# AbeelLab/phasm

Hardware: AMD Instinct MI355X
Metric: overlaps_per_sec (higher is better)
Workload: dtype u64

## Files before the change

include/phasm_overlap.h:

```cpp
#ifndef PHASM_OVERLAP_H
#define PHASM_OVERLAP_H

#include <stddef.h>
#include <stdint.h>

#ifdef __cplusplus
extern "C" {
#endif

#define PO_ABI_VERSION 4

typedef enum {
    PO_OK = 0,
    PO_ERR_INVALID = 1,
    PO_ERR_NOMEM = 2,
    PO_ERR_HIP = 3,
    PO_ERR_CAPACITY = 4
} po_status;

typedef struct po_handle po_handle;
typedef struct po_result po_result;

typedef struct {
    uint32_t a_idx, b_idx;
// ... 192 lines not shown

typedef struct {
    uint64_t n_edges_in;
    uint64_t n_edges_out;
    uint64_t n_nodes;
    uint64_t n_nodes_removed;
    uint64_t n_candidates;
    uint64_t n_diamonds;
    uint64_t n_rounds;
    uint64_t n_invalid;
    float ms_setup, ms_rounds, ms_emit, ms_total;
} po_diamond_stats;

po_status po_layout_diamonds(po_handle* h, po_result* edges, const po_diamond_params* params, uint8_t* edge_flags_out,
                             po_result** kept_out);
po_status po_get_diamond_stats(const po_handle* h, po_diamond_stats* out);


typedef struct {
    uint32_t reserved;
} po_merge_params;

typedef struct {
    uint64_t n_edges_in;
    uint64_t n_edges_out;
    uint64_t n_nodes;
    uint64_t n_merged;
    uint64_t n_nodes_merged;
    uint64_t max_path_nodes;
    uint64_t n_self_loops;
    uint64_t n_cycle_nodes;
    uint64_t n_rounds;
    uint64_t n_overflow;
    uint64_t n_invalid;
    float ms_links, ms_rank, ms_number, ms_emit, ms_total;
} po_merge_stats;

po_status po_layout_merge(po_handle* h, po_result* edges, const po_merge_params* params, uint8_t* edge_flags_out,
                          po_result** merged_out);
po_status po_get_merge_stats(const po_handle* h, po_merge_stats* out);

po_status po_result_merged_paths(po_result* merged, uint64_t* n_paths, uint64_t* n_members, uint64_t* offsets_out,
                                 uint64_t cap_paths, uint32_t* members_out, int32_t* prefix_out, uint64_t cap_members,
                                 int64_t* lengths_out);


typedef struct {
    uint32_t reserved;
} po_coverage_params;

typedef struct {
    uint64_t read_length_sum;
    int64_t path_length;
} po_edge_coverage;

typedef struct {
    uint64_t n_rows, n_edges;
    uint64_t n_nodes;
    uint64_t n_pairs;
    uint64_t max_set;
    uint64_t n_zero_path;
    uint64_t n_invalid;
    float ms_sets, ms_edges, ms_total;
} po_coverage_stats;

po_status po_layout_coverage(po_handle* h, po_result* graph, po_result* rows, const po_coverage_params* params,
                             po_edge_coverage* coverage_out );
po_status po_get_coverage_stats(const po_handle* h, po_coverage_stats* out);


typedef struct {
    uint32_t reserved;
} po_components_params;

typedef struct {
    uint32_t first_node;
    uint32_t n_nodes;
    uint64_t n_edges;
} po_component;

typedef struct {
    uint64_t n_nodes;
    uint64_t n_edges;
    uint64_t n_components;
    uint64_t n_singletons;
    uint64_t max_component_nodes, max_component_edges;
    uint64_t n_invalid;
    uint32_t n_rounds;
    uint32_t n_batches;
    float ms_rounds, ms_label, ms_total;
} po_components_stats;

po_status po_layout_components(po_handle* h, po_result* graph, const po_components_params* params,
                               uint32_t* node_component_out, uint32_t* edge_component_out, po_component* components_out,
                               uint64_t* n_components_out);
po_status po_get_components_stats(const po_handle* h, po_components_stats* out);


typedef struct {
    uint32_t reserved;
} po_partition_params;

typedef struct {
    uint32_t first_node;
    uint32_t n_nodes;
    uint64_t n_edges;
    uint32_t n_r_in;
    uint32_t n_re_out;
} po_scc;

#define PO_PART_R_IN 1u
#define PO_PART_RE_OUT 2u
#define PO_PART_START 4u
#define PO_PART_SINK 8u

typedef struct {
    uint64_t n_nodes;
    uint64_t n_edges;
    uint64_t n_sccs, n_nonsingleton_sccs, n_singletons;
    uint64_t n_self_loops;
    uint64_t max_scc_nodes, max_scc_edges;
    uint64_t n_trimmed;
    uint64_t n_class[5];
    uint64_t n_invalid;
    uint32_t n_outer;
    uint32_t n_trim_rounds, n_forward_rounds, n_backward_rounds;
    uint32_t n_batches;
    float ms_ranks, ms_rounds, ms_label, ms_total;
} po_partition_stats;

po_status po_layout_partition(po_handle* h, po_result* graph, const po_partition_params* params, uint32_t* node_scc_out,
                              uint8_t* node_flags_out, uint8_t* edge_class_out, po_scc* sccs_out, uint64_t* n_sccs_out);
po_status po_get_partition_stats(const po_handle* h, po_partition_stats* out);

po_status po_graph_from_edges(po_handle* h, const po_edge* edges, uint64_t n_edges, const uint32_t* node_order,
                              uint64_t n_order, po_result** out);

po_status po_result_node_order(po_result* r, uint32_t* nodes_out, uint64_t cap, uint64_t* n_out);

typedef struct {
    uint64_t n_rows;
    float ms_first_contained;
    float ms_rank;
    float ms_total;
} po_node_order_stats;
po_status po_get_node_order_stats(const po_handle* h, po_node_order_stats* out);

uint64_t po_debug_host_ranges(uint64_t* out, uint64_t cap_entries);
uint64_t po_debug_store_words(const po_handle* h, int store, const uint64_t** words);
int po_debug_expand_records(const po_cand* records, uint64_t n, const uint32_t* lengths, uint32_t n_reads, uint32_t paired,
                            po_row* rows_out, uint64_t n_rows_expected);
int po_debug_expand_packed(const uint64_t* records, uint64_t n, uint32_t sh_b, uint32_t sh_p, const uint32_t* lengths, uint32_t n_reads,
                           uint32_t paired, po_row* rows_out, uint64_t n_rows_expected);
int po_debug_fault_backtrace(int fd);
int po_debug_pointer_info(const void* p, int32_t* hip_type, int32_t* hsa_type, uint64_t* base, uint64_t* bytes);

po_status po_get_stats(const po_handle* h, po_stats* out);
const char* po_last_error(const po_handle* h);
int po_abi_version(void);

#ifdef __cplusplus
}
#endif
#endif
```

phasm_amd/_lib.py:

```python
from __future__ import annotations

import ctypes
import os

import numpy as np

HERE = os.path.dirname(os.path.abspath(__file__))
LIB_PATH = os.environ.get("PHASM_LIB") or os.path.join(HERE, "libphasm_overlap.so")

PO_OK, PO_ERR_INVALID, PO_ERR_NOMEM, PO_ERR_HIP, PO_ERR_CAPACITY = range(5)

ROW_DTYPE = np.dtype([("a_idx", "<u4"), ("b_idx", "<u4"), ("astart", "<i4"),
                      ("aend", "<i4"), ("bstart", "<i4"), ("bend", "<i4")])


CAND_DTYPE = np.dtype([("a_idx", "<u4"), ("p", "<u4"), ("b_idx", "<u4"), ("type", "<u4")])


EDGE_DTYPE = np.dtype([("u", "<u4"), ("v", "<u4"), ("weight", "<i4"), ("overlap_len", "<i4")])
COVERAGE_DTYPE = np.dtype([("read_length_sum", "<u8"), ("path_length", "<i8")])
COMPONENT_DTYPE = np.dtype([("first_node", "<u4"), ("n_nodes", "<u4"), ("n_edges", "<u8")])
SCC_DTYPE = np.dtype([("first_node", "<u4"), ("n_nodes", "<u4"), ("n_edges", "<u8"), ("n_r_in", "<u4"), ("n_re_out", "<u4")])
PART_R_IN, PART_RE_OUT, PART_START, PART_SINK = 1, 2, 4, 8


class PoLayoutParams(ctypes.Structure):
    _fields_ = [("min_read_length", ctypes.c_uint32), ("min_overlap_length", ctypes.c_uint32),
                ("max_overhang_abs", ctypes.c_uint32), ("reserved", ctypes.c_uint32),
                ("max_overhang_rel", ctypes.c_double)]


class PoLayoutStats(ctypes.Structure):
    _fields_ = [("n_rows", ctypes.c_uint64), ("n_type", ctypes.c_uint64 * 4), ("n_short", ctypes.c_uint64),
                ("n_min_overlap", ctypes.c_uint64), ("n_overhang", ctypes.c_uint64), ("n_pass", ctypes.c_uint64),
                ("n_contained_reads", ctypes.c_uint64), ("n_edges", ctypes.c_uint64),
                ("ms_classify", ctypes.c_float), ("ms_dedupe", ctypes.c_float), ("ms_emit", ctypes.c_float),
                ("ms_total", ctypes.c_float)]

    def as_dict(self) -> dict:
        d = {name: getattr(self, name) for name, _ in self._fields_}
        d["n_type"] = list(self.n_type)
        return d


class PoReduceParams(ctypes.Structure):
    _fields_ = [("length_fuzz", ctypes.c_int32), ("reserved", ctypes.c_uint32)]


class PoReduceStats(ctypes.Structure):
    _fields_ = [("n_edges_in", ctypes.c_uint64), ("n_transitive", ctypes.c_uint64), ("n_asymmetric", ctypes.c_uint64),
                ("n_edges_out", ctypes.c_uint64), ("max_out_degree", ctypes.c_uint64),
                ("ms_csr", ctypes.c_float), ("ms_mark", ctypes.c_float), ("ms_symmetric", ctypes.c_float),
                ("ms_emit", ctypes.c_float), ("ms_total", ctypes.c_float)]

    def as_dict(self) -> dict:
        return {name: getattr(self, name) for name, _ in self._fields_}


class PoTipsParams(ctypes.Structure):
    _fields_ = [("max_tip_len", ctypes.c_uint32), ("max_tip_len_bases", ctypes.c_int32), ("reserved", ctypes.c_uint32)]


class PoTipsStats(ctypes.Structure):
    _fields_ = [("n_edges_in", ctypes.c_uint64), ("n_in_tip_edges", ctypes.c_uint64), ("n_out_tip_edges", ctypes.c_uint64),
                ("n_asymmetric", ctypes.c_uint64), ("n_edges_out", ctypes.c_uint64), ("n_nodes", ctypes.c_uint64),
                ("n_isolated_nodes", ctypes.c_uint64), ("n_candidates_in", ctypes.c_uint64), ("n_candidates_out", ctypes.c_uint64),
                ("n_rounds_in", ctypes.c_uint64), ("n_rounds_out", ctypes.c_uint64),
                ("ms_setup", ctypes.c_float), ("ms_incoming", ctypes.c_float), ("ms_outgoing", ctypes.c_float),
                ("ms_symmetric", ctypes.c_float), ("ms_emit", ctypes.c_float), ("ms_total", ctypes.c_float)]

    def as_dict(self) -> dict:
        return {name: getattr(self, name) for name, _ in self._fields_}


class PoDiamondParams(ctypes.Structure):
    _fields_ = [("reserved", ctypes.c_uint32)]


class PoDiamondStats(ctypes.Structure):
    _fields_ = [("n_edges_in", ctypes.c_uint64), ("n_edges_out", ctypes.c_uint64), ("n_nodes", ctypes.c_uint64),
                ("n_nodes_removed", ctypes.c_uint64), ("n_candidates", ctypes.c_uint64), ("n_diamonds", ctypes.c_uint64),
                ("n_rounds", ctypes.c_uint64), ("n_invalid", ctypes.c_uint64),
                ("ms_setup", ctypes.c_float), ("ms_rounds", ctypes.c_float), ("ms_emit", ctypes.c_float), ("ms_total", ctypes.c_float)]

    def as_dict(self) -> dict:
        return {name: getattr(self, name) for name, _ in self._fields_}


class PoMergeParams(ctypes.Structure):
    _fields_ = [("reserved", ctypes.c_uint32)]


class PoMergeStats(ctypes.Structure):
    _fields_ = [("n_edges_in", ctypes.c_uint64), ("n_edges_out", ctypes.c_uint64), ("n_nodes", ctypes.c_uint64),
                ("n_merged", ctypes.c_uint64), ("n_nodes_merged", ctypes.c_uint64), ("max_path_nodes", ctypes.c_uint64),
                ("n_self_loops", ctypes.c_uint64), ("n_cycle_nodes", ctypes.c_uint64), ("n_rounds", ctypes.c_uint64),
                ("n_overflow", ctypes.c_uint64), ("n_invalid", ctypes.c_uint64),
                ("ms_links", ctypes.c_float), ("ms_rank", ctypes.c_float), ("ms_number", ctypes.c_float), ("ms_emit", ctypes.c_float),
                ("ms_total", ctypes.c_float)]

    def as_dict(self) -> dict:
        return {name: getattr(self, name) for name, _ in self._fields_}


class PoCoverageParams(ctypes.Structure):
    _fields_ = [("reserved", ctypes.c_uint32)]


class PoCoverageStats(ctypes.Structure):
    _fields_ = [("n_rows", ctypes.c_uint64), ("n_edges", ctypes.c_uint64), ("n_nodes", ctypes.c_uint64), ("n_pairs", ctypes.c_uint64),
                ("max_set", ctypes.c_uint64), ("n_zero_path", ctypes.c_uint64), ("n_invalid", ctypes.c_uint64),
                ("ms_sets", ctypes.c_float), ("ms_edges", ctypes.c_float), ("ms_total", ctypes.c_float)]

    def as_dict(self) -> dict:
        return {name: getattr(self, name) for name, _ in self._fields_}


class PoComponentsParams(ctypes.Structure):
    _fields_ = [("reserved", ctypes.c_uint32)]


class PoComponentsStats(ctypes.Structure):
    _fields_ = [("n_nodes", ctypes.c_uint64), ("n_edges", ctypes.c_uint64), ("n_components", ctypes.c_uint64),
                ("n_singletons", ctypes.c_uint64), ("max_component_nodes", ctypes.c_uint64), ("max_component_edges", ctypes.c_uint64),
                ("n_invalid", ctypes.c_uint64), ("n_rounds", ctypes.c_uint32), ("n_batches", ctypes.c_uint32),
                ("ms_rounds", ctypes.c_float), ("ms_label", ctypes.c_float), ("ms_total", ctypes.c_float)]

    def as_dict(self) -> dict:
        return {name: getattr(self, name) for name, _ in self._fields_}


class PoPartitionParams(ctypes.Structure):
    _fields_ = [("reserved", ctypes.c_uint32)]


class PoPartitionStats(ctypes.Structure):
    _fields_ = [("n_nodes", ctypes.c_uint64), ("n_edges", ctypes.c_uint64), ("n_sccs", ctypes.c_uint64),
                ("n_nonsingleton_sccs", ctypes.c_uint64), ("n_singletons", ctypes.c_uint64), ("n_self_loops", ctypes.c_uint64),
                ("max_scc_nodes", ctypes.c_uint64), ("max_scc_edges", ctypes.c_uint64), ("n_trimmed", ctypes.c_uint64),
                ("n_class", ctypes.c_uint64 * 5), ("n_invalid", ctypes.c_uint64), ("n_outer", ctypes.c_uint32),
                ("n_trim_rounds", ctypes.c_uint32), ("n_forward_rounds", ctypes.c_uint32), ("n_backward_rounds", ctypes.c_uint32),
                ("n_batches", ctypes.c_uint32),
                ("ms_ranks", ctypes.c_float), ("ms_rounds", ctypes.c_float), ("ms_label", ctypes.c_float), ("ms_total", ctypes.c_float)]

    def as_dict(self) -> dict:
        d = {name: getattr(self, name) for name, _ in self._fields_}
        d["n_class"] = list(self.n_class)
        return d


class PoNodeOrderStats(ctypes.Structure):
    _fields_ = [("n_rows", ctypes.c_uint64), ("ms_first_contained", ctypes.c_float), ("ms_rank", ctypes.c_float),
                ("ms_total", ctypes.c_float)]

    def as_dict(self) -> dict:
        return {name: getattr(self, name) for name, _ in self._fields_}


class PoStats(ctypes.Structure):
    _fields_ = [
        ("bits_per_base", ctypes.c_uint32), ("kmer", ctypes.c_uint32),
        ("paired", ctypes.c_uint32), ("wide_index", ctypes.c_uint32),
        ("n_reads", ctypes.c_uint64), ("n_eligible", ctypes.c_uint64),
        ("total_bases", ctypes.c_uint64), ("shard_bases", ctypes.c_uint64),
        ("n_tiles", ctypes.c_uint64), ("n_candidates", ctypes.c_uint64),
        ("n_verified", ctypes.c_uint64), ("n_rows", ctypes.c_uint64),
        ("sum_overlap_bases", ctypes.c_uint64), ("verify_bytes_algo", ctypes.c_uint64),
        ("ms_index", ctypes.c_float), ("ms_scan_count", ctypes.c_float),
        ("ms_scan_fill", ctypes.c_float), ("ms_verify", ctypes.c_float),
        ("ms_select", ctypes.c_float), ("ms_emit", ctypes.c_float),
        ("ms_total", ctypes.c_float), ("ms_upload", ctypes.c_float),
        ("ms_scan_probe", ctypes.c_float), ("ms_verify_kernel", ctypes.c_float),
        ("verify_bytes_exec", ctypes.c_uint64), ("dp_steps", ctypes.c_uint64), ("dp_stopped", ctypes.c_uint64),
        ("max_diff", ctypes.c_uint32), ("band", ctypes.c_uint32), ("index_reused", ctypes.c_uint32),
        ("dp_lanes", ctypes.c_uint32), ("upload_bytes", ctypes.c_uint64),
        ("streamed", ctypes.c_uint32), ("n_deferred", ctypes.c_uint32),
        ("fused_tail", ctypes.c_uint32), ("tail_fallback", ctypes.c_uint32),
        ("n_predicted", ctypes.c_uint32), ("home_record_bytes", ctypes.c_uint32),
    ]

    def as_dict(self) -> dict:
        return {name: getattr(self, name) for name, _ in self._fields_}


_P = ctypes.c_void_p
SYMBOLS = [
    ("po_abi_version", ctypes.c_int, []),
    ("po_create", ctypes.c_int, [ctypes.POINTER(_P)]),
    ("po_destroy", None, [_P]),
    ("po_set_device", ctypes.c_int, [_P, ctypes.c_int]),
    ("po_add_sequence", ctypes.c_int, [_P, ctypes.c_char_p, ctypes.c_size_t, ctypes.c_char_p, ctypes.c_size_t]),
    ("po_add_fasta", ctypes.c_int, [_P, ctypes.c_char_p, ctypes.c_int, ctypes.POINTER(ctypes.c_uint64)]),
    ("po_num_sequences", ctypes.c_uint32, [_P]),
    ("po_get_id", ctypes.c_int, [_P, ctypes.c_uint32, ctypes.POINTER(ctypes.c_void_p), ctypes.POINTER(ctypes.c_size_t)]),
    ("po_get_length", ctypes.c_uint32, [_P, ctypes.c_uint32]),
    ("po_upload", ctypes.c_int, [_P]),
    ("po_invalidate", ctypes.c_int, [_P]),
    ("po_upload_piece", ctypes.c_int, [_P, ctypes.c_uint32, ctypes.c_uint32, ctypes.c_void_p, ctypes.c_uint64,
                                       ctypes.POINTER(ctypes.c_uint64), ctypes.POINTER(ctypes.c_int)]),
    ("po_upload_assemble", ctypes.c_int, [_P, ctypes.c_void_p, ctypes.c_uint64, ctypes.c_uint32]),
    ("po_upload_piece_part", ctypes.c_int, [_P, ctypes.c_uint32, ctypes.c_uint32, ctypes.c_uint32, ctypes.c_uint32, ctypes.c_void_p,
                                            ctypes.c_uint64, ctypes.POINTER(ctypes.c_uint64), ctypes.POINTER(ctypes.c_int)]),
    ("po_upload_assemble_parts", ctypes.c_int, [_P, ctypes.c_void_p, ctypes.c_uint64, ctypes.c_uint32, ctypes.c_uint32]),
    ("po_overlaps", ctypes.c_int, [_P, ctypes.c_uint32, ctypes.POINTER(_P)]),
    ("po_overlaps_to_host", ctypes.c_int, [_P, ctypes.c_uint32, ctypes.POINTER(_P)]),
    ("po_overlaps_ex", ctypes.c_int, [_P, ctypes.c_uint32, ctypes.c_uint32, ctypes.c_uint32, ctypes.POINTER(_P)]),
    ("po_overlaps_shard", ctypes.c_int, [_P, ctypes.c_uint32, ctypes.c_uint32, ctypes.c_uint32, ctypes.POINTER(_P)]),
    ("po_candidates_shard", ctypes.c_int, [_P, ctypes.c_uint32, ctypes.c_uint32, ctypes.c_uint32, ctypes.POINTER(_P)]),
    ("po_expand", ctypes.c_int, [_P, ctypes.c_void_p, ctypes.c_uint64, ctypes.POINTER(_P)]),
    ("po_candidates_shard_into", ctypes.c_int, [_P, ctypes.c_uint32, ctypes.c_uint32, ctypes.c_uint32, ctypes.c_void_p,
                                               ctypes.c_uint64, ctypes.POINTER(ctypes.c_int), ctypes.POINTER(_P)]),
    ("po_index_slice_build", ctypes.c_int, [_P, ctypes.c_uint32, ctypes.c_uint32, ctypes.c_uint32, ctypes.POINTER(ctypes.c_uint32),
                                            ctypes.POINTER(ctypes.c_uint32), ctypes.POINTER(ctypes.c_uint64)]),
    ("po_index_chunk_bytes", ctypes.c_uint64, [ctypes.c_uint32, ctypes.c_uint64, ctypes.POINTER(ctypes.c_uint64)]),
    ("po_index_slice_export", ctypes.c_int, [_P, ctypes.c_void_p, ctypes.c_uint64]),
    ("po_candidates_shard_indexed", ctypes.c_int, [_P, ctypes.c_uint32, ctypes.c_uint32, ctypes.c_uint32, ctypes.c_void_p, ctypes.c_uint32,
                                                   ctypes.c_uint32, ctypes.c_uint64, ctypes.c_void_p, ctypes.c_uint64,
                                                   ctypes.POINTER(ctypes.c_int), ctypes.POINTER(_P)]),
    ("po_overlaps_shard_indexed", ctypes.c_int, [_P, ctypes.c_uint32, ctypes.c_uint32, ctypes.c_uint32, ctypes.c_void_p, ctypes.c_uint32,
                                                 ctypes.c_uint32, ctypes.c_uint64, ctypes.POINTER(_P)]),
    ("po_shard_range", ctypes.c_int, [_P, ctypes.c_uint32, ctypes.c_uint32, ctypes.POINTER(ctypes.c_uint32), ctypes.POINTER(ctypes.c_uint32)]),
    ("po_result_count", ctypes.c_uint64, [_P]),
    ("po_result_rows", ctypes.c_void_p, [_P]),
    ("po_result_rows_range", ctypes.c_void_p, [_P, ctypes.c_uint64, ctypes.c_uint64]),
    ("po_result_device_rows", ctypes.c_void_p, [_P]),
    ("po_result_copy_to_device", ctypes.c_int, [_P, ctypes.c_void_p]),
    ("po_result_copy_prefix_to_device", ctypes.c_int, [_P, ctypes.c_void_p, ctypes.c_uint64]),
    ("po_result_free", None, [_P]),
    ("po_write_gfa_edges", ctypes.c_int, [_P, ctypes.c_int, ctypes.POINTER(ctypes.c_uint64)]),
    ("po_write_gfa_segments", ctypes.c_int, [_P, ctypes.c_int, ctypes.POINTER(ctypes.c_uint64)]),
    ("po_add_segment", ctypes.c_int, [_P, ctypes.c_char_p, ctypes.c_size_t, ctypes.c_uint32]),
    ("po_result_from_rows", ctypes.c_int, [_P, ctypes.c_void_p, ctypes.c_uint64, ctypes.POINTER(_P)]),
    ("po_add_gfa", ctypes.c_int, [_P, ctypes.c_char_p, ctypes.POINTER(ctypes.c_uint64), ctypes.POINTER(_P)]),
    ("po_layout_edges", ctypes.c_int, [_P, _P, ctypes.POINTER(PoLayoutParams), ctypes.c_void_p, ctypes.POINTER(_P)]),
    ("po_get_layout_stats", ctypes.c_int, [_P, ctypes.POINTER(PoLayoutStats)]),
    ("po_layout_reduce", ctypes.c_int, [_P, _P, ctypes.POINTER(PoReduceParams), ctypes.c_void_p, ctypes.POINTER(_P)]),
    ("po_get_reduce_stats", ctypes.c_int, [_P, ctypes.POINTER(PoReduceStats)]),
    ("po_layout_tips", ctypes.c_int, [_P, _P, ctypes.POINTER(PoTipsParams), ctypes.c_void_p, ctypes.POINTER(_P)]),
    ("po_get_tips_stats", ctypes.c_int, [_P, ctypes.POINTER(PoTipsStats)]),
    ("po_layout_diamonds", ctypes.c_int, [_P, _P, ctypes.POINTER(PoDiamondParams), ctypes.c_void_p, ctypes.POINTER(_P)]),
    ("po_get_diamond_stats", ctypes.c_int, [_P, ctypes.POINTER(PoDiamondStats)]),
    ("po_layout_merge", ctypes.c_int, [_P, _P, ctypes.POINTER(PoMergeParams), ctypes.c_void_p, ctypes.POINTER(_P)]),
    ("po_get_merge_stats", ctypes.c_int, [_P, ctypes.POINTER(PoMergeStats)]),
    ("po_result_merged_paths", ctypes.c_int, [_P, ctypes.POINTER(ctypes.c_uint64), ctypes.POINTER(ctypes.c_uint64), ctypes.c_void_p,
                                              ctypes.c_uint64, ctypes.c_void_p, ctypes.c_void_p, ctypes.c_uint64, ctypes.c_void_p]),
    ("po_layout_coverage", ctypes.c_int, [_P, _P, _P, ctypes.POINTER(PoCoverageParams), ctypes.c_void_p]),
    ("po_get_coverage_stats", ctypes.c_int, [_P, ctypes.POINTER(PoCoverageStats)]),
    ("po_layout_components", ctypes.c_int, [_P, _P, ctypes.POINTER(PoComponentsParams), ctypes.c_void_p, ctypes.c_void_p, ctypes.c_void_p,
                                            ctypes.POINTER(ctypes.c_uint64)]),
    ("po_get_components_stats", ctypes.c_int, [_P, ctypes.POINTER(PoComponentsStats)]),
    ("po_layout_partition", ctypes.c_int, [_P, _P, ctypes.POINTER(PoPartitionParams), ctypes.c_void_p, ctypes.c_void_p, ctypes.c_void_p,
                                           ctypes.c_void_p, ctypes.POINTER(ctypes.c_uint64)]),
    ("po_get_partition_stats", ctypes.c_int, [_P, ctypes.POINTER(PoPartitionStats)]),
    ("po_graph_from_edges", ctypes.c_int, [_P, ctypes.c_void_p, ctypes.c_uint64, ctypes.c_void_p, ctypes.c_uint64, ctypes.POINTER(_P)]),
    ("po_result_node_order", ctypes.c_int, [_P, ctypes.c_void_p, ctypes.c_uint64, ctypes.POINTER(ctypes.c_uint64)]),
    ("po_get_node_order_stats", ctypes.c_int, [_P, ctypes.POINTER(PoNodeOrderStats)]),
    ("po_get_stats", ctypes.c_int, [_P, ctypes.POINTER(PoStats)]),
    ("po_last_error", ctypes.c_char_p, [_P]),
    ("po_debug_fault_backtrace", ctypes.c_int, [ctypes.c_int]),
    ("po_debug_store_words", ctypes.c_uint64, [_P, ctypes.c_int, ctypes.POINTER(ctypes.c_void_p)]),
    ("po_debug_expand_packed", ctypes.c_int, [ctypes.c_void_p, ctypes.c_uint64, ctypes.c_uint32, ctypes.c_uint32, ctypes.c_void_p, ctypes.c_uint32,
                                              ctypes.c_uint32, ctypes.c_void_p, ctypes.c_uint64]),
    ("po_debug_expand_records", ctypes.c_int, [ctypes.c_void_p, ctypes.c_uint64, ctypes.c_void_p, ctypes.c_uint32, ctypes.c_uint32,
                                               ctypes.c_void_p, ctypes.c_uint64]),
    ("po_debug_host_ranges", ctypes.c_uint64, [ctypes.POINTER(ctypes.c_uint64), ctypes.c_uint64]),
    ("po_debug_pointer_info", ctypes.c_int, [ctypes.c_void_p, ctypes.POINTER(ctypes.c_int32), ctypes.POINTER(ctypes.c_int32),
                                             ctypes.POINTER(ctypes.c_uint64), ctypes.POINTER(ctypes.c_uint64)]),
]

_lib = None


def _preload_torch_hip_runtime() -> None:
    import importlib.util
    if os.environ.get("PHASM_HIP_RUNTIME") == "system":
        return
    try:
        spec = importlib.util.find_spec("torch")
    except (ImportError, ValueError):
        spec = None
    if spec is None or not spec.submodule_search_locations:
        return
    path = os.path.join(list(spec.submodule_search_locations)[0], "lib", "libamdhip64.so")
    if os.path.exists(path):
        try:
            ctypes.CDLL(path, mode=ctypes.RTLD_GLOBAL)
        except OSError:
            pass


def load() -> ctypes.CDLL:
    global _lib
    if _lib is None:
        _preload_torch_hip_runtime()
        if not os.path.exists(LIB_PATH):
            raise ImportError(
                "%s not found: build it with `python -m phasm_amd.build` (hipcc, gfx950). "
                "phasm_amd has no CPU fallback." % LIB_PATH)
        lib = ctypes.CDLL(LIB_PATH)
        for name, restype, argtypes in SYMBOLS:
            fn = getattr(lib, name)
            fn.restype = restype
            fn.argtypes = argtypes
        _lib = lib
    return _lib
```

phasm_amd/csrc/c_api.hip:

```cpp
#include "../../include/phasm_overlap.h"

#include <hip/hip_runtime.h>

#include <dlfcn.h>
#include <execinfo.h>
#include <fcntl.h>
#include <signal.h>
#include <sys/mman.h>
#include <sys/stat.h>
#include <unistd.h>

#include <algorithm>
#include <array>
#include <atomic>
#include <chrono>
#include <cmath>
#include <condition_variable>
#include <cstdio>
#include <cstdlib>
#include <cstring>
#include <deque>
#include <functional>
#include <memory>
#include <mutex>
// ... 113 lines not shown
    T* allocate(size_t n) {
        const size_t bytes = ((n * sizeof(T) + REG_PAGE - 1) / REG_PAGE) * REG_PAGE;
        void* base = nullptr;
        if (posix_memalign(&base, REG_PAGE, bytes + REG_PAGE) != 0 || !base) throw std::bad_alloc();
        RegHeader* hd = static_cast<RegHeader*>(base);
        hd->bytes = bytes;
        hd->registered = 0;
        char* data = static_cast<char*>(base) + REG_PAGE;
        if (getenv("PHASM_POISON_HOST")) std::memset(data, 0xA5, bytes);
        if (!g_reg_defer) reg_now(data);
        return reinterpret_cast<T*>(data);
    }
    static void reg_now(void* data) {
        RegHeader* hd = reinterpret_cast<RegHeader*>(static_cast<char*>(data) - REG_PAGE);
        if (hd->registered || hd->bytes < (1u << 20) || getenv("PHASM_NO_PIN")) return;
        if (hipHostRegister(data, hd->bytes, hipHostRegisterPortable) == hipSuccess) {
            hd->registered = 1;
            pin_note(data, hd->bytes, 2u);
        } else {
            (void)hipGetLastError();
        }
    }
    template <class U> void construct(U*) noexcept {}
    template <class U, class A0, class... Args> void construct(U* q, A0&& a0, Args&&... args) {
        ::new (static_cast<void*>(q)) U(std::forward<A0>(a0), std::forward<Args>(args)...);
    }
    void deallocate(T* p, size_t) {
        char* base = reinterpret_cast<char*>(p) - REG_PAGE;
        RegHeader* hd = reinterpret_cast<RegHeader*>(base);
        if (hd->registered) {
            pin_drop(p);
            (void)hipHostUnregister(p);
        }
        free(base);
    }
    template <class U> bool operator==(const RegAlloc<U>&) const { return true; }
    template <class U> bool operator!=(const RegAlloc<U>&) const { return false; }
};
using WordStore = std::vector<uint64_t, RegAlloc<uint64_t>>;
inline bool store_is_pinned(const WordStore& w) {
    if (w.capacity() == 0) return false;
    const RegHeader* hd = reinterpret_cast<const RegHeader*>(reinterpret_cast<const char*>(w.data()) - REG_PAGE);
    return hd->registered != 0;
}
constexpr size_t STAGE_MAX = 4u << 20;

struct po_handle {
    int device = 0;
    bool dev_ready = false;
    hipStream_t stream = nullptr;
    hipEvent_t ev_sets[2][EV_N] = {};
    hipEvent_t* ev = ev_sets[0];
    hipEvent_t ev_up0 = nullptr, ev_up1 = nullptr;
    uint64_t* pinned = nullptr;
    uint64_t* pinned_dev = nullptr;
    int n_cu = 256;
    size_t lds_max = 64 * 1024;
    std::string err;

    int bits = 2;
    std::vector<std::string> ids;
    std::vector<uint32_t> len;
    std::vector<uint64_t> cum_len;
    std::vector<uint64_t> woff;
    WordStore words[2];
    bool all_pairs_rc = true;
    bool all_pairs_rcx = true;
    uint64_t base1 = 0;
    uint64_t dev_words = 0;
    uint64_t upload_bytes = 0;
    std::vector<uint32_t> exc_off{0};
    std::vector<uint32_t> exc_pos;
    std::vector<uint8_t> exc_byte;
    std::vector<uint8_t> pair_state;
    uint64_t total_bases = 0;
    bool dirty = true;

    DevBuf d_words, d_woff, d_len, d_tiles, d_read_tile0, d_exc_off, d_exc_pos, d_exc_byte, d_pair_state;
    std::vector<uint32_t> h_read_tile0;
    uint32_t n_tiles = 0;
    uint32_t max_len = 0;
    size_t n_exc_uploaded = 0;
    bool paired = false;

    DevBuf d_table, d_slot_cnt, d_slot_cur, d_slot_start, d_read_slot, d_chain, d_chain_tmp, d_long_list;
    DevBuf d_entry_off;
    DevBuf d_bloom, d_selfrep, d_tile_count, d_tile_off, d_truemask, d_ps_blocks, d_scalars, d_left, d_left_cnt, d_tile_extra;
    DevBuf d_cand_a, d_cand_p, d_cand_b, d_type, d_rowcnt, d_row_off, d_flag, d_pair_key, d_pair_min;
    DevBuf d_vlabel, d_vrank, d_vperm;
    DevBuf d_chain_state;
    DevBuf d_tail_state;
    DevBuf spare_rows;
    DevBuf spare_cands;
    DevBuf spare_edges;
    DevBuf spare_nrank;
    HostBuf spare_host;
    HostBuf scratch_host;
    uint64_t pool_bases = 0;
    double ws_scale = 1.0;
    std::vector<void*> arena_chunks;
    char* arena_cur = nullptr;
    size_t arena_left = 0;
    int poison = -1;
    hipStream_t copy_stream = nullptr;
    DevBuf chunk_rows[PO_MAX_PIECES + 1];
    bool chunk_compact[PO_MAX_PIECES + 1] = {};
    bool home_on = false;
    HostBuf home_stage;
    size_t home_used = 0;
    uint64_t home_seq = 0;
    uint32_t home_gen = 0;
    uint32_t home_sh_b = 0, home_sh_p = 0;
    uint64_t home_pack_n = ~0ull, home_pack_bases = ~0ull;
    uint32_t home_pack_b = 0, home_pack_p = 0;
    uint64_t home_last_bytes = 0;

    hipStream_t up_stream = nullptr;
    hipEvent_t ev_piece[PO_MAX_PIECES] = {};
    hipStream_t rc_stream = nullptr;
    hipEvent_t ev_rc[PO_MAX_PIECES] = {};
    hipEvent_t ev_meta = nullptr;
    hipEvent_t ev_first = nullptr;
    WordStore first_words;
    uint32_t first_n = 0;
    WordStore lead_words;
    uint32_t lead_n = 0;
    uint32_t st_lead = 2;
    HostBuf meta_host;
    HostBuf stage_host;
    size_t stage_used = 0;
    uint32_t meta_n = 0xFFFFFFFFu;
    int meta_bits = 0;
    uint64_t elig_n = ~0ull, elig_val = 0;
    uint32_t elig_m = 0;
    DevBuf d_first, d_defer;
    uint32_t defer_need = 0;
    struct Pending {
        bool valid = false;
        uint32_t k = 0;
        po_stats S = {};
        bool ver_timed = false;
        bool full_events = true;
        bool pair_events = true;
        bool tail = false;
        bool compact = false;
        int zone = 48;
        uint32_t cap_c = 0;
        hipEvent_t* ev = nullptr;
    } st_pend;
    std::function<po_status()> st_harvest;
    uint64_t st_pred_cand[PO_MAX_PIECES] = {};
    std::vector<uint32_t> st_pred_sig;
    bool st_pred_valid = false;
    bool phase_events = true;
    bool pair_events = true;
    bool st_selfclean = false;
    bool st_early_index = false;
    bool st_tail_gave_up = false;
    bool idx_only = false;
    bool st_on = false;
    uint32_t st_r_begin = 0, st_r_end = 0, st_defer_cap = 0;
    uint64_t last_host_rows = 0;
    uint64_t upload_gen = 0;
    bool idx_valid = false;
    uint64_t idx_gen = 0;
    uint32_t idx_m = 0, idx_tbits = 0, idx_bits = 0, idx_ww = 0;
    bool idx_wide = false;
    uint32_t sl_build_slice = 0, sl_build_n = 0;
    bool sl_is_wide = false;
    uint32_t sl_tbits = 0;
    uint64_t sl_entries = 0;
    const void* ext_index = nullptr;
    uint32_t ext_slices = 0, ext_tbits = 0, ext_chunk_slots = 0, ext_chain_off = 0;
    const uint64_t* asm_pieces = nullptr;
    uint64_t asm_slot_words = 0;
    uint32_t asm_n = 0, asm_parts = 1;
    bool ex_on = false;
    uint32_t ex_E = 0, ex_W = 0;
    DevBuf d_end_a, d_end_b, d_dpcnt;
    int live_results = 0;

    po_stats stats = {};

    bool segments_only = false;
    int ids_paired = -1;
    hipEvent_t ev_lay[EV_LAY_N] = {};
    DevBuf d_lay_len, d_lay_cnt, d_rflag, d_removed, d_ekey, d_ecnt, d_ewin, d_eoff;
    DevBuf d_efirst;
    po_layout_stats lstats = {};

    DevBuf d_red[RB_N];
    po_reduce_stats rstats = {};

    DevBuf d_lay_firstc;
    DevBuf d_tip[TB_N];
    po_tips_stats tstats = {};
    po_diamond_stats dstats = {};
    po_node_order_stats nostats = {};

    DevBuf d_mrg[MB_N];
    po_merge_stats mstats = {};

    DevBuf d_cov[VB_N];
    po_coverage_stats cstats = {};

    DevBuf d_rank[RK_N];
    DevBuf d_cc[KB_N];
    po_components_stats ccstats = {};
    DevBuf d_scc[PB_N];
    po_partition_stats pstats = {};
};

struct po_result {
    po_handle* h = nullptr;
    DevBuf d_rows;
    uint64_t count = 0;
    size_t elem = sizeof(po_row);
    bool kind_edges = false;
    void* host = nullptr;
    size_t host_cap = 0;
    bool host_malloced = false;
    bool unique_twins = false;
    DevBuf d_rank;
    DevBuf d_nrank;
    bool merged = false;
    bool host_graph = false;
    uint64_t n_merged = 0, n_members = 0;
    DevBuf d_moff, d_member, d_prefix, d_mlen;
    void* ext_dst = nullptr;
    uint64_t ext_cap = 0;
    bool wrote_ext = false;
    bool compact = false;
};

namespace {

po_status fail(po_handle* h, po_status st, const std::string& msg) {
    if (h) h->err = msg;
    return st;
}

#define HIP_TRY(h, expr)                                                                        \
    do {                                                                                        \
        hipError_t e_ = (expr);                                                                 \
        if (e_ != hipSuccess) {                                                                 \
            return fail((h), e_ == hipErrorOutOfMemory ? PO_ERR_NOMEM : PO_ERR_HIP,             \
                        std::string(#expr) + ": " + hipGetErrorString(e_));                     \
        }                                                                                       \
    } while (0)

struct AllocTrace {
    const char* what;
    size_t bytes;
    std::chrono::steady_clock::time_point t0;
    bool on;
    AllocTrace(const char* w, size_t b) : what(w), bytes(b), on(getenv("PHASM_ALLOC_TRACE") != nullptr) {
        if (on) t0 = std::chrono::steady_clock::now();
    }
    ~AllocTrace() {
        if (on)
            std::fprintf(stderr, "[alloc] %-16s %10.3f MB  %8.3f ms\n", what, bytes / 1e6,
                         std::chrono::duration<double, std::milli>(std::chrono::steady_clock::now() - t0).count());
    }
};

po_status ensure(po_handle* h, DevBuf& b, size_t bytes, double scale = 1.0, bool arena_ok = true) {
    if (bytes <= b.cap) return PO_OK;
    AllocTrace tr("hipMalloc", bytes);
    const bool first = b.p == nullptr;
    b.release();
    size_t want = bytes + bytes / 8 + 256;
    if (scale > 1.0) want = (size_t)((double)bytes * scale) + 256;
    if (h && h->st_on) want += 8192;
    constexpr size_t ARENA_CHUNK = 64u << 20, ARENA_MAX = 8u << 20;
    if (h && first && arena_ok && want <= ARENA_MAX && !getenv("PHASM_NO_ARENA")) {
        want = (want + 255) & ~size_t(255);
        if (h->arena_left < want) {
            void* c = nullptr;
            if (hipMalloc(&c, ARENA_CHUNK) == hipSuccess) {
                h->arena_chunks.push_back(c);
                h->arena_cur = static_cast<char*>(c);
                h->arena_left = ARENA_CHUNK;
            } else {
                (void)hipGetLastError();
            }
        }
        if (h->arena_left >= want) {
            b.p = h->arena_cur;
            b.cap = want;
            b.arena = true;
            h->arena_cur += want;
            h->arena_left -= want;
            if (h->poison >= 0 && h->stream) (void)hipMemsetAsync(b.p, h->poison, want, h->stream);
            return PO_OK;
        }
    }
    hipError_t e = hipMalloc(&b.p, want);
    if (e != hipSuccess) {
        b.p = nullptr;
        return fail(h, PO_ERR_NOMEM, "hipMalloc(" + std::to_string(want) + " bytes): " + hipGetErrorString(e));
    }
    b.cap = want;
    if (h && h->poison >= 0 && h->stream) (void)hipMemsetAsync(b.p, h->poison, want, h->stream);
    return PO_OK;
}

po_status ensure_piece(po_handle* h, DevBuf& b, size_t bytes) { return ensure(h, b, bytes, h->ws_scale); }

po_status ensure_host(po_handle* h, HostBuf& b, size_t bytes) {
    if (bytes <= b.cap) return PO_OK;
    AllocTrace tr("hipHostMalloc", bytes);
    b.release();
    const size_t want = bytes + bytes / 16 + 4096;
    hipError_t e = hipHostMalloc(&b.p, want, hipHostMallocDefault);
    if (e != hipSuccess) {
        b.p = nullptr;
        return fail(h, PO_ERR_NOMEM, "hipHostMalloc(" + std::to_string(want) + " bytes): " + hipGetErrorString(e));
    }
    b.cap = want;
    pin_note(b.p, want, 1u);
    return PO_OK;
}

void quiesce_store(po_handle* h) {
    if (!h->dev_ready) return;
    (void)hipSetDevice(h->device);
    (void)hipStreamSynchronize(h->stream);
    if (h->up_stream) (void)hipStreamSynchronize(h->up_stream);
    if (h->rc_stream) (void)hipStreamSynchronize(h->rc_stream);
}

po_status init_device(po_handle* h);

inline bool home_enabled() {
    const char* e = getenv("PHASM_HOME");
    return !(e && atoi(e) == 0);
}

void result_pool_grow(po_handle* h, uint64_t bases = 0) {
    if (!bases) bases = h->total_bases;
    h->pool_bases = bases + bases / 2;
    if (getenv("PHASM_NO_POOL")) return;
    if (!h->dev_ready && init_device(h) != PO_OK) h->err.clear();
    const uint64_t want = std::min<uint64_t>(h->pool_bases / 160 * sizeof(po_row), 4ull << 30);
    if (h->spare_host.cap >= want || h->live_results) return;
    int n = 0;
    if (hipGetDeviceCount(&n) != hipSuccess || n == 0) {
        (void)hipGetLastError();
        h->pool_bases = ~0ull;
        return;
    }
    AllocTrace tr("result pool", want);
    h->spare_host.release();
    if (hipHostMalloc(&h->spare_host.p, want, hipHostMallocPortable) == hipSuccess) {
        h->spare_host.cap = want;
        pin_note(h->spare_host.p, want, 1u);
        if (home_enabled() && h->home_stage.cap < want / 3) (void)ensure_host(h, h->home_stage, want / 3);
        if (h->dev_ready && h->up_stream && h->copy_stream && want >= (16u << 20) && !getenv("PHASM_NO_WARM")) {
            void* w = nullptr;
            const size_t nb = 8u << 20;
            if (hipMalloc(&w, nb) == hipSuccess) {
                (void)hipMemcpyAsync(w, h->spare_host.p, nb, hipMemcpyHostToDevice, h->up_stream);
                (void)hipStreamSynchronize(h->up_stream);
                (void)hipMemcpyAsync(static_cast<char*>(h->spare_host.p) + nb, w, nb, hipMemcpyDeviceToHost, h->copy_stream);
                (void)hipStreamSynchronize(h->copy_stream);
                (void)hipFree(w);
            }
            (void)hipGetLastError();
        }
    } else {
        (void)hipGetLastError();
        h->spare_host.p = nullptr;
        h->pool_bases = ~0ull;
    }
}

#define PO_TRY(expr)                    \
    do {                                \
        po_status s_ = (expr);          \
        if (s_ != PO_OK) return s_;     \
    } while (0)

struct DevKit {
    int device = -1;
    hipStream_t stream = nullptr, copy_stream = nullptr, up_stream = nullptr, rc_stream = nullptr;
    hipEvent_t ev_sets[2][EV_N] = {};
    hipEvent_t ev_up0 = nullptr, ev_up1 = nullptr, ev_meta = nullptr, ev_first = nullptr;
    hipEvent_t ev_piece[PO_MAX_PIECES] = {}, ev_rc[PO_MAX_PIECES] = {}, ev_lay[EV_LAY_N] = {};

    uint64_t* pinned = nullptr;
    uint64_t* pinned_dev = nullptr;
};
static_assert(sizeof(DevKit::ev_lay) == sizeof(po_handle::ev_lay), "a kit carries every layout event of a handle");
std::mutex g_kit_mu;
std::vector<DevKit> g_kits;
constexpr size_t KIT_POOL_MAX = 8;

bool kit_take(po_handle* h) {
    std::lock_guard<std::mutex> lock(g_kit_mu);
    for (size_t i = 0; i < g_kits.size(); ++i) {
        if (g_kits[i].device != h->device) continue;
        const DevKit k = g_kits[i];
        g_kits.erase(g_kits.begin() + (long)i);
        h->stream = k.stream;
        h->copy_stream = k.copy_stream;
        h->up_stream = k.up_stream;
        h->rc_stream = k.rc_stream;
        std::memcpy(h->ev_sets, k.ev_sets, sizeof(k.ev_sets));
        h->ev_up0 = k.ev_up0;
        h->ev_up1 = k.ev_up1;
        h->ev_meta = k.ev_meta;
        h->ev_first = k.ev_first;
        std::memcpy(h->ev_piece, k.ev_piece, sizeof(k.ev_piece));
        std::memcpy(h->ev_rc, k.ev_rc, sizeof(k.ev_rc));
        std::memcpy(h->ev_lay, k.ev_lay, sizeof(k.ev_lay));
        h->pinned = k.pinned;
        h->pinned_dev = k.pinned_dev;
        return true;
    }
    return false;
}

bool kit_give(po_handle* h) {
    if (getenv("PHASM_NO_KIT_POOL") || !h->stream || !h->copy_stream || !h->up_stream || !h->rc_stream || !h->pinned) return false;
    if (hipStreamSynchronize(h->stream) != hipSuccess || hipStreamSynchronize(h->copy_stream) != hipSuccess ||
        hipStreamSynchronize(h->up_stream) != hipSuccess || hipStreamSynchronize(h->rc_stream) != hipSuccess) {
        (void)hipGetLastError();
        return false;
    }
    DevKit k;
    k.device = h->device;
    k.stream = h->stream;
    k.copy_stream = h->copy_stream;
    k.up_stream = h->up_stream;
    k.rc_stream = h->rc_stream;
    std::memcpy(k.ev_sets, h->ev_sets, sizeof(k.ev_sets));
    k.ev_up0 = h->ev_up0;
    k.ev_up1 = h->ev_up1;
    k.ev_meta = h->ev_meta;
    k.ev_first = h->ev_first;
    std::memcpy(k.ev_piece, h->ev_piece, sizeof(k.ev_piece));
    std::memcpy(k.ev_rc, h->ev_rc, sizeof(k.ev_rc));
    std::memcpy(k.ev_lay, h->ev_lay, sizeof(k.ev_lay));
    k.pinned = h->pinned;
    k.pinned_dev = h->pinned_dev;
    std::lock_guard<std::mutex> lock(g_kit_mu);
    if (g_kits.size() >= KIT_POOL_MAX) return false;
    g_kits.push_back(k);
    return true;
}


unsigned cpu_share() {
    static const unsigned share = [] {
        unsigned n = std::thread::hardware_concurrency();
        n = n ? n : 4u;
        long long q = -1, per = 100000;
        if (FILE* f = std::fopen("/sys/fs/cgroup/cpu.max", "r")) {
            char buf[64] = {0};
            if (std::fscanf(f, "%63s %lld", buf, &per) >= 1 && std::strcmp(buf, "max") != 0) q = atoll(buf);
            std::fclose(f);
        } else if (FILE* g = std::fopen("/sys/fs/cgroup/cpu/cpu.cfs_quota_us", "r")) {
            if (std::fscanf(g, "%lld", &q) != 1) q = -1;
            std::fclose(g);
            if (FILE* g2 = std::fopen("/sys/fs/cgroup/cpu/cpu.cfs_period_us", "r")) {
                if (std::fscanf(g2, "%lld", &per) != 1) per = 100000;
                std::fclose(g2);
            }
        }
        if (q > 0 && per > 0) n = std::min<unsigned>(n, (unsigned)std::max<long long>(1, q / per));
        return n;
    }();
    return share;
}

namespace home {

constexpr uint32_t CHUNK = 4096;

struct Job {
    const void* rec = nullptr;
    uint32_t sh_b = 0, sh_p = 0;
    uint64_t n_rec = 0;
    po_row* out = nullptr;
    uint64_t n_rows = 0;
    const volatile uint32_t* flag = nullptr;
    uint32_t want = 0;
    uint32_t paired = 0, bits = 2;
};

struct Pool {
    std::vector<std::thread> thr;
    std::mutex mu;
    std::condition_variable cv_queue;
    std::condition_variable cv_job;
    std::mutex call_mu;
// ... 428 lines not shown
    h->first_words.clear();
    h->lead_n = 0;
    h->lead_words.clear();
    h->exc_off.assign(1, 0);
    h->exc_pos.clear();
    h->exc_byte.clear();
    h->pair_state.clear();
}

const unsigned char* comp_table() {
    static unsigned char comp[256];
    static bool init = false;
    if (!init) {
        for (int i = 0; i < 256; ++i) comp[i] = (unsigned char)i;
        const char* from = "ACGTURYKMBVDHSWNacgturykmbvdhswn";
        const char* to = "TGCAAYRMKVBHDSWNtgcaayrmkvbhdswn";
        for (int i = 0; from[i]; ++i) comp[(unsigned char)from[i]] = (unsigned char)to[i];
        init = true;
    }
    return comp;
}

void host_pair_check(po_handle* h, size_t r, const unsigned char* s) {
    const size_t pair = r / 2;
    if (h->pair_state.size() <= pair) h->pair_state.resize(pair + 1, 0);
    const bool has_exc = h->exc_off[r - 1] != h->exc_off[r] || h->exc_off[r] != h->exc_off[r + 1];
    if (!has_exc) return;
    const uint32_t n = h->len[r];
    uint8_t state = 1;
    if (h->len[r - 1] != n) {
        state = 2;
    } else {
        std::vector<unsigned char> prev;
        materialize(h, r - 1, h->words, h->woff.data(), prev);
        const unsigned char* c = comp_table();
        for (uint32_t i = 0; i < n; ++i) {
            const unsigned char x = prev[n - 1 - i], y = s[i];
            if (c[x] != y || c[y] != x) {
                state = 2;
                break;
            }
        }
    }
    h->pair_state[pair] = state;
}

bool packed_is_revcomp(const po_handle* h, size_t r) {
    const uint32_t L = h->len[r];
    if (h->len[r - 1] != L) return false;
    if (h->exc_off[r - 1] != h->exc_off[r] || h->exc_off[r] != h->exc_off[r + 1]) return false;
    const uint64_t* R = h->words[0].data() + h->woff[r - 1];
    const uint64_t* S = h->words[1].data() + h->woff[r];
    const uint32_t nw = (L + 31) / 32;
    for (uint32_t w = 0; w < nw; ++w) {
        const int64_t o = (int64_t)L - 32 * (int64_t)w - 32;
        uint64_t x;
        uint32_t valid = 32;
        if (o >= 0) {
            const uint32_t sh = (uint32_t)(o & 31) * 2;
            x = sh ? (R[o >> 5] >> sh) | (R[(o >> 5) + 1] << (64 - sh)) : R[o >> 5];
        } else {
            valid = (uint32_t)(32 + o);
            x = R[0] << ((uint32_t)(-o) * 2);
        }
        uint64_t y = __builtin_bitreverse64(x);
        y = ((y >> 1) & 0x5555555555555555ull) | ((y & 0x5555555555555555ull) << 1);
        y = ~y;
        const uint64_t mask = valid >= 32 ? ~0ull : ((1ull << (valid * 2)) - 1ull);
        if (((y ^ S[w]) & mask) != 0) return false;
    }
    return true;
}

inline uint32_t cdiv(uint64_t a, uint32_t b) { return (uint32_t)((a + b - 1) / b); }

void note_first_words(po_handle* h) {
    const uint32_t n = (uint32_t)h->len.size();
    if (h->first_n == n && h->first_words.size() == 2 * (size_t)n) return;
    if (h->first_n > n || h->first_words.size() != 2 * (size_t)h->first_n) {
        h->first_n = 0;
        h->first_words.clear();
    }
    if (n - h->first_n > 1) h->first_words.reserve(2 * (size_t)n);
    for (uint32_t r = h->first_n; r < n; ++r) {
        const WordStore& store = h->words[r & 1];
        const uint64_t o = h->woff[r];
        h->first_words.push_back(o < store.size() ? store[o] : 0);
        h->first_words.push_back(o + 1 < store.size() ? store[o + 1] : 0);
    }
    h->first_n = n;
}

constexpr uint32_t LEAD_WORDS = 5;
void note_lead_words(po_handle* h) {
    const uint32_t n = (uint32_t)h->len.size();
    if (h->lead_n == n && h->lead_words.size() == (size_t)LEAD_WORDS * n) return;
    if (h->lead_n > n || h->lead_words.size() != (size_t)LEAD_WORDS * h->lead_n) {
        h->lead_n = 0;
        h->lead_words.clear();
    }
    h->lead_words.resize((size_t)LEAD_WORDS * n, 0);
    uint64_t* out = h->lead_words.data();
    for (uint32_t r = h->lead_n; r < n; ++r) {
        const WordStore& store = h->words[r & 1];
        const uint64_t o = h->woff[r];
        for (uint32_t k = 0; k < LEAD_WORDS; ++k) out[(size_t)r * LEAD_WORDS + k] = o + k < store.size() ? store[o + k] : 0;
    }
    h->lead_n = n;
}

uint64_t count_eligible(po_handle* h, uint32_t m) {
    const uint64_t n = h->len.size();
    if (h->elig_n != n || h->elig_m != m) {
        uint64_t c = 0;
        for (uint64_t r = 0; r < n; ++r) c += h->len[r] >= m;
        h->elig_n = n;
        h->elig_m = m;
        h->elig_val = c;
    }
    return h->elig_val;
}

void shard_range(const po_handle* h, uint32_t shard, uint32_t nshards, uint32_t* r_begin, uint32_t* r_end, uint64_t* bases);

void store0_range(const po_handle* h, uint32_t shard, uint32_t nshards, uint64_t* begin, uint64_t* count) {
    uint32_t rb = 0, re = 0;
    shard_range(h, shard, nshards, &rb, &re, nullptr);
    const uint32_t n = (uint32_t)h->len.size();
    const uint32_t e0 = (rb + 1u) & ~1u, e1 = (re + 1u) & ~1u;
    const uint64_t w0 = e0 < n ? h->woff[e0] : h->words[0].size();
    const uint64_t w1 = e1 < n ? h->woff[e1] : h->words[0].size();
    *begin = w0;
    *count = w1 > w0 ? w1 - w0 : 0;
}

void store0_part_range(const po_handle* h, uint32_t shard, uint32_t nshards, uint32_t part, uint32_t nparts, uint64_t* begin, uint64_t* count) {
    uint64_t wb = 0, wc = 0;
    store0_range(h, shard, nshards, &wb, &wc);
    const uint64_t cs = (((wc + nparts - 1) / nparts) + 1) & ~uint64_t(1);
    const uint64_t lo = std::min(wc, (uint64_t)part * cs), hi = std::min(wc, (uint64_t)(part + 1) * cs);
    *begin = wb + lo;
    *count = hi - lo;
}

const void* staged(po_handle* h, const void* src, size_t bytes) {
    if (!bytes || bytes > STAGE_MAX || !h->stage_host.p) return src;
    const size_t off = (h->stage_used + 63) & ~size_t(63);
    if (off + bytes > h->stage_host.cap) return src;
    std::memcpy(static_cast<char*>(h->stage_host.p) + off, src, bytes);
    h->stage_used = off + bytes;
    return static_cast<const char*>(h->stage_host.p) + off;
}

po_status upload_meta(po_handle* h, bool* generate_out) {
    const uint32_t n = (uint32_t)h->len.size();
    const size_t per = 64 / h->bits;
    {
        size_t need = 0;
        for (const WordStore& w : h->words)
            if (!store_is_pinned(w) && w.size() * 8 <= STAGE_MAX) need += w.size() * 8 + 64;
        if (h->bits == 2) need += ((size_t)n + 1) * 4 + h->exc_pos.size() * 5 + 192;
        need += n / 2 + 64;
        h->stage_used = 0;
        if (need > 256) PO_TRY(ensure_host(h, h->stage_host, need));
    }
    if (h->meta_n != n || h->meta_bits != h->bits || !h->meta_host.p) {
        h->h_read_tile0.assign((size_t)n + 1, 0);
        h->max_len = 0;
        uint64_t nt = 0;
        for (uint32_t r = 0; r < n; ++r) {
            h->h_read_tile0[r] = (uint32_t)nt;
            h->max_len = std::max(h->max_len, h->len[r]);
            const size_t nw = (h->len[r] + per - 1) / per;
            nt += (nw + po::TILE_WORDS - 1) / po::TILE_WORDS;
            if (nt > 0x7FFFFF00ull / po::WAVE) return fail(h, PO_ERR_CAPACITY, "too many scan tiles");
        }
        h->h_read_tile0[n] = (uint32_t)nt;
        h->n_tiles = (uint32_t)nt;
        PO_TRY(ensure_host(h, h->meta_host, (size_t)n * 16 + 64));
        char* mh = static_cast<char*>(h->meta_host.p);
        if (n) {
            std::memcpy(mh, h->woff.data(), (size_t)n * 8);
            std::memcpy(mh + (size_t)n * 8, h->len.data(), (size_t)n * 4);
        }
        std::memcpy(mh + (size_t)n * 12, h->h_read_tile0.data(), ((size_t)n + 1) * 4);
        h->meta_n = n;
        h->meta_bits = h->bits;
    }
    const char* mh = static_cast<const char*>(h->meta_host.p);

    const uint64_t base1 = (h->words[0].size() + 1) & ~uint64_t(1);
    const uint64_t nwords = base1 + h->words[1].size() + 72;
    const bool generate = h->bits == 2 && n >= 2 && (n % 2) == 0 && h->all_pairs_rcx && !getenv("PHASM_FULL_UPLOAD");
    *generate_out = generate;
    h->base1 = base1;
    h->dev_words = nwords;
    PO_TRY(ensure(h, h->d_words, nwords * 8));
    PO_TRY(ensure(h, h->d_woff, ((size_t)n + 1) * 8));
    PO_TRY(ensure(h, h->d_len, ((size_t)n + 1) * 4));
    PO_TRY(ensure(h, h->d_tiles, ((size_t)h->n_tiles + 1) * sizeof(po::TileRec)));
    PO_TRY(ensure(h, h->d_read_tile0, ((size_t)n + 1) * 4));
    HIP_TRY(h, hipEventRecord(h->ev_up0, h->stream));
    uint64_t* dw = h->d_words.as<uint64_t>();
    HIP_TRY(h, hipMemsetAsync(dw + base1 + h->words[1].size(), 0, 72 * 8, h->stream));
    if (base1 != h->words[0].size()) HIP_TRY(h, hipMemsetAsync(dw + h->words[0].size(), 0, 8, h->stream));
    h->upload_bytes = 0;
    if (n) {
        HIP_TRY(h, hipMemcpyAsync(h->d_woff.p, mh, (size_t)n * 8, hipMemcpyHostToDevice, h->stream));
        HIP_TRY(h, hipMemcpyAsync(h->d_len.p, mh + (size_t)n * 8, (size_t)n * 4, hipMemcpyHostToDevice, h->stream));
        h->upload_bytes += (size_t)n * 12;
        hipLaunchKernelGGL(po::k_abs_woff, dim3(cdiv(n, 256)), dim3(256), 0, h->stream, h->d_woff.as<uint64_t>(), n, base1);
    }
    HIP_TRY(h, hipMemcpyAsync(h->d_read_tile0.p, mh + (size_t)n * 12, ((size_t)n + 1) * 4, hipMemcpyHostToDevice, h->stream));
    h->upload_bytes += ((size_t)n + 1) * 4;
    if (h->n_tiles) {
        hipLaunchKernelGGL(po::k_build_tiles, dim3(cdiv(h->n_tiles, 256)), dim3(256), 0, h->stream, h->d_woff.as<uint64_t>(),
                           h->d_len.as<uint32_t>(), h->d_read_tile0.as<uint32_t>(), n, h->n_tiles, h->d_tiles.as<po::TileRec>());
    }
    const size_t n_exc = h->bits == 2 ? h->exc_pos.size() : 0;
    if (n_exc) {
        PO_TRY(ensure(h, h->d_exc_off, ((size_t)n + 1) * 4));
        PO_TRY(ensure(h, h->d_exc_pos, n_exc * 4));
        PO_TRY(ensure(h, h->d_exc_byte, n_exc));
        HIP_TRY(h, hipMemcpyAsync(h->d_exc_off.p, staged(h, h->exc_off.data(), ((size_t)n + 1) * 4), ((size_t)n + 1) * 4, hipMemcpyHostToDevice, h->stream));
        HIP_TRY(h, hipMemcpyAsync(h->d_exc_pos.p, staged(h, h->exc_pos.data(), n_exc * 4), n_exc * 4, hipMemcpyHostToDevice, h->stream));
        HIP_TRY(h, hipMemcpyAsync(h->d_exc_byte.p, staged(h, h->exc_byte.data(), n_exc), n_exc, hipMemcpyHostToDevice, h->stream));
        h->upload_bytes += ((size_t)n + 1) * 4 + n_exc * 5;
    }
    h->n_exc_uploaded = n_exc;
    HIP_TRY(h, hipGetLastError());
    return PO_OK;
}

po_status upload(po_handle* h) {
    PO_TRY(init_device(h));
    if (!h->dirty) return PO_OK;
    const uint32_t n = (uint32_t)h->len.size();
    bool generate = false;
    PO_TRY(upload_meta(h, &generate));
    uint64_t* dw = h->d_words.as<uint64_t>();
    const uint64_t base1 = h->base1;
    if (h->asm_pieces) {
        if (!generate) return fail(h, PO_ERR_INVALID, "po_upload_assemble needs reads added as (x, reverse complement of x) pairs");
        for (uint32_t part = 0; part < h->asm_parts; ++part) {
            for (uint32_t k = 0; k < h->asm_n; ++k) {
                uint64_t wb = 0, wc = 0;
                store0_part_range(h, k, h->asm_n, part, h->asm_parts, &wb, &wc);
                if (wc > h->asm_slot_words) return fail(h, PO_ERR_INVALID, "po_upload_assemble: a piece is longer than the slot");
                if (wc) HIP_TRY(h, hipMemcpyAsync(dw + wb, h->asm_pieces + ((size_t)part * h->asm_n + k) * h->asm_slot_words, wc * 8,
                                                  hipMemcpyDeviceToDevice, h->stream));
            }
        }
    } else if (!h->words[0].empty()) {
        const void* src0 = store_is_pinned(h->words[0]) ? h->words[0].data() : staged(h, h->words[0].data(), h->words[0].size() * 8);
        HIP_TRY(h, hipMemcpyAsync(dw, src0, h->words[0].size() * 8, hipMemcpyHostToDevice, h->stream));
        h->upload_bytes += h->words[0].size() * 8;
    }
    if (!generate && !h->words[1].empty()) {
        const void* src1 = store_is_pinned(h->words[1]) ? h->words[1].data() : staged(h, h->words[1].data(), h->words[1].size() * 8);
        HIP_TRY(h, hipMemcpyAsync(dw + base1, src1, h->words[1].size() * 8, hipMemcpyHostToDevice, h->stream));
        h->upload_bytes += h->words[1].size() * 8;
    }
    if (generate) {
        hipLaunchKernelGGL(po::k_revcomp_store, dim3(cdiv((uint64_t)(n / 2) * 64, 256)), dim3(256), 0, h->stream, dw,
                           h->d_woff.as<uint64_t>(), h->d_len.as<uint32_t>(), 0u, n / 2,
                           h->n_exc_uploaded ? h->d_exc_off.as<uint32_t>() : nullptr, h->d_exc_pos.as<uint32_t>());
        if (getenv("PHASM_VERIFY_GENERATED") && !h->words[1].empty()) {
            DevBuf tmp;
            PO_TRY(ensure(h, tmp, h->words[1].size() * 8));
            PO_TRY(ensure(h, h->d_scalars, 128));
            HIP_TRY(h, hipMemsetAsync(h->d_scalars.p, 0, 64, h->stream));
            HIP_TRY(h, hipMemcpyAsync(tmp.p, h->words[1].data(), h->words[1].size() * 8, hipMemcpyHostToDevice, h->stream));
            hipLaunchKernelGGL(po::k_count_diff, dim3(1024), dim3(256), 0, h->stream, dw + base1, tmp.as<uint64_t>(),
                               (uint64_t)h->words[1].size(), h->d_scalars.as<unsigned long long>());
            HIP_TRY(h, hipMemcpyAsync(h->pinned, h->d_scalars.p, 8, hipMemcpyDeviceToHost, h->stream));
            HIP_TRY(h, hipStreamSynchronize(h->stream));
            tmp.release();
            if (h->pinned[0] != 0)
                return fail(h, PO_ERR_HIP, "generated reverse-complement store differs from the host's in " +
                                               std::to_string(h->pinned[0]) + " words");
        }
    }
    HIP_TRY(h, hipGetLastError());
    const size_t n_exc = h->n_exc_uploaded;
    h->paired = false;
    const bool mirror_ok = !getenv("PHASM_NO_MIRROR");
    const bool try_paired = h->bits == 2 && n >= 2 && (n % 2) == 0 && mirror_ok && !generate;
    if (generate && mirror_ok) h->paired = true;
    if (try_paired) {
        PO_TRY(ensure(h, h->d_scalars, 128));
        HIP_TRY(h, hipMemsetAsync(h->d_scalars.p, 0, 64, h->stream));
        const uint8_t* pair_state = nullptr;
        if (n_exc) {
            h->pair_state.resize(n / 2, 0);
            PO_TRY(ensure(h, h->d_pair_state, n / 2));
            HIP_TRY(h, hipMemcpyAsync(h->d_pair_state.p, staged(h, h->pair_state.data(), n / 2), n / 2, hipMemcpyHostToDevice, h->stream));
            pair_state = h->d_pair_state.as<uint8_t>();
        }
        hipLaunchKernelGGL(po::k_paired_check, dim3(cdiv((uint64_t)(n / 2) * 64, 256)), dim3(256), 0, h->stream,
                           h->d_words.as<uint64_t>(), h->d_woff.as<uint64_t>(), h->d_len.as<uint32_t>(), n / 2, pair_state,
                           h->d_scalars.as<uint32_t>());
        HIP_TRY(h, hipGetLastError());
        HIP_TRY(h, hipMemcpyAsync(h->pinned, h->d_scalars.p, 8, hipMemcpyDeviceToHost, h->stream));
    }
    HIP_TRY(h, hipEventRecord(h->ev_up1, h->stream));
    HIP_TRY(h, hipStreamSynchronize(h->stream));
    if (try_paired) h->paired = (uint32_t)h->pinned[0] == 0;
    float ms = 0;
    (void)hipEventElapsedTime(&ms, h->ev_up0, h->ev_up1);
    h->stats.ms_upload = ms;
    h->stats.upload_bytes = h->upload_bytes;
    ++h->upload_gen;
    h->dirty = false;
    return PO_OK;
}

void shard_range(const po_handle* h, uint32_t shard, uint32_t nshards, uint32_t* r_begin, uint32_t* r_end, uint64_t* bases) {
    const uint32_t n = (uint32_t)h->len.size();
    std::vector<uint64_t>& cum = const_cast<po_handle*>(h)->cum_len;
    if (cum.size() != (size_t)n + 1) {
        size_t have = cum.empty() ? 0 : std::min(cum.size() - 1, (size_t)n);
        cum.resize((size_t)n + 1);
        if (have == 0) cum[0] = 0;
        for (size_t r = have; r < n; ++r) cum[r + 1] = cum[r] + h->len[r];
    }
    auto cut = [&](uint32_t s) -> uint32_t {
        if (s == 0) return 0;
        if (s >= nshards) return n;
        const uint64_t target = (uint64_t)((__uint128_t)cum[n] * s / nshards);
        return (uint32_t)(std::lower_bound(cum.begin(), cum.end(), target) - cum.begin());
    };
    *r_begin = cut(shard);
    *r_end = cut(shard + 1);
    if (*r_end < *r_begin) *r_end = *r_begin;
    if (bases) *bases = cum[*r_end] - cum[*r_begin];
}

po_status chain_state(po_handle* h, uint32_t n_tiles, po::ChainState** out, hipStream_t on) {
    const size_t need = po::chain_state_bytes(n_tiles);
    if (need > h->d_chain_state.cap) {
        PO_TRY(ensure(h, h->d_chain_state, std::max<size_t>(need * 2, 1u << 16)));
        HIP_TRY(h, hipMemsetAsync(h->d_chain_state.p, 0, h->d_chain_state.cap, on));
    }
    *out = h->d_chain_state.as<po::ChainState>();
    return PO_OK;
}

template <typename T>
po_status prefix_sum(po_handle* h, const T* in, uint64_t n, uint32_t* out, volatile uint64_t* total_host,
                     const uint64_t* also_src = nullptr, volatile uint64_t* also_host = nullptr, const uint32_t* extra = nullptr,
                     hipStream_t on = nullptr, uint64_t* total_dev_at = nullptr) {
    *total_host = 0;
    if (n == 0) return PO_OK;
    const hipStream_t ps = on ? on : h->stream;
    const uint32_t nblocks = cdiv(n, po::PS_TILE);
    uint64_t* total_dev = total_dev_at ? total_dev_at : h->d_scalars.as<uint64_t>();
    uint64_t* total_mapped = h->pinned_dev + (const_cast<uint64_t*>(total_host) - h->pinned);
    uint64_t* also_mapped = also_host ? h->pinned_dev + (const_cast<uint64_t*>(also_host) - h->pinned) : nullptr;
    if (nblocks <= 64 && !getenv("PHASM_PS_CLASSIC")) {

        po::ChainState* cs = nullptr;
        PO_TRY(chain_state(h, nblocks, &cs, ps));
        hipLaunchKernelGGL(po::k_ps_chain<T>, dim3(nblocks), dim3(po::PS_BLOCK), 0, ps, const_cast<T*>(in), extra, n, out, cs,
                           nblocks, total_dev, total_mapped, also_src, also_mapped);
        HIP_TRY(h, hipGetLastError());
        return PO_OK;
    }
    if (extra) {
        hipLaunchKernelGGL(po::k_add_extra, dim3(cdiv(n, 256)), dim3(256), 0, ps, const_cast<uint32_t*>(reinterpret_cast<const uint32_t*>(in)),
                           extra, 0u, (uint32_t)n);
    }
    PO_TRY(ensure_piece(h, h->d_ps_blocks, (size_t)nblocks * 8));
    uint64_t* blocks = h->d_ps_blocks.as<uint64_t>();
    hipLaunchKernelGGL(po::k_ps_reduce<T>, dim3(nblocks), dim3(po::PS_BLOCK), 0, ps, in, n, blocks);
    hipLaunchKernelGGL(po::k_ps_spine, dim3(1), dim3(1024), 0, ps, blocks, nblocks, total_dev, total_mapped, also_src, also_mapped);
    hipLaunchKernelGGL(po::k_ps_down<T>, dim3(nblocks), dim3(po::PS_BLOCK), 0, ps, in, n, blocks, out);
    HIP_TRY(h, hipGetLastError());
    return PO_OK;
}

po_status prefix_sum_small(po_handle* h, uint32_t* in, const uint32_t* extra, uint32_t n, uint32_t* out, volatile uint64_t* total_host,
                           const uint64_t* also_src, volatile uint64_t* also_host, hipStream_t on = nullptr, uint64_t* total_dev_at = nullptr) {
    *total_host = 0;
    if (n == 0) return PO_OK;
    const hipStream_t ps = on ? on : h->stream;
    uint64_t* total_dev = total_dev_at ? total_dev_at : h->d_scalars.as<uint64_t>();
    uint64_t* total_mapped = h->pinned_dev + (const_cast<uint64_t*>(total_host) - h->pinned);
    uint64_t* also_mapped = also_host ? h->pinned_dev + (const_cast<uint64_t*>(also_host) - h->pinned) : nullptr;
    hipLaunchKernelGGL(po::k_ps_small, dim3(1), dim3(1024), 0, ps, in, extra, n, out, total_dev, total_mapped,
                       also_src, also_mapped);
    HIP_TRY(h, hipGetLastError());
    return PO_OK;
}

void stage_times(po_stats& S, hipEvent_t* ev, bool ver_timed, bool full, bool pairs = true) {
    if (!full && !pairs) {
        S.ms_index = S.ms_scan_count = S.ms_scan_fill = S.ms_verify = S.ms_select = S.ms_emit = 0.f;
        S.ms_total = S.ms_scan_probe = S.ms_verify_kernel = 0.f;
        return;
    }
    if (!full) {
        S.ms_index = S.ms_scan_count = S.ms_scan_fill = S.ms_verify = S.ms_select = S.ms_emit = 0.f;
        (void)hipEventElapsedTime(&S.ms_total, ev[EV_START], ev[EV_EMIT]);
        (void)hipEventElapsedTime(&S.ms_scan_probe, ev[EV_PROBE0], ev[EV_PROBE1]);
        S.ms_verify_kernel = 0.f;
        if (ver_timed) (void)hipEventElapsedTime(&S.ms_verify_kernel, ev[EV_VER0], ev[EV_VER1]);
        return;
    }
    (void)hipEventElapsedTime(&S.ms_index, ev[EV_START], ev[EV_INDEX]);
    (void)hipEventElapsedTime(&S.ms_scan_count, ev[EV_INDEX], ev[EV_COUNT]);
    (void)hipEventElapsedTime(&S.ms_scan_fill, ev[EV_COUNT], ev[EV_FILL]);
    (void)hipEventElapsedTime(&S.ms_verify, ev[EV_FILL], ev[EV_VERIFY]);
    (void)hipEventElapsedTime(&S.ms_select, ev[EV_VERIFY], ev[EV_SELECT]);
    (void)hipEventElapsedTime(&S.ms_emit, ev[EV_SELECT], ev[EV_EMIT]);
    (void)hipEventElapsedTime(&S.ms_total, ev[EV_START], ev[EV_EMIT]);
    (void)hipEventElapsedTime(&S.ms_scan_probe, ev[EV_PROBE0], ev[EV_PROBE1]);
    S.ms_verify_kernel = 0.f;
    if (ver_timed) (void)hipEventElapsedTime(&S.ms_verify_kernel, ev[EV_VER0], ev[EV_VER1]);
}

uint64_t finish_piece(po_handle* h, bool* needs_classic) {
    po_handle::Pending& P = h->st_pend;
    const int o = P.tail ? P.zone : 2, c = P.tail ? P.zone + 1 : 4;
    *needs_classic = P.tail && h->pinned[P.zone + 7] != 0;
    if (P.cap_c) {
        P.S.n_candidates = h->pinned[P.zone + 8];
        if (P.S.n_candidates > P.cap_c) *needs_classic = true;
    }
    const uint64_t n_rows = h->pinned[o];
    P.S.n_rows = n_rows;
    P.S.n_verified = h->pinned[c];
    P.S.sum_overlap_bases = h->pinned[c + 1];
    P.S.verify_bytes_algo = h->pinned[c + 2];
    P.S.verify_bytes_exec = h->pinned[c + 3];
    stage_times(P.S, P.ev, P.ver_timed, P.full_events, P.pair_events);
    P.valid = false;
    return n_rows;
}

template <int BITS>
po_status run_overlaps(po_handle* h, uint32_t min_length, uint32_t shard, uint32_t nshards, bool want_cands,
                       po_result* res) {
    constexpr uint32_t W = 64 / BITS;
    const uint32_t n = (uint32_t)h->len.size();
    const uint32_t m = min_length ? min_length : 1;
    const uint32_t K = m < W ? m : W;
    const uint64_t kmask = K * BITS >= 64 ? ~0ull : ((1ull << (K * BITS)) - 1ull);
    hipStream_t st = h->stream;
    po_stats& S = h->stats;
    const float keep_upload = S.ms_upload;
    S = po_stats();
    S.ms_upload = keep_upload;
    S.upload_bytes = h->upload_bytes;
    S.bits_per_base = BITS;
    S.kmer = K;
    S.n_reads = n;
    S.total_bases = h->total_bases;
    const bool dp = h->ex_on;
    const uint32_t dpE = dp ? h->ex_E : 0u, dpW = dp && h->ex_E ? h->ex_W : 0u;
    const bool streamed = h->st_on;
    const uint32_t paired = (BITS == 2 && h->paired && dpE == 0) ? (streamed ? po::PAIRED_STREAM_ALL : nshards > 1 ? 2u : 1u) : 0u;
    const uint32_t paired_ver = streamed ? po::paired_stream(h->st_r_end) : paired;
    if (streamed && (!paired || want_cands)) return fail(h, PO_ERR_INVALID, "streamed step without strand pairs");
    S.paired = paired ? 1u : 0u;
    S.max_diff = dpE;
    S.band = dpW;
    if (dp && dpE && want_cands) return fail(h, PO_ERR_INVALID, "the candidate (multi-GPU) form has no inexact mode");
    if (dp && dpE && BITS == 2 && !h->exc_pos.empty())
        return fail(h, PO_ERR_INVALID, "po_overlaps_ex with max_diff > 0 needs pure upper-case ACGT reads (or the 8-bit representation)");

    uint32_t r_begin = 0, r_end = n;
    S.shard_bases = h->total_bases;
    if (streamed) {
        r_begin = h->st_r_begin;
        r_end = h->st_r_end;
        S.shard_bases = 0;
        for (uint32_t r = r_begin; r < r_end; ++r) S.shard_bases += h->len[r];
    } else if (nshards > 1) {
        shard_range(h, shard, nshards, &r_begin, &r_end, &S.shard_bases);
    }
    const uint32_t tile_begin = h->h_read_tile0[r_begin], tile_end = h->h_read_tile0[r_end];
    const uint32_t ntiles = tile_end - tile_begin;
    S.n_tiles = ntiles;

    const uint64_t n_elig = count_eligible(h, m);
    S.n_eligible = n_elig;
    res->count = 0;
    if (n == 0 || n_elig == 0 || ntiles == 0) return PO_OK;

    bool wide = n_elig > 160000 && m >= 2 * W - 1;
    if (const char* e = getenv("PHASM_INDEX")) {
        if (!strcmp(e, "wide")) wide = m >= 2 * W - 1;
        if (!strcmp(e, "narrow")) wide = false;
    }
    S.wide_index = wide ? 1u : 0u;
    uint32_t ww = 1;
    if (wide && BITS == 2) {
        ww = m >= W * 16 + W - 1 ? 16u : m >= W * 4 + W - 1 ? 4u : 1u;
        if (streamed) ww = (ww >= 4 && h->st_lead >= LEAD_WORDS) ? 4u : 1u;
        if (const char* e = getenv("PHASM_WIDE_WINDOW")) {
            const uint32_t v = (uint32_t)atoi(e);
            if ((v == 1 || v == 4 || v == 16) && v <= ww) ww = v;
        }
    }
    bool WA_ext = false;
    const bool slice_build = h->sl_build_n > 1;
    const bool ext_idx = h->ext_index != nullptr;
    if (slice_build) {
        h->sl_is_wide = wide;
        if (!wide) return PO_OK;
    }
    if (ext_idx && !wide) return fail(h, PO_ERR_INVALID, "a sliced index was supplied, but this call uses the narrow index");
    bool rows_late = false;
    bool cands_late = false, cands_ext = false;
    uint64_t cands_cap = 0;
    bool self_clean = false;
    bool used_tail = false;
    int tail_zone = 48;
    std::function<po_status()> tail_fallback;
    bool ver_timed = false;
    uint64_t n_keys = wide ? n_elig * W : n_elig;
    if (slice_build) n_keys = n_keys / h->sl_build_n + n_keys / (16ull * h->sl_build_n) + 4096;
    uint32_t tbits = 10;
    double table_mult = wide ? 2.0 : 5.0;
    if (const char* e = getenv("PHASM_TABLE_MULT")) table_mult = std::max(wide ? 2.0 : 1.5, atof(e));
    if (slice_build) table_mult = 1.5;
    while ((double)(1ull << tbits) < table_mult * (double)n_keys) ++tbits;
    if (ext_idx) tbits = h->ext_tbits;
    if (tbits > 30) return fail(h, PO_ERR_CAPACITY, "too many reads for the anchor table");
    const uint32_t nslots = (1u << tbits) + (wide ? 1u : po::PROBE_GROUP);
    uint32_t bloom_log2 = 13;
    while (bloom_log2 < 20 && (1ull << bloom_log2) < 16 * n_elig) ++bloom_log2;
    const size_t bloom_bytes = (size_t)1 << (bloom_log2 - 3);

    PO_TRY(ensure(h, h->d_scalars, 128));
    const size_t n_entries = wide ? (size_t)n * W : (size_t)n;
    const size_t chain_elem = wide ? 8 : 4;
    if (!ext_idx) {
        PO_TRY(ensure(h, h->d_table, (size_t)nslots * sizeof(po::Slot)));
        PO_TRY(ensure(h, h->d_slot_cnt, (size_t)nslots * 4));
        PO_TRY(ensure(h, h->d_slot_cur, (size_t)nslots * 4));
        PO_TRY(ensure(h, h->d_slot_start, ((size_t)nslots + 1) * 4));
        PO_TRY(ensure(h, h->d_read_slot, n_entries * 4));
        const size_t chain_entries = slice_build ? n_entries / h->sl_build_n + n_entries / (4ull * h->sl_build_n) + 65536 : n_entries;
        PO_TRY(ensure(h, h->d_chain, std::min(chain_entries, n_entries) * chain_elem));
        PO_TRY(ensure(h, h->d_chain_tmp, std::min(chain_entries, n_entries) * chain_elem));
        PO_TRY(ensure(h, h->d_long_list, (size_t)nslots * 4));
        if (wide) PO_TRY(ensure(h, h->d_entry_off, n_entries * 2));
    }
    PO_TRY(ensure(h, h->d_bloom, bloom_bytes));
    PO_TRY(ensure(h, h->d_selfrep, (size_t)n * 4));
    PO_TRY(ensure(h, h->d_tile_count, ((size_t)h->n_tiles + 1) * 4));
    PO_TRY(ensure(h, h->d_tile_off, ((size_t)h->n_tiles + 2) * 4 * 2));
    PO_TRY(ensure(h, h->d_truemask, ((size_t)h->n_tiles + 1) * po::WAVE * 4));

    const uint64_t* words = h->d_words.as<uint64_t>();
    const uint64_t* woff = h->d_woff.as<uint64_t>();
    const uint32_t* len = h->d_len.as<uint32_t>();
    po::Slot* table = h->d_table.as<po::Slot>();
    uint32_t* slot_cnt = h->d_slot_cnt.as<uint32_t>();
    uint32_t* slot_cur = h->d_slot_cur.as<uint32_t>();
    uint32_t* slot_start = h->d_slot_start.as<uint32_t>();
    uint32_t* read_slot = h->d_read_slot.as<uint32_t>();
    uint32_t* chain = h->d_chain.as<uint32_t>();
    uint32_t* bloom = h->d_bloom.as<uint32_t>();
    uint32_t* selfrep = h->d_selfrep.as<uint32_t>();
    const uint32_t parity = streamed ? (shard & 1u) : 0u;
    unsigned long long* scalars = h->d_scalars.as<unsigned long long>() + 8 * parity;
    uint32_t* const tile_off_p = h->d_tile_off.as<uint32_t>() + (size_t)parity * ((size_t)h->n_tiles + 2);
    uint32_t* n_long = reinterpret_cast<uint32_t*>(scalars + 1);

    if (h->poison >= 0) {
        DevBuf* ws[] = {&h->d_table, &h->d_slot_cnt, &h->d_slot_cur, &h->d_slot_start, &h->d_read_slot, &h->d_chain,
                        &h->d_chain_tmp, &h->d_long_list, &h->d_bloom, &h->d_selfrep, &h->d_tile_count, &h->d_tile_off,
                        &h->d_truemask, &h->d_ps_blocks, &h->d_left, &h->d_left_cnt, &h->d_tile_extra, &h->d_cand_a,
                        &h->d_cand_p, &h->d_cand_b, &h->d_type, &h->d_rowcnt, &h->d_row_off, &h->d_flag, &h->d_pair_key,
                        &h->d_vlabel, &h->d_vrank, &h->d_vperm, &h->spare_rows, &h->spare_cands};
        for (DevBuf* b : ws)
            if (b->p) HIP_TRY(h, hipMemsetAsync(b->p, h->poison, b->cap, st));
    }
// ... 48 lines not shown
        hipLaunchKernelGGL(k_cfill, dim3(cdiv(n_entries, 256)), dim3(256), 0, st, read_slot, entry_off,
                           (uint64_t)n_entries, slot_start, slot_cur, chain64, len);
        hipLaunchKernelGGL(po::k_chain_sort_short<uint64_t>, dim3(cdiv(nslots, 256)), dim3(256), 0, st, slot_cnt, slot_start,
                           nslots, chain64, h->d_long_list.as<uint32_t>(), n_long);
        hipLaunchKernelGGL(po::k_chain_sort_long<uint64_t>, dim3(64), dim3(256), 0, st, slot_cnt, slot_start,
                           h->d_long_list.as<uint32_t>(), n_long, chain64, h->d_chain_tmp.as<uint64_t>());
        hipLaunchKernelGGL(k_fin, dim3(cdiv(nslots, 256)), dim3(256), 0, st, table, nslots, slot_cnt,
                           slot_start, chain64, len);
    }
    HIP_TRY(h, hipGetLastError());
    if (h->phase_events) HIP_TRY(h, hipEventRecord(h->ev[EV_INDEX], st));
    if (slice_build) {
        HIP_TRY(h, hipStreamSynchronize(st));
        h->sl_tbits = tbits;
        h->sl_entries = h->pinned[0];
        if (h->phase_events) (void)hipEventElapsedTime(&S.ms_index, h->ev[EV_START], h->ev[EV_INDEX]);
        return PO_OK;
    }
    if (ext_idx) {
        WA_ext = true;
    }
    if (h->idx_only) {
        h->idx_valid = true;
        h->idx_gen = h->upload_gen;
        h->idx_m = m;
        h->idx_wide = wide;
        h->idx_tbits = tbits;
        h->idx_bits = (uint32_t)BITS;
        h->idx_ww = ww;
        return PO_OK;
    }
    h->idx_valid = !ext_idx;
    h->idx_gen = h->upload_gen;
    h->idx_m = m;
    h->idx_wide = wide;
    h->idx_tbits = tbits;
    h->idx_bits = (uint32_t)BITS;
    h->idx_ww = ww;

    po::ScanArgs A = {};
    A.words = words;
    A.tiles = h->d_tiles.as<po::TileRec>();
    A.tile_begin = tile_begin;
    A.tile_end = tile_end;
    A.m = m;
    A.kmask = kmask;
    A.bloom = bloom;
    A.bloom_log2 = bloom_log2;
    A.table = table;
    A.tbits = tbits;
    A.chain = chain;
    A.len = len;
    A.paired = paired;
    A.selfrep = selfrep;
    A.n_selfrep = reinterpret_cast<uint32_t*>(scalars + 2);
    A.tile_count = h->d_tile_count.as<uint32_t>();
    A.tile_off = tile_off_p;
    A.truemask = h->d_truemask.as<uint32_t>();
#ifdef PO_STAMPS
    PO_TRY(ensure(h, h->d_flag, (size_t)4096 * 64));
    HIP_TRY(h, hipMemsetAsync(h->d_flag.p, 0, (size_t)4096 * 64, st));
    A.dbg = h->d_flag.as<unsigned long long>();
#endif
    uint32_t scan_waves = po::SCAN_BLOCK / 64;
    if (const char* e = getenv("PHASM_SCAN_WAVES")) scan_waves = std::max(1, std::min(16, atoi(e)));
    const uint32_t scan_grid = std::max<uint32_t>(1, std::min<uint32_t>((uint32_t)h->n_cu, cdiv(ntiles, scan_waves)));
    po::WideArgs WA = {};
    WA.words = words;
    WA.tiles = A.tiles;
    WA.tile_begin = tile_begin;
    WA.tile_end = tile_end;
    WA.m = m;
    WA.table = table;
    WA.tbits = tbits;
    WA.chain = h->d_chain.as<uint64_t>();
    WA.n_slices = 1;
    if (WA_ext) {
        WA.table = static_cast<const po::Slot*>(h->ext_index);
        WA.chain = nullptr;
        WA.n_slices = h->ext_slices;
        WA.chunk_slots = h->ext_chunk_slots;
        WA.chain_off_slots = h->ext_chain_off;
    }
    WA.len = len;
    WA.paired = paired;
    WA.tile_count = A.tile_count;
    WA.lane_slot = A.truemask;
    WA.tile_off = A.tile_off;
    if (wide) {
        if (h->pair_events) HIP_TRY(h, hipEventRecord(h->ev[EV_PROBE0], st));
        auto wscan = streamed ? (ww == 4 ? po::k_wide_scan<BITS, false, BITS == 2, 4> : po::k_wide_scan<BITS, false, BITS == 2, 1>)
                     : ww == 16 ? po::k_wide_scan<BITS, false, false, 16> : ww == 4 ? po::k_wide_scan<BITS, false, false, 4> : po::k_wide_scan<BITS, false, false, 1>;
        hipLaunchKernelGGL(wscan, dim3(cdiv(ntiles, 4)), dim3(256), 0, st, WA, po::CandGuard{nullptr, 0u});
        if (h->pair_events) HIP_TRY(h, hipEventRecord(h->ev[EV_PROBE1], st));
    } else {
        const size_t scan_lds = (size_t)scan_waves * po::SCAN_LDS_PER_WAVE + bloom_bytes;
        if (scan_lds > h->lds_max) return fail(h, PO_ERR_HIP, "device LDS too small for the scan kernel");
        constexpr bool CAN_STREAM = BITS == 2;
        auto probe_full = streamed ? po::k_scan_probe<BITS, true, CAN_STREAM> : po::k_scan_probe<BITS, true, false>;
        auto probe_part = streamed ? po::k_scan_probe<BITS, false, CAN_STREAM> : po::k_scan_probe<BITS, false, false>;
        HIP_TRY(h, hipFuncSetAttribute(reinterpret_cast<const void*>(probe_full), hipFuncAttributeMaxDynamicSharedMemorySize, (int)scan_lds));
        HIP_TRY(h, hipFuncSetAttribute(reinterpret_cast<const void*>(probe_part), hipFuncAttributeMaxDynamicSharedMemorySize, (int)scan_lds));
        const uint32_t n_scan_waves = scan_grid * scan_waves;
        PO_TRY(ensure(h, h->d_left, (size_t)n_scan_waves * po::LEFT_CAP * sizeof(uint2)));
        PO_TRY(ensure(h, h->d_left_cnt, (size_t)n_scan_waves * 4));
        PO_TRY(ensure(h, h->d_tile_extra, ((size_t)h->n_tiles + 1) * 4));
        self_clean = streamed && !getenv("PHASM_DEBUG_LEFT") && !getenv("PHASM_PIECE_RESET");
        if (fold_clear && self_clean && h->st_selfclean) {
        } else if (fold_clear) {
            const uint32_t te0 = self_clean ? 0u : tile_begin, ten = self_clean ? h->n_tiles : ntiles;
            hipLaunchKernelGGL(po::k_call_reset, dim3(cdiv(std::max(std::max(n, 16u), std::max(n_scan_waves, ten)), 256)), dim3(256), 0, st,
                               selfrep, n, self_clean ? h->d_scalars.as<unsigned long long>() : scalars, self_clean ? 16u : 8u,
                               h->d_left_cnt.as<uint32_t>(), n_scan_waves, h->d_tile_extra.as<uint32_t>() + te0, ten);
        } else {
            HIP_TRY(h, hipMemsetAsync(h->d_left_cnt.p, 0, (size_t)n_scan_waves * 4, st));
            HIP_TRY(h, hipMemsetAsync(h->d_tile_extra.as<uint32_t>() + tile_begin, 0, (size_t)ntiles * 4, st));
        }
        A.left = h->d_left.as<uint2>();
        A.left_cnt = h->d_left_cnt.as<uint32_t>();
        A.tile_extra = h->d_tile_extra.as<uint32_t>();
        if (h->pair_events) HIP_TRY(h, hipEventRecord(h->ev[EV_PROBE0], st));
        hipLaunchKernelGGL(K == W ? probe_full : probe_part, dim3(scan_grid), dim3(scan_waves * 64), scan_lds, st, A);
        if (h->pair_events) HIP_TRY(h, hipEventRecord(h->ev[EV_PROBE1], st));
        auto fixup = streamed ? po::k_scan_fixup<BITS, CAN_STREAM> : po::k_scan_fixup<BITS, false>;
        hipLaunchKernelGGL(fixup, dim3(n_scan_waves), dim3(256), 0, st, A, n_scan_waves, self_clean ? 1u : 0u);
        if (getenv("PHASM_DEBUG_LEFT")) {
            PO_TRY(ensure_host(h, h->scratch_host, (size_t)n_scan_waves * 4));
            HIP_TRY(h, hipMemcpyAsync(h->scratch_host.p, h->d_left_cnt.p, (size_t)n_scan_waves * 4, hipMemcpyDeviceToHost, st));
            HIP_TRY(h, hipStreamSynchronize(st));
            const uint32_t* lc = static_cast<const uint32_t*>(h->scratch_host.p);
            uint64_t sum = 0;
            uint32_t mx = 0;
            for (uint32_t k = 0; k < n_scan_waves; ++k) sum += lc[k], mx = std::max(mx, lc[k]);
            std::fprintf(stderr, "[left] %u scan waves deferred %llu positions (max %u per wave, cap %d)\n", n_scan_waves,
                         (unsigned long long)sum, mx, (int)po::LEFT_CAP);
        }
    }
    HIP_TRY(h, hipGetLastError());
#ifdef PO_STAMPS
    if (!wide) {
        std::vector<unsigned long long> dbg(4096 * 8);
        HIP_TRY(h, hipMemcpyAsync(dbg.data(), h->d_flag.p, dbg.size() * 8, hipMemcpyDeviceToHost, st));
        HIP_TRY(h, hipStreamSynchronize(st));
        double sum[6] = {0, 0, 0, 0, 0, 0};
        for (size_t w = 0; w < 4096; ++w) for (int k = 0; k < 6; ++k) sum[k] += (double)dbg[w * 8 + k];
        if (sum[5] > 0)
            std::fprintf(stderr, "[stamps] per pass (cycles): wait_rw %.0f  filter %.0f  wait_probe %.0f  consume %.0f  issue %.0f  (passes %.0f)\n",
                         sum[0] / sum[5], sum[1] / sum[5], sum[2] / sum[5], sum[3] / sum[5], sum[4] / sum[5], sum[5]);
    }
#endif
    const int zone = 64 + 16 * (int)(shard & 1u);
    uint32_t cap_c = 0;
    bool async_count = false, pred_order = true;
    if (streamed && h->st_harvest && h->st_pred_valid && !dp && !want_cands && !getenv("PHASM_SYNC_COUNT") && !getenv("PHASM_TAIL_CLASSIC")) {
        uint64_t pred = h->st_pred_cand[shard];
        uint64_t cap = pred + pred / 50 + 256;
        if (const char* e = getenv("PHASM_PRED_SCALE")) cap = pred = (uint64_t)((double)pred * atof(e));
        const uint64_t worst = cap * 4u;
        bool order = pred >= 400000 && (r_end - r_begin) >= 4096;
        if (const char* e = getenv("PHASM_VERIFY_ORDER")) order = atoi(e) != 0;
        pred_order = order;
        auto fits = [](const DevBuf& b, uint64_t bytes) { return b.p && b.cap >= bytes; };
        async_count = pred > 0 && cap < (16u << 20) && cdiv(cap, po::TAIL_TILE) <= po::TAIL_MAX_TILES &&
                      fits(h->d_cand_a, cap * 4) && fits(h->d_cand_p, cap * 4) && fits(h->d_cand_b, cap * 4) && fits(h->d_type, cap) &&
                      fits(h->d_rowcnt, cap) && fits(h->d_row_off, (cap + 1) * 4) &&
                      fits(h->spare_rows, h->home_on ? cap * sizeof(po::Cand) : worst * sizeof(po_row)) &&
                      (!order || (fits(h->d_vlabel, (uint64_t)(r_end - r_begin) * 4) && fits(h->d_vperm, (uint64_t)(r_end - r_begin) * 4) &&
                                  fits(h->d_vrank, (uint64_t)(r_end - r_begin) * 4))) && h->dev_words < 0xFFFFFFF0ull;
        cap_c = (uint32_t)cap;
    }
    volatile uint64_t* count_slot = async_count ? &h->pinned[zone + 8] : &h->pinned[1];
    volatile uint64_t* also_slot = async_count ? &h->pinned[zone + 9] : &h->pinned[8];
    if (ntiles <= po::PS_SMALL_MAX) {
        PO_TRY(prefix_sum_small(h, A.tile_count + tile_begin, wide ? nullptr : A.tile_extra + tile_begin, ntiles,
                                tile_off_p + tile_begin, count_slot,
                                reinterpret_cast<const uint64_t*>(scalars + 2), also_slot, st, reinterpret_cast<uint64_t*>(scalars)));
    } else {
        PO_TRY(prefix_sum<uint32_t>(h, A.tile_count + tile_begin, ntiles, tile_off_p + tile_begin, count_slot,
                                    reinterpret_cast<const uint64_t*>(scalars + 2), also_slot,
                                    wide ? nullptr : A.tile_extra + tile_begin, st, reinterpret_cast<uint64_t*>(scalars)));
    }
    if (h->phase_events) HIP_TRY(h, hipEventRecord(h->ev[EV_COUNT], st));
    po::CandGuard G = {nullptr, 0u};
    uint64_t n_cand64;
    uint32_t n_selfrep_reads;
    if (async_count) {
        n_cand64 = cap_c;
        n_selfrep_reads = 0;
        S.n_predicted = 1;
        G.n_dev = scalars;
        G.cap = cap_c;
    } else {
        if (h->st_pend.valid && h->st_harvest) {
            HIP_TRY(h, hipEventSynchronize(h->st_pend.ev[EV_DONE]));
            PO_TRY(h->st_harvest());
        }
        HIP_TRY(h, hipStreamSynchronize(st));
        n_cand64 = h->pinned[1];
        n_selfrep_reads = (uint32_t)h->pinned[8];
    }
    if (nshards > 1 || streamed || wide || dpE) n_selfrep_reads |= 1u;
    S.n_candidates = n_cand64;
    if (n_cand64 >= 0xFFFFFF00ull)
        return fail(h, PO_ERR_CAPACITY, "candidate count " + std::to_string(n_cand64) + " exceeds one call's capacity (2^32)");
    const uint32_t n_cand = (uint32_t)n_cand64;

    uint64_t n_rows64 = 0;
    po::PairSlot* ptab = nullptr;
    uint32_t pbits = 0;
    uint32_t* n_deferred = reinterpret_cast<uint32_t*>(scalars + 1) + 1;
    const uint32_t* gate = nullptr;
    const uint64_t worst_rows = (uint64_t)n_cand * (paired ? 4u : 2u);
    std::function<po_status()> classic_tail;
    const bool sel_in_verify = (nshards > 1 || streamed || wide) && !dp && !getenv("PHASM_SELECT_KERNEL");
    if (n_cand) {
        PO_TRY(ensure_piece(h, h->d_cand_a, (size_t)n_cand * 4));
        PO_TRY(ensure_piece(h, h->d_cand_p, (size_t)n_cand * 4));
        PO_TRY(ensure_piece(h, h->d_cand_b, (size_t)n_cand * 4));
        PO_TRY(ensure_piece(h, h->d_type, (size_t)n_cand));
        PO_TRY(ensure_piece(h, h->d_rowcnt, (size_t)n_cand));
        PO_TRY(ensure_piece(h, h->d_row_off, ((size_t)n_cand + 1) * 4));
        A.cand_a = h->d_cand_a.as<uint32_t>();
        A.cand_p = h->d_cand_p.as<uint32_t>();
        A.cand_b = h->d_cand_b.as<uint32_t>();
        if (wide) {
            WA.cand_a = A.cand_a;
            WA.cand_p = A.cand_p;
            WA.cand_b = A.cand_b;
            auto wfill = streamed ? (ww == 4 ? po::k_wide_scan<BITS, true, BITS == 2, 4> : po::k_wide_scan<BITS, true, BITS == 2, 1>)
                         : ww == 16 ? po::k_wide_scan<BITS, true, false, 16> : ww == 4 ? po::k_wide_scan<BITS, true, false, 4> : po::k_wide_scan<BITS, true, false, 1>;
            hipLaunchKernelGGL(wfill, dim3(cdiv(ntiles, 4)), dim3(256), 0, st, WA, G);
        } else {
            auto fill = streamed ? po::k_scan_fill<BITS, BITS == 2> : po::k_scan_fill<BITS, false>;
            hipLaunchKernelGGL(fill, dim3(cdiv(ntiles, 4 * po::FILL_TILES)), dim3(256), 0, st, A, G);
        }
        const bool use_order_early = [&]() {
            bool u = n_cand >= 400000 && (r_end - r_begin) >= 4096;
            if (const char* e = getenv("PHASM_VERIFY_ORDER")) u = atoi(e) != 0;
            if (async_count) u = pred_order;
            return u && !dp;
        }();
        const bool defer_needed = streamed && r_end < n;
        if (defer_needed && !use_order_early) {
            hipLaunchKernelGGL(po::k_defer_split, dim3(cdiv(n_cand, 256)), dim3(256), 0, st, A.cand_a, A.cand_p, A.cand_b, n_cand,
                               r_end, h->d_defer.as<po::Cand>(), h->st_defer_cap, h->d_defer.as<uint32_t>() + (size_t)h->st_defer_cap * 4, G);
        }
        HIP_TRY(h, hipGetLastError());
        if (h->phase_events) HIP_TRY(h, hipEventRecord(h->ev[EV_FILL], st));
        if (dp) {
            if (2ull * h->max_len + 64ull >= (1ull << 30))
                return fail(h, PO_ERR_CAPACITY, "po_overlaps_ex: reads of 2^29 bases or more are beyond the DP kernel");
            PO_TRY(ensure(h, h->d_end_a, (size_t)n_cand * 4));
            PO_TRY(ensure(h, h->d_end_b, (size_t)n_cand * 4));
            PO_TRY(ensure(h, h->d_dpcnt, 64));
            HIP_TRY(h, hipMemsetAsync(h->d_dpcnt.p, 0, 64, st));
            po::ExtArgs X = {};
            X.words = words;
            X.woff = woff;
            X.len = len;
            X.cand_a = A.cand_a;
            X.cand_p = A.cand_p;
            X.cand_b = A.cand_b;
            X.n_cand = n_cand;
            X.max_diff = dpE;
            X.band = dpW;
            X.paired = paired;
            X.exc_off = h->n_exc_uploaded ? h->d_exc_off.as<uint32_t>() : nullptr;
            X.exc_pos = h->d_exc_pos.as<uint32_t>();
            X.exc_byte = h->d_exc_byte.as<uint8_t>();
            X.type = h->d_type.as<uint8_t>();
            X.end_a = h->d_end_a.as<uint32_t>();
            X.end_b = h->d_end_b.as<uint32_t>();
            X.counters = h->d_dpcnt.as<unsigned long long>();
            bool lanes = BITS == 2 && dpW <= 15;
            bool bitvec = lanes;
            if (const char* e = getenv("PHASM_DP_KERNEL")) {
                if (!strcmp(e, "wave")) lanes = bitvec = false;
                if (!strcmp(e, "lanes")) bitvec = false;
                if ((!strcmp(e, "lanes") || !strcmp(e, "bits")) && !(BITS == 2 && dpW <= 15))
                    return fail(h, PO_ERR_INVALID, "PHASM_DP_KERNEL=lanes|bits needs 2-bit reads and band <= 15");
            }
            if (const char* e = getenv("PHASM_DP_KERNEL_SOFT"))
                if (!strcmp(e, "lanes")) bitvec = false;
            S.dp_lanes = bitvec ? 2u : lanes ? 1u : 0u;
            if (h->pair_events) HIP_TRY(h, hipEventRecord(h->ev[EV_VER0], st));
            if (lanes) {
                const uint32_t* perm = nullptr;
                bool sorted = n_cand >= 4096;
                if (const char* e = getenv("PHASM_DP_SORT")) sorted = atoi(e) != 0;
                if (sorted) {
                    const uint32_t max_bins = (uint32_t)((std::min<size_t>(h->lds_max, 160 * 1024) - 1024) / 4);
                    const uint32_t max_rows = h->max_len + dpW;
                    uint32_t shift = 0;
                    while ((max_rows >> shift) + 1 > max_bins) ++shift;
                    const uint32_t n_bins = (max_rows >> shift) + 1;
                    const size_t sort_lds = ((size_t)n_bins + po::SORT_BLOCK / 64) * 4;
                    PO_TRY(ensure(h, h->d_vlabel, (size_t)n_cand * 4));
                    PO_TRY(ensure(h, h->d_vrank, (size_t)n_cand * 4));
                    PO_TRY(ensure(h, h->d_vperm, (size_t)n_cand * 4));
                    hipLaunchKernelGGL(po::k_dp_rows, dim3(cdiv(n_cand, 256)), dim3(256), 0, st, A.cand_a, A.cand_p, A.cand_b, len, n_cand,
                                       dpW, h->d_vlabel.as<uint32_t>());
                    if (sort_lds > 48 * 1024)
                        HIP_TRY(h, hipFuncSetAttribute(reinterpret_cast<const void*>(po::k_read_sort),
                                                       hipFuncAttributeMaxDynamicSharedMemorySize, (int)sort_lds));
                    hipLaunchKernelGGL(po::k_read_sort, dim3(1), dim3(po::SORT_BLOCK), sort_lds, st, h->d_vlabel.as<uint32_t>(), n_cand,
                                       shift, n_bins, h->d_vrank.as<uint32_t>());
                    hipLaunchKernelGGL(po::k_read_invert, dim3(cdiv(n_cand, 256)), dim3(256), 0, st, h->d_vrank.as<uint32_t>(), n_cand, 0u,
                                       h->d_vperm.as<uint32_t>());
                    perm = h->d_vperm.as<uint32_t>();
                }
                auto kern = bitvec ? po::k_extend_bits : dpW <= 4 ? po::k_extend_lanes<4> : dpW <= 8 ? po::k_extend_lanes<8> : po::k_extend_lanes<15>;
                hipLaunchKernelGGL(kern, dim3(cdiv(n_cand, 256)), dim3(256), 0, st, X, perm);
            } else {
                hipLaunchKernelGGL((po::k_extend_dp<BITS>), dim3(cdiv(n_cand, 256 / po::WAVE)), dim3(256), 0, st, X);
            }
            if (h->pair_events) HIP_TRY(h, hipEventRecord(h->ev[EV_VER1], st));
            HIP_TRY(h, hipMemcpyAsync(h->pinned + 32, h->d_dpcnt.p, 16, hipMemcpyDeviceToHost, st));
            ver_timed = true;
        } else {
            const uint64_t need_words = ((uint64_t)h->max_len + W - 1) / W + 3;
            const uint32_t lds_words_raw = (uint32_t)std::min<uint64_t>(need_words, 8192 - 1100);
            const uint32_t n_a = r_end - r_begin;
            const uint32_t* perm = nullptr;
            const bool use_order = use_order_early;
            if (use_order) {
                const uint32_t max_bins = (uint32_t)((std::min<size_t>(h->lds_max, 160 * 1024) - 1024) / 4);
                uint32_t shift = 0, n_bins;
                while ((n >> shift) + 1 > max_bins) ++shift;
                n_bins = (n >> shift) + 1;
                const size_t sort_lds = ((size_t)n_bins + po::SORT_BLOCK / 64) * 4;
                PO_TRY(ensure(h, h->d_vlabel, (size_t)n_a * 4));
                PO_TRY(ensure(h, h->d_vperm, (size_t)n_a * 4));
                po::DeferOut dfo = {};
                if (defer_needed) {
                    dfo.cand_p = A.cand_p;
                    dfo.b_limit = r_end;
                    dfo.list = h->d_defer.as<uint4>();
                    dfo.cap = h->st_defer_cap;
                    dfo.counter = h->d_defer.as<uint32_t>() + (size_t)h->st_defer_cap * 4;
                }
                hipLaunchKernelGGL(po::k_read_label, dim3(cdiv((uint64_t)n_a * 16, 256)), dim3(256), 0, st,
                                   h->d_read_tile0.as<uint32_t>(), tile_off_p, A.cand_b, r_begin, n_a, paired,
                                   h->d_vlabel.as<uint32_t>(), dfo, G);
                if (sort_lds > 48 * 1024)
                    HIP_TRY(h, hipFuncSetAttribute(reinterpret_cast<const void*>(po::k_read_sort),
                                                   hipFuncAttributeMaxDynamicSharedMemorySize, (int)sort_lds));
                PO_TRY(ensure(h, h->d_vrank, (size_t)n_a * 4));
                hipLaunchKernelGGL(po::k_read_sort, dim3(1), dim3(po::SORT_BLOCK), sort_lds, st, h->d_vlabel.as<uint32_t>(), n_a,
                                   shift, n_bins, h->d_vrank.as<uint32_t>());
                hipLaunchKernelGGL(po::k_read_invert, dim3(cdiv(n_a, 256)), dim3(256), 0, st, h->d_vrank.as<uint32_t>(), n_a, r_begin,
                                   h->d_vperm.as<uint32_t>());
                perm = h->d_vperm.as<uint32_t>();
            }
            const uint32_t ver_grid = perm ? 8 * ((n_a + 7) / 8) : n_a;
            bool staged = h->dev_words < 0xFFFFFFF0ull;
            if (const char* e = getenv("PHASM_VERIFY_STAGED")) staged = staged && atoi(e) != 0;
            auto verify = paired == 2u ? (staged ? po::k_verify_a<BITS, true, true> : po::k_verify_a<BITS, true, false>)
                                       : (staged ? po::k_verify_a<BITS, false, true> : po::k_verify_a<BITS, false, false>);
            if (streamed) verify = staged ? po::k_verify_a<BITS, false, true, BITS == 2> : po::k_verify_a<BITS, false, false, BITS == 2>;
            const uint32_t lds_words = (lds_words_raw + 1u) & ~1u;
            const size_t ver_lds = (size_t)lds_words * 8 + (size_t)po::VREC_CAP * sizeof(po::VRec) + 16;
            if (ver_lds > 48 * 1024)
                HIP_TRY(h, hipFuncSetAttribute(reinterpret_cast<const void*>(verify), hipFuncAttributeMaxDynamicSharedMemorySize, (int)ver_lds));
            if (h->pair_events) HIP_TRY(h, hipEventRecord(h->ev[EV_VER0], st));
            hipLaunchKernelGGL(verify, dim3(ver_grid), dim3(po::VER_BLOCK), ver_lds, st,
                               words, woff, len, h->d_read_tile0.as<uint32_t>(), tile_off_p, A.cand_p,
                               A.cand_b, r_begin, lds_words, paired_ver,
                               h->n_exc_uploaded ? h->d_exc_off.as<uint32_t>() : nullptr, h->d_exc_pos.as<uint32_t>(),
                               h->d_exc_byte.as<uint8_t>(), h->d_type.as<uint8_t>(), perm, n_a, G,
                               sel_in_verify ? selfrep : nullptr, sel_in_verify ? n_deferred : nullptr);
            if (h->pair_events) HIP_TRY(h, hipEventRecord(h->ev[EV_VER1], st));
            ver_timed = true;
        }
        HIP_TRY(h, hipGetLastError());
#ifdef PO_VSTAMPS
        {
            unsigned long long v[64 * 8], z[64 * 8] = {};
            HIP_TRY(h, hipStreamSynchronize(st));
            HIP_TRY(h, hipMemcpyFromSymbol(v, HIP_SYMBOL(po::g_vstamps), sizeof(v)));
            HIP_TRY(h, hipMemcpyToSymbol(HIP_SYMBOL(po::g_vstamps), z, sizeof(z)));
            double sum[8] = {};
            for (int i = 0; i < 64; ++i) for (int k = 0; k < 8; ++k) sum[k] += (double)v[i * 8 + k];
            if (sum[6] > 0)
                std::fprintf(stderr, "[vstamps] per wave (shader clocks): setup %.0f  wait_b %.0f  lds+cmp %.0f  book+init %.0f  life %.0f | iterations %.1f  group-steps/iteration %.2f  waves %.0f\n",
                             sum[0] / sum[6], sum[1] / sum[6], sum[2] / sum[6], sum[3] / sum[6], sum[4] / sum[6], sum[5] / sum[6], sum[7] / sum[5], sum[6]);
        }
#endif
        if (h->phase_events) HIP_TRY(h, hipEventRecord(h->ev[EV_VERIFY], st));
        if ((nshards > 1 || streamed || wide || dpE) && !sel_in_verify) {
            static_assert(po::SEL_CAP == 512, "k_select_local hashes to 9 bits");
            hipLaunchKernelGGL(po::k_select_local, dim3(cdiv(r_end - r_begin, 256 / po::WAVE)), dim3(256), 0, st,
                               h->d_read_tile0.as<uint32_t>(), tile_off_p, A.cand_p, A.cand_b, h->d_type.as<uint8_t>(),
                               r_begin, r_end - r_begin, selfrep, n_deferred, G);
        }
        const bool home_tail_ok = h->home_on && !want_cands && !dpE && !getenv("PHASM_TAIL_CLASSIC") &&
                                  (!n_selfrep_reads || ((nshards > 1 || streamed || wide) && n_cand < (16u << 20))) &&
                                  cdiv(n_cand, po::TAIL_TILE) <= po::TAIL_MAX_TILES;
        if (home_tail_ok && !async_count && h->spare_rows.cap < (size_t)n_cand * sizeof(po::Cand))
            PO_TRY(ensure(h, h->spare_rows, (size_t)n_cand * sizeof(po::Cand) + (streamed ? 65536 : 0), 1.0, false));
        const bool compact_tail = home_tail_ok && h->spare_rows.p && h->spare_rows.cap >= (size_t)n_cand * sizeof(po::Cand);
        const bool can_tail = compact_tail ||
                              (!want_cands && !dpE && h->spare_rows.p && h->spare_rows.cap >= worst_rows * sizeof(po_row) &&
                               (!n_selfrep_reads || ((nshards > 1 || streamed || wide) && n_cand < (16u << 20))) &&
                               cdiv(n_cand, po::TAIL_TILE) <= (streamed || h->home_on ? po::TAIL_MAX_TILES : 4096u) && !getenv("PHASM_TAIL_CLASSIC"));
        if (async_count && !can_tail) return fail(h, PO_ERR_HIP, "internal: a piece with a predicted candidate count needs the fused tail");
        classic_tail = [&]() -> po_status {
        if (n_selfrep_reads) {
            uint32_t n_sus;
            if ((nshards > 1 || streamed || wide) && n_cand < (4u << 20)) {
                n_sus = n_cand;
                gate = n_deferred;
            } else {
                uint32_t* n_suspect = reinterpret_cast<uint32_t*>(scalars + 2) + 1;
                hipLaunchKernelGGL(po::k_count_suspects, dim3(std::min<uint32_t>(cdiv(n_cand, 256), (uint32_t)h->n_cu * 8)), dim3(256), 0,
                                   st, A.cand_b, h->d_type.as<uint8_t>(), n_cand, selfrep, n_suspect);
                HIP_TRY(h, hipMemcpyAsync(h->pinned + 8, scalars + 2, 8, hipMemcpyDeviceToHost, st));
                HIP_TRY(h, hipStreamSynchronize(st));
                n_sus = (uint32_t)(h->pinned[8] >> 32);
            }
            if (n_sus) {
                pbits = 4;
                while ((1ull << pbits) < 2ull * n_sus) ++pbits;
                PO_TRY(ensure_piece(h, h->d_pair_key, ((size_t)1 << pbits) * sizeof(po::PairSlot)));
                hipLaunchKernelGGL(po::k_fill_gated, dim3((uint32_t)h->n_cu * 8), dim3(256), 0, st, h->d_pair_key.as<uint4>(),
                                   (uint64_t)((size_t)1 << pbits) * sizeof(po::PairSlot) / 16, 0xFFFFFFFFu, gate);
                ptab = h->d_pair_key.as<po::PairSlot>();
                hipLaunchKernelGGL(po::k_select_mark, dim3(cdiv(n_cand, 256)), dim3(256), 0, st, A.cand_a, A.cand_p, A.cand_b,
                                   h->d_type.as<uint8_t>(), n_cand, selfrep, ptab, pbits, gate);
            }
        }
        if (want_cands) PO_TRY(ensure(h, h->d_flag, (size_t)n_cand));
        hipLaunchKernelGGL(po::k_select, dim3(cdiv(n_cand, 256)), dim3(256), 0, st, A.cand_a, A.cand_p, A.cand_b,
                           h->d_type.as<uint8_t>(), n_cand, selfrep, ptab, pbits, paired, h->d_rowcnt.as<uint8_t>(),
                           want_cands ? h->d_flag.as<uint8_t>() : nullptr, gate);
        HIP_TRY(h, hipGetLastError());
        if (!want_cands) {
            PO_TRY(prefix_sum<uint8_t>(h, h->d_rowcnt.as<uint8_t>(), n_cand, h->d_row_off.as<uint32_t>(), &h->pinned[2]));
            if (h->phase_events) HIP_TRY(h, hipEventRecord(h->ev[EV_SELECT], st));
            rows_late = h->spare_rows.p && h->spare_rows.cap >= worst_rows * sizeof(po_row);
            if (!rows_late) {
                HIP_TRY(h, hipStreamSynchronize(st));
                n_rows64 = h->pinned[2];
                if (n_rows64 >= 0xFFFFFF00ull) return fail(h, PO_ERR_CAPACITY, "row count exceeds one call's capacity (2^32)");
            }
        }
        if (want_cands) {
            PO_TRY(prefix_sum<uint8_t>(h, h->d_flag.as<uint8_t>(), n_cand, h->d_row_off.as<uint32_t>(), &h->pinned[3]));
            if (h->phase_events) HIP_TRY(h, hipEventRecord(h->ev[EV_SELECT], st));
            po::Cand* dst;
            uint64_t dst_cap;
            if (res->ext_dst && res->ext_cap && !getenv("PHASM_COMPACT_SYNC")) {
                dst = static_cast<po::Cand*>(res->ext_dst);
                dst_cap = res->ext_cap;
                cands_late = true;
                cands_ext = true;
            } else if (h->spare_cands.p && h->spare_cands.cap >= (size_t)n_cand * sizeof(po::Cand) && !getenv("PHASM_COMPACT_SYNC")) {
                res->d_rows = h->spare_cands;
                h->spare_cands = DevBuf();
                dst = res->d_rows.as<po::Cand>();
                dst_cap = n_cand;
                cands_late = true;
            } else {
                HIP_TRY(h, hipStreamSynchronize(st));
                const uint64_t n_ver = h->pinned[3];
                if (res->ext_dst && n_ver <= res->ext_cap) {
                    dst = static_cast<po::Cand*>(res->ext_dst);
                    res->wrote_ext = true;
                } else {
                    if (h->spare_cands.p && h->spare_cands.cap >= n_ver * sizeof(po::Cand)) {
                        res->d_rows = h->spare_cands;
                        h->spare_cands = DevBuf();
                    }
                    PO_TRY(ensure(h, res->d_rows, std::max<size_t>(n_ver * sizeof(po::Cand), 256), 1.0, false));
                    dst = res->d_rows.as<po::Cand>();
                }
                dst_cap = n_ver;
                n_rows64 = n_ver;
            }
            cands_cap = dst_cap;
            hipLaunchKernelGGL(po::k_compact, dim3(cdiv(n_cand, 256)), dim3(256), 0, st, A.cand_a, A.cand_p, A.cand_b,
                               h->d_type.as<uint8_t>(), h->d_flag.as<uint8_t>(), h->d_row_off.as<uint32_t>(), n_cand, dst,
                               (uint32_t)std::min<uint64_t>(dst_cap, 0xFFFFFFFFull));
            HIP_TRY(h, hipGetLastError());
            res->elem = sizeof(po::Cand);
        } else {
            if (rows_late || (h->spare_rows.cap >= n_rows64 * sizeof(po_row) && h->spare_rows.p)) {
                res->d_rows = h->spare_rows;
                h->spare_rows = DevBuf();
            } else {
                h->spare_rows.release();
            }
            if (!rows_late) {
                const size_t exact = n_rows64 * sizeof(po_row);
                size_t roomy = worst_rows * sizeof(po_row) <= (2ull << 30) ? (size_t)(worst_rows * sizeof(po_row)) : 0;
                if (roomy && streamed) roomy += 4096 * sizeof(po_row);
                PO_TRY(ensure(h, res->d_rows, std::max<size_t>(std::max(exact, roomy), 256), 1.0, false));
            }
            if (dpE)
                hipLaunchKernelGGL(po::k_emit_ex, dim3(std::min<uint32_t>(cdiv(n_cand, 256), (uint32_t)h->n_cu * 16)), dim3(256), 0,
                                   st, A.cand_a, A.cand_p, A.cand_b, h->d_type.as<uint8_t>(), h->d_end_a.as<uint32_t>(),
                                   h->d_end_b.as<uint32_t>(), h->d_row_off.as<uint32_t>(), n_cand, len,
                                   res->d_rows.as<po::Row>(), (uint32_t)BITS, scalars + 4);
            else
            hipLaunchKernelGGL(po::k_emit, dim3(std::min<uint32_t>(cdiv(n_cand, 256), (uint32_t)h->n_cu * 16)), dim3(256), 0,
                               st, A.cand_a, A.cand_p, A.cand_b, h->d_type.as<uint8_t>(), h->d_row_off.as<uint32_t>(),
                               n_cand, len, res->d_rows.as<po::Row>(), (uint32_t)BITS, paired, scalars + 4);
            HIP_TRY(h, hipGetLastError());
        }
        return PO_OK;
        };
        if (can_tail) {
            const uint32_t n_tt = cdiv(n_cand, po::TAIL_TILE);
            if (((size_t)po::TAIL_MAX_TILES + 4) * 4 > h->d_tail_state.cap) {
                PO_TRY(ensure(h, h->d_tail_state, ((size_t)po::TAIL_MAX_TILES + 4) * 4));
                HIP_TRY(h, hipMemsetAsync(h->d_tail_state.p, 0, h->d_tail_state.cap, st));
            }
            uint32_t* tile_rows = h->d_tail_state.as<uint32_t>();
            uint32_t* tail_done = tile_rows + po::TAIL_MAX_TILES;
            const uint32_t* tgate = n_selfrep_reads ? n_deferred : nullptr;
            hipLaunchKernelGGL(compact_tail ? po::k_tile_rows<true> : po::k_tile_rows<false>, dim3(n_tt), dim3(po::TAIL_BLOCK), 0, st, A.cand_a,
                               A.cand_b, h->d_type.as<uint8_t>(), n_cand, paired, tgate, tile_rows, G);
            if (h->phase_events) HIP_TRY(h, hipEventRecord(h->ev[EV_SELECT], st));
            rows_late = true;
            used_tail = true;
            S.fused_tail = 1;
            res->d_rows = h->spare_rows;
            h->spare_rows = DevBuf();
            tail_zone = async_count ? zone : 48;
            h->pinned[tail_zone] = 0;
            h->pinned[tail_zone + 7] = 0;
            if (compact_tail) {
                res->compact = true;
                hipLaunchKernelGGL(po::k_tail_cands, dim3(n_tt), dim3(po::TAIL_BLOCK), 0, st, A.cand_a, A.cand_p, A.cand_b, h->d_type.as<uint8_t>(),
                                   n_cand, res->d_rows.as<po::Cand>(), paired, tgate, tile_rows, n_tt, tail_done,
                                   scalars + 3, h->pinned_dev + tail_zone, G, h->home_sh_b, h->home_sh_p);
            } else
            hipLaunchKernelGGL(po::k_tail, dim3(n_tt), dim3(po::TAIL_BLOCK), 0, st, A.cand_a, A.cand_p, A.cand_b, h->d_type.as<uint8_t>(),
                               n_cand, len, res->d_rows.as<po::Row>(), (uint32_t)BITS, paired, tgate, tile_rows, n_tt, tail_done,
                               scalars + 4, h->pinned_dev + tail_zone, G);
            HIP_TRY(h, hipGetLastError());
        } else {
            PO_TRY(classic_tail());
        }
        tail_fallback = [&]() -> po_status {
            h->spare_rows = res->d_rows;
            res->d_rows = DevBuf();
            res->compact = false;
            rows_late = false;
            used_tail = false;
            S.fused_tail = 0;
            S.tail_fallback = 1;
            PO_TRY(classic_tail());
// ... 1457 lines not shown
    const bool ftrace = getenv("PHASM_FASTA_TRACE") != nullptr;
    const auto ft0 = std::chrono::steady_clock::now();
    auto fmark = [&](const char* what) {
        if (ftrace) std::fprintf(stderr, "[fasta] %s at %.1f ms\n", what, std::chrono::duration<double, std::milli>(std::chrono::steady_clock::now() - ft0).count());
    };
    g_reg_defer = true;
    try {
        h->words[0].resize(cur[0]);
        h->words[1].resize(cur[1]);
    } catch (...) {
        g_reg_defer = false;
        throw;
    }
    g_reg_defer = false;
    fmark("stores sized");
    uint64_t* words[2] = {h->words[0].data(), h->words[1].data()};
    std::thread reg_thread;
    try {
        uint64_t* blocks[2] = {h->words[0].capacity() ? words[0] : nullptr, h->words[1].capacity() ? words[1] : nullptr};
        reg_thread = std::thread([blocks, &fmark] {
            for (int k = 0; k < 2; ++k)
                if (blocks[k]) RegAlloc<uint64_t>::reg_now(blocks[k]);
            fmark("stores registered");
        });
    } catch (const std::system_error&) {
    }
    struct RegJoin {
        std::thread& t;
        po_handle* h;
        ~RegJoin() {
            if (t.joinable()) t.join();
            else
                for (int k = 0; k < 2; ++k)
                    if (h->words[k].capacity()) RegAlloc<uint64_t>::reg_now(h->words[k].data());
        }
    } reg_join{reg_thread, h};
    const uint8_t* lut = g_lut.v;
    const unsigned char* comp = comp_table();
    std::atomic<size_t> next{0};
    std::atomic<int> bad{0};
    auto pack = [&](const unsigned char* sq, size_t n, uint64_t* w) -> uint8_t {
        uint8_t b = 0;
        const size_t full = n / 32;
        for (size_t k = 0; k < full; ++k) {
            const unsigned char* q = sq + k * 32;
            uint64_t acc = 0;
            for (int j = 0; j < 32; ++j) {
                const uint8_t c = lut[q[j]];
                b |= c;
                acc |= (uint64_t)(c & 3) << (2 * j);
            }
            w[k] = acc;
        }
        if (full * 32 < n) {
            uint64_t acc = 0;
            for (size_t i = full * 32; i < n; ++i) {
                const uint8_t c = lut[sq[i]];
                b |= c;
                acc |= (uint64_t)(c & 3) << (2 * (i & 31));
            }
            w[full] = acc;
        }
        return b;
    };
    auto worker = [&]() {
      try {
        std::string seq, rc;
        for (;;) {
            const size_t lo = next.fetch_add(64);
            if (lo >= recs.size() || bad.load(std::memory_order_relaxed)) return;
            const size_t hi = std::min(recs.size(), lo + 64);
            for (size_t i = lo; i < hi; ++i) {
                const FastaRec& r = recs[i];
                seq.clear();
                seq.reserve(r.seq_len);
                for (const char* p = r.seq_begin; p < r.seq_end;) {
                    const char* nl = static_cast<const char*>(std::memchr(p, '\n', (size_t)(r.seq_end - p)));
                    size_t n = nl ? (size_t)(nl - p) + 1 : (size_t)(r.seq_end - p);
                    const char* q = p;
                    size_t m = n;
                    trim_seq_line(q, m);
                    seq.append(q, m);
                    p += n;
                }
                const size_t n = seq.size();
                if (n != r.seq_len) {
                    bad.store(1);
                    return;
                }
                rc.resize(n);
                for (size_t k = 0; k < n; ++k) rc[k] = (char)comp[(unsigned char)seq[n - 1 - k]];
                const size_t nw = (n + 31) / 32;
                for (int k = 0; k < 2; ++k) {
                    const size_t prev_end = i ? off[2 * (i - 1) + k] + (recs[i - 1].seq_len + 31) / 32 + 1 : old_words[k];
                    if (off[2 * i + k] > prev_end) words[k][off[2 * i + k] - 1] = 0;
                    words[k][off[2 * i + k] + nw] = 0;
                }
                uint8_t b = pack(reinterpret_cast<const unsigned char*>(seq.data()), n, words[0] + off[2 * i]);
                b |= pack(reinterpret_cast<const unsigned char*>(rc.data()), n, words[1] + off[2 * i + 1]);
                if (n != r.seq_len || (b & 0x80)) {
                    bad.store(1);
                    return;
                }
            }
        }
      } catch (...) {
        bad.store(1);
      }
    };
    {
        const unsigned hw = std::max(1u, cpu_share() > 3 ? cpu_share() - 2 : cpu_share());
        const unsigned n_thr = std::max(1u, std::min(hw, 16u));
        std::vector<std::thread> thr;
        try {
            for (unsigned t = 1; t < n_thr; ++t) thr.emplace_back(worker);
        } catch (const std::system_error&) {
        }
        worker();
        for (auto& th : thr) th.join();
    }
    fmark("packed");
    if (bad.load()) {
        h->words[0].resize(old_words[0]);
        h->words[1].resize(old_words[1]);
        return false;
    }
    h->ids.reserve(h->ids.size() + 2 * recs.size());
    for (size_t i = 0; i < recs.size(); ++i) {
        std::string id(recs[i].name, recs[i].name_len);
        id.push_back('+');
        h->ids.push_back(id);
        id.back() = '-';
        h->ids.push_back(std::move(id));
        for (int k = 0; k < 2; ++k) {
            h->len.push_back((uint32_t)recs[i].seq_len);
            h->woff.push_back(off[2 * i + k]);
            h->exc_off.push_back((uint32_t)h->exc_pos.size());
        }
        h->total_bases += 2 * recs[i].seq_len;
    }
    h->dirty = true;
    h->ids_paired = -1;
    if (n_records) *n_records = recs.size();
    fmark("ids and tables appended");
    return true;
}

}

extern "C" {

int po_abi_version(void) { return PO_ABI_VERSION; }

po_status po_create(po_handle** out) {
    if (!out) return PO_ERR_INVALID;
    po_handle* h = new (std::nothrow) po_handle();
    if (!h) return PO_ERR_NOMEM;
    *out = h;
    return PO_OK;
}

void po_destroy(po_handle* h) {
    if (!h) return;
    if (h->dev_ready) {
        (void)hipSetDevice(h->device);
        (void)hipStreamSynchronize(h->stream);
        DevBuf* bufs[] = {&h->d_words, &h->d_woff, &h->d_len, &h->d_tiles, &h->d_read_tile0, &h->d_left, &h->d_left_cnt, &h->d_tile_extra, &h->d_exc_off, &h->d_exc_pos, &h->d_exc_byte, &h->d_pair_state, &h->d_truemask,
                          &h->d_table, &h->d_slot_cnt, &h->d_slot_cur, &h->d_slot_start, &h->d_read_slot, &h->d_chain,
                          &h->d_chain_tmp, &h->d_long_list, &h->d_entry_off, &h->d_bloom, &h->d_selfrep, &h->d_tile_count, &h->d_tile_off,
                          &h->d_ps_blocks, &h->d_scalars, &h->d_cand_a, &h->d_cand_p, &h->d_cand_b, &h->d_type,
                          &h->d_rowcnt, &h->d_row_off, &h->d_flag, &h->d_pair_key, &h->d_pair_min, &h->spare_rows, &h->spare_cands, &h->spare_edges, &h->spare_nrank,
                          &h->d_vlabel, &h->d_vrank, &h->d_vperm, &h->d_end_a, &h->d_end_b, &h->d_dpcnt, &h->d_lay_len, &h->d_lay_cnt, &h->d_rflag, &h->d_removed, &h->d_ekey, &h->d_ecnt,
                          &h->d_ewin, &h->d_eoff, &h->d_chain_state, &h->d_tail_state, &h->d_efirst, &h->d_lay_firstc};
        if (h->copy_stream) (void)hipStreamSynchronize(h->copy_stream);
        if (h->up_stream) (void)hipStreamSynchronize(h->up_stream);
        if (h->rc_stream) (void)hipStreamSynchronize(h->rc_stream);
        for (DevBuf* b : bufs) b->release();
        for (DevBuf& b : h->d_red) b.release();
        for (DevBuf& b : h->d_tip) b.release();
        for (DevBuf& b : h->d_mrg) b.release();
        for (DevBuf& b : h->d_cov) b.release();
        for (DevBuf& b : h->d_rank) b.release();
        for (DevBuf& b : h->d_cc) b.release();
        for (DevBuf& b : h->d_scc) b.release();
        const bool pooled = kit_give(h);
        if (!pooled) {
        for (int i = 0; i < 2 * EV_N; ++i) (void)hipEventDestroy(h->ev_sets[i / EV_N][i % EV_N]);
        for (hipEvent_t e : h->ev_lay)
            if (e) (void)hipEventDestroy(e);
        (void)hipEventDestroy(h->ev_up0);
        (void)hipEventDestroy(h->ev_up1);
        if (h->pinned) {
            pin_drop(h->pinned);
            (void)hipHostFree(h->pinned);
        }
        }
        h->spare_host.release();
        h->scratch_host.release();
        h->home_stage.release();
        for (DevBuf& b : h->chunk_rows) b.release();
        h->d_first.release();
        h->d_defer.release();
        h->meta_host.release();
        h->stage_host.release();
        for (void* c : h->arena_chunks) (void)hipFree(c);
        h->arena_chunks.clear();
        if (!pooled) {
        if (h->up_stream) {
            (void)hipStreamSynchronize(h->up_stream);
            (void)hipStreamDestroy(h->up_stream);
        }
        for (hipEvent_t e : h->ev_piece)
            if (e) (void)hipEventDestroy(e);
        for (hipEvent_t e : h->ev_rc)
            if (e) (void)hipEventDestroy(e);
        if (h->ev_meta) (void)hipEventDestroy(h->ev_meta);
        if (h->rc_stream) {
            (void)hipStreamSynchronize(h->rc_stream);
            (void)hipStreamDestroy(h->rc_stream);
        }
        if (h->ev_first) (void)hipEventDestroy(h->ev_first);
        if (h->copy_stream) {
            (void)hipStreamSynchronize(h->copy_stream);
            (void)hipStreamDestroy(h->copy_stream);
        }
        (void)hipStreamDestroy(h->stream);
        }
    }
    h->spare_host.release();
    h->home_stage.release();
    delete h;
}

po_status po_set_device(po_handle* h, int device) {
    if (!h) return PO_ERR_INVALID;
    if (h->dev_ready && device != h->device) return fail(h, PO_ERR_INVALID, "device already initialised");
    h->device = device;
    return PO_OK;
}

po_status po_add_sequence(po_handle* h, const char* id, size_t id_len, const char* seq, size_t seq_len) {
    if (!h || (!id && id_len) || (!seq && seq_len)) return PO_ERR_INVALID;
    if (h->segments_only) return fail(h, PO_ERR_INVALID, "this handle holds GFA segments (no sequences); use a new handle");
    if (seq_len > 0x7FFFFFF0ull) return fail(h, PO_ERR_CAPACITY, "read longer than 2^31 bases");
    if (h->len.size() >= 0xFFFFFFF0ull) return fail(h, PO_ERR_CAPACITY, "too many reads");
    quiesce_store(h);
    try {
        const unsigned char* s = reinterpret_cast<const unsigned char*>(seq);
        if (h->bits != 2 || !append_packed(h, s, seq_len, 2)) {
            if (h->bits == 2) widen_to_bytes(h);
            append_packed(h, s, seq_len, 8);
        }
        h->ids.emplace_back(id ? id : "", id_len);
        h->len.push_back((uint32_t)seq_len);
        h->total_bases += seq_len;
        h->dirty = true;
        h->ids_paired = -1;
        if (h->total_bases >= h->pool_bases && h->total_bases >= (64ull << 20)) result_pool_grow(h);
        if (h->bits == 2 && h->first_n + 1 == h->len.size()) note_first_words(h);
        if (h->bits == 2 && (h->len.size() & 1) == 0) {
            const size_t r = h->len.size() - 1;
            if (!h->exc_pos.empty()) host_pair_check(h, r, s);
            const bool has_exc = h->exc_off[r - 1] != h->exc_off[r] || h->exc_off[r] != h->exc_off[r + 1];
            if (h->all_pairs_rcx) {
                const bool ok = has_exc ? (h->pair_state.size() > r / 2 && h->pair_state[r / 2] == 1) : packed_is_revcomp(h, r);
                h->all_pairs_rcx = ok;
                if (has_exc || !ok) h->all_pairs_rc = false;
            } else {
                h->all_pairs_rc = false;
            }
        }
    } catch (const std::bad_alloc&) {
        return fail(h, PO_ERR_NOMEM, "out of host memory in po_add_sequence");
    }
    return PO_OK;
}

po_status po_add_fasta(po_handle* h, const char* path, int both_strands, uint64_t* n_records) {
    if (!h || !path) return PO_ERR_INVALID;
    if (n_records) *n_records = 0;
    quiesce_store(h);
    if (both_strands && !h->segments_only && !getenv("PHASM_FASTA_SEQUENTIAL")) {
        const int fd = ::open(path, O_RDONLY);
        if (fd < 0) return fail(h, PO_ERR_INVALID, std::string("cannot open ") + path);
        struct stat sb;
        bool done = false;
        if (::fstat(fd, &sb) == 0 && sb.st_size > 0) {
            void* m = ::mmap(nullptr, (size_t)sb.st_size, PROT_READ, MAP_PRIVATE, fd, 0);
            if (m != MAP_FAILED) {
                std::thread warm;
                if ((uint64_t)sb.st_size >= (32ull << 20) && !h->dev_ready && !getenv("PHASM_NO_POOL") && !getenv("PHASM_NO_WARM")) {
                    const uint64_t est_bases = 2ull * (uint64_t)sb.st_size;
                    try {
                        warm = std::thread([h, est_bases] {
                            if (h->total_bases + est_bases >= h->pool_bases) result_pool_grow(h, h->total_bases + est_bases);
                        });
                    } catch (const std::system_error&) {
                    }
                }
                struct Joiner {
                    std::thread& t;
                    ~Joiner() {
                        if (t.joinable()) t.join();
                    }
                } joiner{warm};
                try {
                    const auto tf0 = std::chrono::steady_clock::now();
                    done = add_fasta_parallel(h, static_cast<const char*>(m), (size_t)sb.st_size, n_records);
                    if (getenv("PHASM_FASTA_TRACE")) {
                        const double t_parse = std::chrono::duration<double, std::milli>(std::chrono::steady_clock::now() - tf0).count();
                        if (warm.joinable()) warm.join();
                        std::fprintf(stderr, "[fasta] parsed and packed in %.1f ms; the device and the result pool were ready %.1f ms after the start\n", t_parse,
                                     std::chrono::duration<double, std::milli>(std::chrono::steady_clock::now() - tf0).count());
                    }
                } catch (const std::bad_alloc&) {
                    ::munmap(m, (size_t)sb.st_size);
                    ::close(fd);
                    return fail(h, PO_ERR_NOMEM, "out of host memory in po_add_fasta");
                } catch (const std::system_error&) {
                    done = false;
                }
                ::munmap(m, (size_t)sb.st_size);
            }
        }
        ::close(fd);
        if (done) {
            if (h->total_bases >= h->pool_bases && h->total_bases >= (64ull << 20)) result_pool_grow(h);
            if (h->bits == 2) note_first_words(h);
            return PO_OK;
        }
    }
    FILE* f = std::fopen(path, "rb");
    if (!f) return fail(h, PO_ERR_INVALID, std::string("cannot open ") + path);
    const unsigned char* comp = comp_table();
    po_status st = PO_OK;
    uint64_t nrec = 0;
    try {
        std::string name, seq, rc, line;
        bool have = false;
        std::vector<char> buf(1 << 22);
        auto flush_record = [&]() -> po_status {
            if (!have) return PO_OK;
            ++nrec;
            if (!both_strands) return po_add_sequence(h, name.data(), name.size(), seq.data(), seq.size());
            std::string id = name + "+";
            po_status s1 = po_add_sequence(h, id.data(), id.size(), seq.data(), seq.size());
            if (s1 != PO_OK) return s1;
            rc.resize(seq.size());
            for (size_t i = 0, n = seq.size(); i < n; ++i) rc[i] = (char)comp[(unsigned char)seq[n - 1 - i]];
            id.back() = '-';
            return po_add_sequence(h, id.data(), id.size(), rc.data(), rc.size());
        };
        auto handle_line = [&](const char* p, size_t n) -> po_status {
            while (n && (p[n - 1] == '\r' || p[n - 1] == '\n')) --n;
            if (n == 0) return PO_OK;
            if (p[0] == '>') {
                po_status s1 = flush_record();
                if (s1 != PO_OK) return s1;
                name.assign(p + 1, n - 1);
                seq.clear();
                have = true;
            } else if (have) {
                while (n && (p[n - 1] == ' ' || p[n - 1] == '\t')) --n;
                size_t b = 0;
                while (b < n && (p[b] == ' ' || p[b] == '\t')) ++b;
                seq.append(p + b, n - b);
            }
            return PO_OK;
        };
        size_t got;
        while (st == PO_OK && (got = std::fread(buf.data(), 1, buf.size(), f)) > 0) {
            size_t pos = 0;
            while (pos < got && st == PO_OK) {
                const char* nl = static_cast<const char*>(std::memchr(buf.data() + pos, '\n', got - pos));
                if (!nl) {
                    line.append(buf.data() + pos, got - pos);
                    pos = got;
                } else {
                    const size_t len = (size_t)(nl - (buf.data() + pos)) + 1;
                    if (line.empty()) {
                        st = handle_line(buf.data() + pos, len);
                    } else {
                        line.append(buf.data() + pos, len);
                        st = handle_line(line.data(), line.size());
                        line.clear();
                    }
                    pos += len;
                }
            }
        }
        if (st == PO_OK && !line.empty()) st = handle_line(line.data(), line.size());
        if (st == PO_OK) st = flush_record();
    } catch (const std::bad_alloc&) {
        st = fail(h, PO_ERR_NOMEM, "out of host memory in po_add_fasta");
    }
    std::fclose(f);
    if (n_records) *n_records = nrec;
    return st;
}

uint32_t po_num_sequences(const po_handle* h) { return h ? (uint32_t)h->len.size() : 0; }

po_status po_get_id(const po_handle* h, uint32_t idx, const char** id, size_t* id_len) {
    if (!h || idx >= h->ids.size() || !id || !id_len) return PO_ERR_INVALID;
    *id = h->ids[idx].data();
    *id_len = h->ids[idx].size();
    return PO_OK;
}

uint32_t po_get_length(const po_handle* h, uint32_t idx) { return (h && idx < h->len.size()) ? h->len[idx] : 0; }

po_status po_upload(po_handle* h) {
    if (!h) return PO_ERR_INVALID;
    po_status st;
    try {
        st = upload(h);
    } catch (const std::bad_alloc&) {
        st = fail(h, PO_ERR_NOMEM, "out of host memory in po_upload");
    }
    if (st != PO_OK && h->dev_ready) (void)hipStreamSynchronize(h->stream);
    return st;
}

po_status po_upload_piece_part(po_handle* h, uint32_t shard, uint32_t nshards, uint32_t part, uint32_t nparts, void* dst_device,
                               uint64_t capacity_words, uint64_t* word_count, int* ok) {
    if (!h || !word_count || !ok || nshards == 0 || shard >= nshards || nparts == 0 || part >= nparts || nparts > 64) return PO_ERR_INVALID;
    *ok = 0;
    *word_count = 0;
    const uint32_t n = (uint32_t)h->len.size();
    if (!(h->bits == 2 && n >= 2 && (n % 2) == 0 && h->all_pairs_rc && h->exc_pos.empty()) || h->segments_only) return PO_OK;
    PO_TRY(init_device(h));
    uint64_t wb = 0, wc = 0;
    try {
        store0_part_range(h, shard, nshards, part, nparts, &wb, &wc);
    } catch (const std::bad_alloc&) {
        return fail(h, PO_ERR_NOMEM, "out of host memory");
    }
    *word_count = wc;
    *ok = 1;
    if (!dst_device) return PO_OK;
    if (wc > capacity_words) return fail(h, PO_ERR_INVALID, "po_upload_piece: the piece does not fit the destination");
    if (wc) {
        const void* src = h->words[0].data() + wb;
        if (!store_is_pinned(h->words[0]) && wc * 8 <= STAGE_MAX) {
            h->stage_used = 0;
            PO_TRY(ensure_host(h, h->stage_host, wc * 8 + 64));
            src = staged(h, src, wc * 8);
        }
        HIP_TRY(h, hipMemcpyAsync(dst_device, src, wc * 8, hipMemcpyHostToDevice, h->stream));
    }
    HIP_TRY(h, hipStreamSynchronize(h->stream));
    h->upload_bytes = (part == 0 ? 0 : h->upload_bytes) + wc * 8;
    return PO_OK;
}

po_status po_upload_piece(po_handle* h, uint32_t shard, uint32_t nshards, void* dst_device, uint64_t capacity_words,
                          uint64_t* word_count, int* ok) {
    return po_upload_piece_part(h, shard, nshards, 0, 1, dst_device, capacity_words, word_count, ok);
}

po_status po_upload_assemble_parts(po_handle* h, const void* pieces_device, uint64_t slot_words, uint32_t nshards, uint32_t nparts) {
    if (!h || !pieces_device || nshards == 0 || nparts == 0 || nparts > 64) return PO_ERR_INVALID;
    h->asm_pieces = static_cast<const uint64_t*>(pieces_device);
    h->asm_slot_words = slot_words;
    h->asm_n = nshards;
    h->asm_parts = nparts;
    h->dirty = true;
    const uint64_t piece_bytes = h->upload_bytes;
    po_status st;
    try {
        st = upload(h);
    } catch (const std::bad_alloc&) {
        st = fail(h, PO_ERR_NOMEM, "out of host memory in po_upload_assemble");
    }
    h->asm_pieces = nullptr;
    h->asm_parts = 1;
    if (st != PO_OK && h->dev_ready) (void)hipStreamSynchronize(h->stream);
    if (st == PO_OK) {
        h->upload_bytes += piece_bytes;
        h->stats.upload_bytes = h->upload_bytes;
// ... 121 lines not shown
    const bool pack = !(pk && atoi(pk) == 0);
    h->home_sh_b = pack ? h->home_pack_b : 0u;
    h->home_sh_p = pack ? h->home_pack_p : 0u;
    return true;
}

void home_wait(po_handle* h) {
    if (h->home_on) home::wait_all(home::g_pool);
}

int home_end(po_handle* h, po_stats* sum = nullptr) {
    if (!h->home_on) return 0;
    home::Pool* P = home::g_pool;
    home::wait_all(P);
    const int err = P->error.load();
    if (sum) {
        sum->sum_overlap_bases += P->sum_l.load();
        sum->verify_bytes_algo += P->sum_b.load();
        sum->verify_bytes_exec += P->sum_e.load();
    }
    if (P->tracing)
        for (size_t i = 0; i < P->trace.size(); ++i)
            std::fprintf(stderr, "[home] piece %zu: records home at %.3f ms, %.0f rows written at %.3f ms (since the call set the pool up)\n", i,
                         P->trace[i][0] * 1e-3, P->trace[i][2], P->trace[i][1] * 1e-3);
    h->home_on = false;
    P->call_mu.unlock();
    return err;
}

po_status rows_room(po_handle* h, HostRows& R, uint64_t nk, uint32_t k, uint32_t n_chunks, double seen_share) {
    const size_t need = (size_t)(R.total + nk) * sizeof(po_row);
    if (need <= R.hb.cap) return PO_OK;
    uint64_t guess = std::max<uint64_t>(h->last_host_rows, (R.total + nk) * n_chunks / (k + 1));
    if (seen_share > 0.0) guess = std::max<uint64_t>(guess, (uint64_t)((double)(R.total + nk) / seen_share * 1.05));
    HostBuf bigger;
    PO_TRY(ensure_host(h, bigger, std::max<size_t>(need, (size_t)(guess + guess / 8) * sizeof(po_row))));
    home_wait(h);
    if (hipStreamSynchronize(h->copy_stream) != hipSuccess) {
        bigger.release();
        return fail(h, PO_ERR_HIP, "copy stream");
    }
    if (R.total) std::memcpy(bigger.p, R.hb.p, (size_t)R.total * sizeof(po_row));
    R.hb.release();
    R.hb = bigger;
    return PO_OK;
}

po_status append_home(po_handle* h, HostRows& R, const DevBuf& dev, uint64_t n_rec, uint64_t nk, uint32_t k, uint32_t n_chunks,
                      double seen_share = 0.0) {
    if (nk == 0) return PO_OK;
    home::Pool* P = home::g_pool;
    PO_TRY(rows_room(h, R, nk, k, n_chunks, seen_share));
    const size_t elem = h->home_sh_b ? sizeof(uint64_t) : sizeof(po::Cand);
    const size_t bytes = (size_t)n_rec * elem;
    constexpr uint64_t N_EV = 32;
    if (h->home_used + bytes > h->home_stage.cap || (h->home_seq && h->home_seq % N_EV == 0)) {
        home_wait(h);
        if (hipStreamSynchronize(h->copy_stream) != hipSuccess) return fail(h, PO_ERR_HIP, "copy stream");
        h->home_used = 0;
        if (bytes > h->home_stage.cap)
            PO_TRY(ensure_host(h, h->home_stage, std::max<size_t>({bytes * 2, (size_t)(h->home_last_bytes + h->home_last_bytes / 8), (size_t)8 << 20})));
    }
    const uint32_t slot = (uint32_t)(h->home_seq % N_EV);
    const uint32_t want = ++h->home_gen;
    char* dst = static_cast<char*>(h->home_stage.p) + h->home_used;
    HIP_TRY(h, hipMemcpyAsync(dst, dev.p, bytes, hipMemcpyDeviceToHost, h->copy_stream));
    hipLaunchKernelGGL(po::k_fill_u32, dim3(1), dim3(64), 0, h->copy_stream, reinterpret_cast<uint32_t*>(h->pinned_dev + 96 + slot), (uint64_t)1, want);
    HIP_TRY(h, hipGetLastError());
    home::Job j;
    j.rec = dst;
    j.sh_b = h->home_sh_b;
    j.sh_p = h->home_sh_p;
    j.n_rec = n_rec;
    j.out = static_cast<po_row*>(R.hb.p) + R.total;
    j.n_rows = nk;
    j.flag = reinterpret_cast<const volatile uint32_t*>(h->pinned + 96 + slot);
    j.want = want;
    j.paired = (h->bits == 2 && h->paired) ? 1u : 0u;
    j.bits = (uint32_t)h->bits;
    home::submit(P, j);
    ++h->home_seq;
    h->home_used += (bytes + 255) & ~size_t(255);
    h->home_last_bytes += bytes;
    R.total += nk;
    return PO_OK;
}

po_status append_rows(po_handle* h, HostRows& R, const DevBuf& dev, uint64_t nk, uint32_t k, uint32_t n_chunks, double seen_share = 0.0) {
    if (nk == 0) return PO_OK;
    PO_TRY(rows_room(h, R, nk, k, n_chunks, seen_share));
    HIP_TRY(h, hipMemcpyAsync(static_cast<char*>(R.hb.p) + (size_t)R.total * sizeof(po_row), dev.p, (size_t)nk * sizeof(po_row),
                              hipMemcpyDeviceToHost, h->copy_stream));
    R.total += nk;
    return PO_OK;
}

void add_stats(po_stats& sum, const po_stats& S) {
    sum.n_candidates += S.n_candidates;
    sum.n_verified += S.n_verified;
    sum.n_rows += S.n_rows;
    sum.sum_overlap_bases += S.sum_overlap_bases;
    sum.verify_bytes_algo += S.verify_bytes_algo;
    sum.verify_bytes_exec += S.verify_bytes_exec;
    sum.n_tiles += S.n_tiles;
    sum.shard_bases += S.shard_bases;
    sum.fused_tail += S.fused_tail;
    sum.tail_fallback += S.tail_fallback;
    sum.n_predicted += S.n_predicted;
    sum.ms_index += S.ms_index;
    sum.ms_scan_count += S.ms_scan_count;
    sum.ms_scan_fill += S.ms_scan_fill;
    sum.ms_verify += S.ms_verify;
    sum.ms_select += S.ms_select;
    sum.ms_emit += S.ms_emit;
    sum.ms_total += S.ms_total;
    sum.ms_scan_probe += S.ms_scan_probe;
    sum.ms_verify_kernel += S.ms_verify_kernel;
}

po_status run_chunk(po_handle* h, uint32_t min_length, uint32_t k, uint32_t n_chunks, uint64_t* nk) {
    po_result part;
    part.h = h;
    if (h->chunk_rows[k].p) {
        h->spare_rows.release();
        h->spare_rows = h->chunk_rows[k];
        h->chunk_rows[k] = DevBuf();
    }
    const po_status st = h->bits == 2 ? run_overlaps<2>(h, min_length, k, n_chunks, false, &part)
                                      : run_overlaps<8>(h, min_length, k, n_chunks, false, &part);
    h->chunk_rows[k] = part.d_rows;
    h->chunk_compact[k] = part.compact;
    part.d_rows = DevBuf();
    *nk = part.count;
    return st;
}

bool stream_eligible(const po_handle* h, uint32_t min_length) {
    const uint32_t n = (uint32_t)h->len.size();
    if (!h->dirty || h->bits != 2 || n < 4 || (n % 2) != 0 || !h->all_pairs_rcx) return false;
    if (h->asm_pieces || h->ex_on || h->sl_build_n > 1 || h->ext_index) return false;
    if (getenv("PHASM_FULL_UPLOAD") || getenv("PHASM_NO_MIRROR")) return false;
    bool want = n >= 4096 && h->words[0].size() * 8 >= (16ull << 20);
    if (const char* e = getenv("PHASM_STREAM")) want = atoi(e) != 0;
    if (!want) return false;
    const uint32_t m = min_length ? min_length : 1;
    const uint64_t n_elig = count_eligible(const_cast<po_handle*>(h), m);
    if (n_elig == 0) return false;
    return true;
}

std::vector<uint32_t> stream_bounds(const po_handle* h) {
    const uint32_t n = (uint32_t)h->len.size();
    const uint64_t bytes0 = (uint64_t)h->words[0].size() * 8;
    uint64_t max_pieces = h->chunk_rows[0].p ? 12 : 8;
    const bool big = bytes0 >= (512ull << 20) && h->chunk_rows[0].p;
    if (big) max_pieces = 15;
    if (const char* e = getenv("PHASM_STREAM_MAX_PIECES")) max_pieces = (uint64_t)std::max(2, std::min(PO_MAX_PIECES - 1, atoi(e)));
    const uint32_t n_pieces = (uint32_t)std::min<uint64_t>(max_pieces, std::max<uint64_t>(2, (bytes0 + (8ull << 20)) / (16ull << 20)));
    const double skew = big ? 1.6 : 1.25;
    std::vector<uint32_t> cuts;
    for (uint32_t i = 1; i < n_pieces; ++i) cuts.push_back((uint32_t)(1000.0 * (1.0 - std::pow(1.0 - (double)i / n_pieces, skew))));
    if (const char* e = getenv("PHASM_STREAM_CUTS")) {
        cuts.clear();
        for (const char* q = e; *q;) {
            char* endp = nullptr;
            const long v = strtol(q, &endp, 10);
            if (endp == q) break;
            if (v > 0 && v < 1000 && (cuts.empty() || (uint32_t)v > cuts.back()) && cuts.size() + 1 < (size_t)PO_MAX_PIECES) cuts.push_back((uint32_t)v);
            q = *endp ? endp + 1 : endp;
        }
    }
    std::vector<uint32_t> b{0};
    const uint64_t total = h->words[0].size();
    for (uint32_t c : cuts) {
        const uint64_t target = total * c / 1000;
        uint32_t lo = 0, hi = n / 2;
        while (lo < hi) {
            const uint32_t mid = (lo + hi) / 2;
            if (h->woff[2 * (size_t)mid] >= target) hi = mid; else lo = mid + 1;
        }
        if (2 * lo > b.back() && 2 * lo < n) b.push_back(2 * lo);
    }
    b.push_back(n);
    return b;
}

po_status stream_begin(po_handle* h, const std::vector<uint32_t>& bounds) {
    const uint32_t n = (uint32_t)h->len.size();
    const uint32_t P = (uint32_t)bounds.size() - 1;
    bool generate = false;
    if (!h->up_stream) HIP_TRY(h, hipStreamCreateWithFlags(&h->up_stream, hipStreamNonBlocking));
    for (uint32_t k = 0; k < P; ++k)
        if (!h->ev_piece[k]) HIP_TRY(h, hipEventCreate(&h->ev_piece[k]));
    auto queue_piece = [&](uint32_t k) -> po_status {
        uint64_t* dw = h->d_words.as<uint64_t>();
        const uint64_t wb = bounds[k] < n ? h->woff[bounds[k]] : h->words[0].size();
        const uint64_t we = bounds[k + 1] < n ? h->woff[bounds[k + 1]] : h->words[0].size();
        if (we > wb) {
            HIP_TRY(h, hipMemcpyAsync(dw + wb, h->words[0].data() + wb, (we - wb) * 8, hipMemcpyHostToDevice, h->up_stream));
            h->upload_bytes += (we - wb) * 8;
        }
        HIP_TRY(h, hipEventRecord(h->ev_piece[k], h->up_stream));
        return PO_OK;
    };
    PO_TRY(upload_meta(h, &generate));
    if (!generate) return fail(h, PO_ERR_INVALID, "streamed step on reads that are not (x, reverse complement of x) pairs");
    uint64_t* dw = h->d_words.as<uint64_t>();
    if (h->poison >= 0) {
        HIP_TRY(h, hipEventRecord(h->ev_up1, h->stream));
        HIP_TRY(h, hipStreamWaitEvent(h->up_stream, h->ev_up1, 0));
    }
    HIP_TRY(h, hipEventRecord(h->ev_up0, h->up_stream));
    PO_TRY(queue_piece(0));
    if (P > 1) {
        const uint32_t r0 = h->st_early_index ? 0u : bounds[1];
        if (h->st_lead > 2) {
            note_lead_words(h);
            PO_TRY(ensure(h, h->d_first, (size_t)n * LEAD_WORDS * 8));
            HIP_TRY(h, hipMemcpyAsync(h->d_first.as<uint64_t>() + (size_t)LEAD_WORDS * r0, h->lead_words.data() + (size_t)LEAD_WORDS * r0,
                                      (size_t)(n - r0) * LEAD_WORDS * 8, hipMemcpyHostToDevice, h->stream));
            h->upload_bytes += (size_t)(n - r0) * LEAD_WORDS * 8;
            hipLaunchKernelGGL(po::k_scatter_lead, dim3(cdiv((uint64_t)(n - r0) * LEAD_WORDS, 256)), dim3(256), 0, h->stream, dw,
                               h->d_woff.as<uint64_t>(), h->d_len.as<uint32_t>(), h->d_first.as<uint64_t>(), LEAD_WORDS, r0, n);
        } else {
            note_first_words(h);
            PO_TRY(ensure(h, h->d_first, (size_t)n * 16));
            HIP_TRY(h, hipMemcpyAsync(h->d_first.as<uint64_t>() + 2 * (size_t)r0, h->first_words.data() + 2 * (size_t)r0,
                                      (size_t)(n - r0) * 16, hipMemcpyHostToDevice, h->stream));
            h->upload_bytes += (size_t)(n - r0) * 16;
            hipLaunchKernelGGL(po::k_scatter_first, dim3(cdiv(n - r0, 256)), dim3(256), 0, h->stream, dw, h->d_woff.as<uint64_t>(),
                               h->d_first.as<ulonglong2>(), r0, n);
        }
        HIP_TRY(h, hipGetLastError());
        if (!h->ev_first) HIP_TRY(h, hipEventCreateWithFlags(&h->ev_first, hipEventDisableTiming));
        HIP_TRY(h, hipEventRecord(h->ev_first, h->stream));
        HIP_TRY(h, hipStreamWaitEvent(h->up_stream, h->ev_first, 0));
    }
    for (uint32_t k = 1; k < P; ++k) PO_TRY(queue_piece(k));
    HIP_TRY(h, hipEventRecord(h->ev_up1, h->up_stream));
    if (!h->rc_stream) HIP_TRY(h, hipStreamCreateWithFlags(&h->rc_stream, hipStreamNonBlocking));
    if (!h->ev_meta) HIP_TRY(h, hipEventCreateWithFlags(&h->ev_meta, hipEventDisableTiming));
    HIP_TRY(h, hipEventRecord(h->ev_meta, h->stream));
    HIP_TRY(h, hipStreamWaitEvent(h->rc_stream, h->ev_meta, 0));
    for (uint32_t k = 0; k < P; ++k) {
        if (!h->ev_rc[k]) HIP_TRY(h, hipEventCreateWithFlags(&h->ev_rc[k], hipEventDisableTiming));
        HIP_TRY(h, hipStreamWaitEvent(h->rc_stream, h->ev_piece[k], 0));
        const uint32_t p0 = bounds[k] / 2, p1 = bounds[k + 1] / 2;
        if (p1 > p0)
            hipLaunchKernelGGL(po::k_revcomp_store, dim3(cdiv((uint64_t)(p1 - p0) * 64, 256)), dim3(256), 0, h->rc_stream, dw,
                               h->d_woff.as<uint64_t>(), h->d_len.as<uint32_t>(), p0, p1,
                               h->n_exc_uploaded ? h->d_exc_off.as<uint32_t>() : nullptr, h->d_exc_pos.as<uint32_t>());
        HIP_TRY(h, hipGetLastError());
        HIP_TRY(h, hipEventRecord(h->ev_rc[k], h->rc_stream));
    }
    h->st_defer_cap = std::max<uint32_t>(1u << 16, h->defer_need + h->defer_need / 2);
    if (const char* e = getenv("PHASM_DEFER_CAP")) h->st_defer_cap = (uint32_t)std::max(1, atoi(e));
    PO_TRY(ensure(h, h->d_defer, (size_t)h->st_defer_cap * sizeof(po::Cand) + 16));
    if (!getenv("PHASM_DEFER_CAP")) h->st_defer_cap = (uint32_t)std::min<size_t>((h->d_defer.cap - 16) / sizeof(po::Cand), 0xFFFFFF00u);
    HIP_TRY(h, hipMemsetAsync(h->d_defer.as<char>() + (size_t)h->st_defer_cap * sizeof(po::Cand), 0, 16, h->stream));
    h->paired = true;
    ++h->upload_gen;
    h->dirty = false;
    return PO_OK;
}

po_status overlaps_streamed(po_handle* h, uint32_t min_length, HostRows& R, po_stats& sum, bool* overflow) {
    *overflow = false;
    const uint32_t n = (uint32_t)h->len.size();
    const std::vector<uint32_t> bounds = stream_bounds(h);
    const uint32_t P = (uint32_t)bounds.size() - 1;
    const bool trace = getenv("PHASM_STREAM_TRACE") != nullptr;
    const auto t_start = std::chrono::steady_clock::now();
    auto since = [&]() { return std::chrono::duration<double, std::milli>(std::chrono::steady_clock::now() - t_start).count(); };
    std::vector<uint32_t> sig(bounds);
    sig.push_back(min_length);
    sig.push_back((uint32_t)(h->total_bases & 0xFFFFFFFFu));
    h->st_pred_valid = h->st_pred_valid && sig == h->st_pred_sig;
    uint64_t new_pred[PO_MAX_PIECES] = {};
    h->st_selfclean = false;
    h->st_early_index = P > 1 && h->poison < 0 && !getenv("PHASM_NO_INDEX_REUSE") && !getenv("PHASM_LATE_INDEX");
    {
        const uint32_t m = min_length ? min_length : 1;
        const char* idx = getenv("PHASM_INDEX");
        const char* win = getenv("PHASM_WIDE_WINDOW");
        const bool wide = (idx && !strcmp(idx, "wide")) || (!(idx && !strcmp(idx, "narrow")) && count_eligible(h, m) > 160000);
        h->st_lead = (h->bits == 2 && wide && m >= 32u * 4u + 31u && !(win && atoi(win) < 4) && !getenv("PHASM_STREAM_LEAD2")) ? LEAD_WORDS : 2u;
    }
    PO_TRY(stream_begin(h, bounds));
    if (trace) std::fprintf(stderr, "[stream] %u pieces queued at %.3f ms\n", P, since());
    if (h->st_early_index) {
        po_result part;
        part.h = h;
        h->st_on = true;
        h->st_r_begin = bounds[0];
        h->st_r_end = bounds[1];
        h->idx_only = true;
        const po_status ist = run_overlaps<2>(h, min_length, 0, P, false, &part);
        h->idx_only = false;
        h->st_on = false;
        part.d_rows.release();
        if (ist != PO_OK) {
            (void)hipStreamSynchronize(h->stream);
            (void)hipStreamSynchronize(h->up_stream);
            (void)hipStreamSynchronize(h->rc_stream);
            h->dirty = true;
            return ist;
        }
    }
    uint64_t* dw = h->d_words.as<uint64_t>();
    po_status st = PO_OK;
    auto completed = [&](uint32_t k, const po_stats& S, uint64_t nk) -> po_status {
        add_stats(sum, S);
        new_pred[k] = S.n_candidates;
        const double seen = (double)bounds[k + 1] / (double)n;
        if (h->chunk_compact[k]) PO_TRY(append_home(h, R, h->chunk_rows[k], S.n_verified, nk, k, P, seen * seen));
        else PO_TRY(append_rows(h, R, h->chunk_rows[k], nk, k, P, seen * seen));
        if (trace) {
            float up = 0;
            (void)hipEventElapsedTime(&up, h->ev_up0, h->ev_piece[k]);
            std::fprintf(stderr, "[stream] piece %u reads [%u, %u): landed %.3f ms after the first copy started, rows counted at %.3f ms (device %.3f ms: scan %.3f verify %.3f), %llu rows (%.1f MB) queued for home\n",
                         k, bounds[k], bounds[k + 1], up, since(), S.ms_total, S.ms_scan_count + S.ms_scan_fill, S.ms_verify,
                         (unsigned long long)nk, nk * 24e-6);
        }
        return PO_OK;
    };
    h->st_pend.valid = false;
    bool tail_gave_up = false;
    h->st_harvest = [&]() -> po_status {
        const uint32_t k = h->st_pend.k;
        bool needs_classic = false;
        const uint64_t nk = finish_piece(h, &needs_classic);
        if (needs_classic) {
            tail_gave_up = true;
            return PO_OK;
        }
        return completed(k, h->st_pend.S, nk);
    };
    if (getenv("PHASM_STREAM_SYNC")) h->st_harvest = nullptr;
    for (uint32_t k = 0; k < P && st == PO_OK; ++k) {
        if (hipStreamWaitEvent(h->stream, h->ev_rc[k], 0) != hipSuccess) { st = fail(h, PO_ERR_HIP, "hipStreamWaitEvent"); break; }
        h->st_on = true;
        h->st_r_begin = bounds[k];
        h->st_r_end = bounds[k + 1];
        h->ws_scale = 1.0;
        {
            const double mine = (double)bounds[k + 1] * bounds[k + 1] - (double)bounds[k] * bounds[k];
            for (uint32_t j = k + 1; j < P; ++j)
                h->ws_scale = std::max(h->ws_scale, ((double)bounds[j + 1] * bounds[j + 1] - (double)bounds[j] * bounds[j]) / mine * 1.1);
        }
        h->ev = h->ev_sets[k & 1];
        uint64_t nk = 0;
        st = run_chunk(h, min_length, k, P, &nk);
        h->st_on = false;
        h->ws_scale = 1.0;
        if (st != PO_OK || tail_gave_up) break;
        if (h->st_pend.valid && h->st_pend.k == k) continue;
        if (h->st_pend.valid) {
            if (hipStreamSynchronize(h->stream) != hipSuccess) { st = fail(h, PO_ERR_HIP, "stream"); break; }
            st = h->st_harvest();
            if (st != PO_OK) break;
        }
        st = completed(k, h->stats, nk);
    }
    if (st == PO_OK && h->st_pend.valid && !tail_gave_up) {
        if (hipStreamSynchronize(h->stream) != hipSuccess) st = fail(h, PO_ERR_HIP, "stream");
        else st = h->st_harvest();
    }
    h->st_harvest = nullptr;
    h->st_pend.valid = false;
    h->ev = h->ev_sets[0];
    if (st == PO_OK && tail_gave_up) {
        (void)hipStreamSynchronize(h->stream);
        (void)hipStreamSynchronize(h->up_stream);
        (void)hipStreamSynchronize(h->rc_stream);
        h->dirty = true;
        h->st_tail_gave_up = true;
        h->st_pred_valid = false;
        *overflow = true;
        return PO_OK;
    }
    if (st != PO_OK) {
        (void)hipStreamSynchronize(h->up_stream);
        (void)hipStreamSynchronize(h->rc_stream);
        h->dirty = true;
        h->st_pred_valid = false;
        return st;
    }
    h->st_pred_sig = sig;
    std::memcpy(h->st_pred_cand, new_pred, sizeof(new_pred));
    h->st_pred_valid = true;
    float ms = 0;
    (void)hipEventSynchronize(h->ev_up1);
    (void)hipEventElapsedTime(&ms, h->ev_up0, h->ev_up1);
    h->stats.ms_upload = ms;
    HIP_TRY(h, hipMemcpyAsync(h->pinned + 40, h->d_defer.as<char>() + (size_t)h->st_defer_cap * sizeof(po::Cand), 8,
                              hipMemcpyDeviceToHost, h->stream));
    HIP_TRY(h, hipStreamSynchronize(h->stream));
    const uint32_t n_def = (uint32_t)h->pinned[40];
    h->defer_need = n_def;
    if (n_def > h->st_defer_cap) {
        *overflow = true;
        return PO_OK;
    }
    if (n_def) {
        hipStream_t s = h->stream;
        po::Cand* list = h->d_defer.as<po::Cand>();
        PO_TRY(ensure(h, h->d_rowcnt, (size_t)n_def));
        PO_TRY(ensure(h, h->d_row_off, ((size_t)n_def + 1) * 4));
        HIP_TRY(h, hipEventRecord(h->ev[EV_START], s));
        hipLaunchKernelGGL(po::k_verify_flat, dim3(cdiv((uint64_t)n_def * 64, 256)), dim3(256), 0, s, dw, h->d_woff.as<uint64_t>(),
                           h->d_len.as<uint32_t>(), list, n_def, h->n_exc_uploaded ? h->d_exc_off.as<uint32_t>() : nullptr,
                           h->d_exc_pos.as<uint32_t>(), h->d_exc_byte.as<uint8_t>());
        hipLaunchKernelGGL(po::k_deferred_rowcnt, dim3(cdiv(n_def, 256)), dim3(256), 0, s, list, n_def, 1u, h->d_rowcnt.as<uint8_t>());
        HIP_TRY(h, hipGetLastError());
        PO_TRY(prefix_sum<uint8_t>(h, h->d_rowcnt.as<uint8_t>(), n_def, h->d_row_off.as<uint32_t>(), &h->pinned[2]));
        HIP_TRY(h, hipStreamSynchronize(s));
        const uint64_t n_rows = h->pinned[2];
        if (n_rows) {
            PO_TRY(ensure(h, h->chunk_rows[P], n_rows * sizeof(po_row)));
            unsigned long long* scalars = h->d_scalars.as<unsigned long long>();
            HIP_TRY(h, hipMemsetAsync(scalars + 4, 0, 32, s));
            hipLaunchKernelGGL(po::k_emit_cands, dim3(std::min<uint32_t>(cdiv(n_def, 256), (uint32_t)h->n_cu * 16)), dim3(256), 0, s,
                               list, h->d_rowcnt.as<uint8_t>(), h->d_row_off.as<uint32_t>(), n_def, h->d_len.as<uint32_t>(),
                               h->chunk_rows[P].as<po::Row>(), 2u, 1u, scalars + 4);
            HIP_TRY(h, hipGetLastError());
            HIP_TRY(h, hipMemcpyAsync(h->pinned + 4, scalars + 4, 4 * sizeof(uint64_t), hipMemcpyDeviceToHost, s));
            HIP_TRY(h, hipEventRecord(h->ev[EV_EMIT], s));
            HIP_TRY(h, hipStreamSynchronize(s));
            float ms_def = 0;
            (void)hipEventElapsedTime(&ms_def, h->ev[EV_START], h->ev[EV_EMIT]);
            sum.n_verified += h->pinned[4];
            sum.sum_overlap_bases += h->pinned[5];
            sum.verify_bytes_algo += h->pinned[6];
            sum.verify_bytes_exec += h->pinned[7];
            sum.n_rows += n_rows;
            sum.ms_verify += ms_def;
            sum.ms_total += ms_def;
            PO_TRY(append_rows(h, R, h->chunk_rows[P], n_rows, P, P + 1));
        }
    }
    (void)n;
    if (trace) {
        std::fprintf(stderr, "[stream] deferred list settled at %.3f ms (%u candidates)\n", since(), n_def);
        (void)hipStreamSynchronize(h->copy_stream);
        std::fprintf(stderr, "[stream] last row home at %.3f ms\n", since());
    }
    return PO_OK;
}

}
}

po_status po_overlaps_to_host(po_handle* h, uint32_t min_length, po_result** out) {
    if (!h || !out) return PO_ERR_INVALID;
    *out = nullptr;
    if (h->segments_only) return fail(h, PO_ERR_INVALID, "this handle holds GFA segments without sequences: nothing to overlap");
    uint32_t n_chunks = (h->len.size() >= 8192 && h->total_bases >= (64ull << 20)) ? 4u : 1u;
    if (const char* e = getenv("PHASM_HOST_CHUNKS")) n_chunks = (uint32_t)std::max(1, std::min(4, atoi(e)));
    po_result* r = new (std::nothrow) po_result();
    if (!r) return fail(h, PO_ERR_NOMEM, "out of host memory");
    r->h = h;
    po_status st = PO_OK;
    HostRows R;
    po_stats sum = {};
    bool streamed = false, overflowed = false;
    float ms_upload = 0;
    try {
        st = init_device(h);
        if (st == PO_OK && !h->copy_stream && hipStreamCreateWithFlags(&h->copy_stream, hipStreamNonBlocking) != hipSuccess)
            st = fail(h, PO_ERR_HIP, "cannot create the copy stream");
        if (st == PO_OK && h->spare_host.p) {
            R.hb = h->spare_host;
            h->spare_host = HostBuf();
        }
        if (st == PO_OK) {
            (void)home_begin(h);
            h->home_last_bytes = 0;
        }
        if (st == PO_OK && stream_eligible(h, min_length)) {
            bool overflow = false;
            st = overlaps_streamed(h, min_length, R, sum, &overflow);
            ms_upload = h->stats.ms_upload;
            if (st == PO_OK && !overflow) {
                streamed = true;
            } else if (st == PO_OK) {
                overflowed = true;
                home_wait(h);
                if (h->home_on) {
                    home::g_pool->sum_l.store(0);
                    home::g_pool->sum_b.store(0);
                    home::g_pool->sum_e.store(0);
                }
                if (hipStreamSynchronize(h->copy_stream) != hipSuccess) st = fail(h, PO_ERR_HIP, "copy stream");
                R.total = 0;
                sum = po_stats();
            }
        }
        if (st == PO_OK && !streamed) st = upload(h);
        for (uint32_t k = 0; k < n_chunks && st == PO_OK && !streamed; ++k) {
            uint64_t nk = 0;
            st = run_chunk(h, min_length, k, n_chunks, &nk);
            if (st != PO_OK) break;
            add_stats(sum, h->stats);
            st = h->chunk_compact[k] ? append_home(h, R, h->chunk_rows[k], h->stats.n_verified, nk, k, n_chunks)
                                     : append_rows(h, R, h->chunk_rows[k], nk, k, n_chunks);
        }
    } catch (const std::bad_alloc&) {
        st = fail(h, PO_ERR_NOMEM, "out of host memory in po_overlaps_to_host");
    }
    h->st_on = false;
    h->st_harvest = nullptr;
    h->st_pend.valid = false;
    h->ev = h->ev_sets[0];
    if (h->dev_ready) (void)hipStreamSynchronize(h->stream);
    if (h->up_stream) (void)hipStreamSynchronize(h->up_stream);
    if (h->rc_stream) (void)hipStreamSynchronize(h->rc_stream);
    if (h->copy_stream && hipStreamSynchronize(h->copy_stream) != hipSuccess && st == PO_OK) st = fail(h, PO_ERR_HIP, "row copy device->host");
    {
        const int herr = home_end(h, &sum);
        if (herr && st == PO_OK)
            st = fail(h, PO_ERR_HIP, herr == 1 ? "internal: the host's row count of a piece differs from the device's"
                                     : herr == 2 ? "internal: a verified-candidate record names a read the handle does not hold"
                                                 : "the event behind a device->host copy of records failed");
    }
    if (st != PO_OK) {
        R.hb.release();
        delete r;
        return st;
    }
    po_stats& S = h->stats;
    S.n_candidates = sum.n_candidates;
    S.n_verified = sum.n_verified;
    S.n_rows = sum.n_rows;
    S.sum_overlap_bases = sum.sum_overlap_bases;
    S.verify_bytes_algo = sum.verify_bytes_algo;
    S.verify_bytes_exec = sum.verify_bytes_exec;
    S.n_tiles = sum.n_tiles;
    S.shard_bases = sum.shard_bases;
    S.ms_index = sum.ms_index;
    S.ms_scan_count = sum.ms_scan_count;
    S.ms_scan_fill = sum.ms_scan_fill;
    S.ms_verify = sum.ms_verify;
    S.ms_select = sum.ms_select;
    S.ms_emit = sum.ms_emit;
    S.ms_total = sum.ms_total;
    S.ms_scan_probe = sum.ms_scan_probe;
    S.ms_verify_kernel = sum.ms_verify_kernel;
    S.fused_tail = sum.fused_tail;
    S.n_predicted = sum.n_predicted;
    S.home_record_bytes = h->home_last_bytes ? (h->home_sh_b ? 8u : 16u) : 0u;
    S.tail_fallback = sum.tail_fallback + (h->st_tail_gave_up ? 1u : 0u);
    h->st_tail_gave_up = false;
    S.streamed = streamed ? 1u : 0u;
    S.n_deferred = (streamed || overflowed) ? h->defer_need : 0u;
    if (streamed) {
        S.ms_upload = ms_upload;
        S.upload_bytes = h->upload_bytes;
    }
    h->last_host_rows = R.total;
    r->count = R.total;
    r->unique_twins = h->bits == 2 && h->paired;
    if (R.total) {
        r->host = R.hb.p;
        r->host_cap = R.hb.cap;
    } else if (R.hb.p) {
        h->spare_host = R.hb;
    }
    ++h->live_results;
    *out = r;
    return PO_OK;
}

po_status po_index_slice_build(po_handle* h, uint32_t min_length, uint32_t slice, uint32_t n_slices, uint32_t* is_wide,
                               uint32_t* slice_bits, uint64_t* chain_entries) {
    if (!h || !is_wide || !slice_bits || !chain_entries) return PO_ERR_INVALID;
    if (n_slices < 2 || slice >= n_slices) return fail(h, PO_ERR_INVALID, "po_index_slice_build: need 2 or more slices and slice < n_slices");
    *is_wide = 0;
    *slice_bits = 0;
    *chain_entries = 0;
    h->sl_build_slice = slice;
    h->sl_build_n = n_slices;
    h->sl_is_wide = false;
    po_result* r = nullptr;
    const po_status st = overlaps_common(h, min_length, 0, 1, false, &r);
    h->sl_build_n = 0;
    if (r) po_result_free(r);
    if (st != PO_OK) return st;
    *is_wide = h->sl_is_wide ? 1u : 0u;
    if (h->sl_is_wide) {
        *slice_bits = h->sl_tbits;
        *chain_entries = h->sl_entries;
    }
    return PO_OK;
}

static bool slice_args_ok(uint32_t n_slices, uint32_t slice_bits, uint64_t chain_capacity) {
    return n_slices >= 2 && n_slices <= 4096 && slice_bits >= 1 && slice_bits <= 30 && chain_capacity < (1ull << 36);
}

uint64_t po_index_chunk_bytes(uint32_t slice_bits, uint64_t chain_capacity, uint64_t* chain_offset_bytes) {
    if (chain_offset_bytes) *chain_offset_bytes = 0;
    if (slice_bits < 1 || slice_bits > 30 || chain_capacity >= (1ull << 36)) return 0;
    const uint64_t off = ((((1ull << slice_bits) + 1ull) * sizeof(po::Slot)) + 255ull) & ~255ull;
    if (chain_offset_bytes) *chain_offset_bytes = off;
    return (off + chain_capacity * 8ull + 255ull) & ~255ull;
}

po_status po_index_slice_export(po_handle* h, void* dst_device, uint64_t chain_capacity) {
    if (!h || !dst_device) return PO_ERR_INVALID;
    if (!h->sl_is_wide || !h->dev_ready) return fail(h, PO_ERR_INVALID, "po_index_slice_export: no sub-table has been built on this handle");
    if (chain_capacity < h->sl_entries) return fail(h, PO_ERR_INVALID, "po_index_slice_export: chain capacity below this sub-table's entries");
    uint64_t off = 0;
    (void)po_index_chunk_bytes(h->sl_tbits, chain_capacity, &off);
    HIP_TRY(h, hipSetDevice(h->device));
    HIP_TRY(h, hipMemcpyAsync(dst_device, h->d_table.p, ((size_t)(1ull << h->sl_tbits) + 1) * sizeof(po::Slot), hipMemcpyDeviceToDevice, h->stream));
    if (h->sl_entries)
        HIP_TRY(h, hipMemcpyAsync(static_cast<char*>(dst_device) + off, h->d_chain.p, (size_t)h->sl_entries * 8, hipMemcpyDeviceToDevice, h->stream));
    HIP_TRY(h, hipStreamSynchronize(h->stream));
    return PO_OK;
}

po_status po_candidates_shard_indexed(po_handle* h, uint32_t min_length, uint32_t shard, uint32_t nshards,
                                      const void* index_device, uint32_t n_slices, uint32_t slice_bits, uint64_t chain_capacity,
                                      void* dst_device, uint64_t capacity, int* written, po_result** out) {
    if (written) *written = 0;
    if (!h || !out || !index_device) return PO_ERR_INVALID;
    if (!slice_args_ok(n_slices, slice_bits, chain_capacity))
        return fail(h, PO_ERR_INVALID, "sliced index: need 2..4096 slices of 2^1..2^30 slots (slice_bits as po_index_slice_build reported it)");
    if (!dst_device && capacity) return PO_ERR_INVALID;
    uint64_t off = 0;
    const uint64_t chunk = po_index_chunk_bytes(slice_bits, chain_capacity, &off);
    if ((chunk / 16) * n_slices >= 0xFFFFFFF0ull) return fail(h, PO_ERR_CAPACITY, "sliced index larger than 64 GB");
    h->ext_index = index_device;
    h->ext_slices = n_slices;
    h->ext_tbits = slice_bits;
    h->ext_chunk_slots = (uint32_t)(chunk / 16);
    h->ext_chain_off = (uint32_t)(off / 16);
    const po_status st = overlaps_common(h, min_length, shard, nshards, true, out, dst_device, capacity);
    h->ext_index = nullptr;
    if (st == PO_OK && written) *written = (*out)->wrote_ext ? 1 : 0;
    return st;
}

po_status po_overlaps_shard_indexed(po_handle* h, uint32_t min_length, uint32_t shard, uint32_t nshards, const void* index_device,
                                    uint32_t n_slices, uint32_t slice_bits, uint64_t chain_capacity, po_result** out) {
    if (!h || !out || !index_device) return PO_ERR_INVALID;
    if (!slice_args_ok(n_slices, slice_bits, chain_capacity))
        return fail(h, PO_ERR_INVALID, "sliced index: need 2..4096 slices of 2^1..2^30 slots (slice_bits as po_index_slice_build reported it)");
    uint64_t off = 0;
    const uint64_t chunk = po_index_chunk_bytes(slice_bits, chain_capacity, &off);
    if ((chunk / 16) * n_slices >= 0xFFFFFFF0ull) return fail(h, PO_ERR_CAPACITY, "sliced index larger than 64 GB");
    h->ext_index = index_device;
    h->ext_slices = n_slices;
    h->ext_tbits = slice_bits;
    h->ext_chunk_slots = (uint32_t)(chunk / 16);
    h->ext_chain_off = (uint32_t)(off / 16);
    const po_status st = overlaps_common(h, min_length, shard, nshards, false, out);
    h->ext_index = nullptr;
    return st;
}

po_status po_overlaps_ex(po_handle* h, uint32_t min_length, uint32_t max_diff, uint32_t band, po_result** out) {
    if (!h || !out) return PO_ERR_INVALID;
// ... 836 lines not shown
```

phasm_amd/overlapper.py:

```python
from __future__ import annotations

import ctypes
import os
from typing import List, Optional, Tuple

import numpy as np

from . import _lib
from ._lib import CAND_DTYPE, EDGE_DTYPE, ROW_DTYPE, PoLayoutParams, PoLayoutStats, PoNodeOrderStats, PoReduceParams, PoReduceStats, PoStats, PoTipsParams, PoTipsStats, PoDiamondParams, PoDiamondStats, PoMergeParams, PoMergeStats, PoCoverageParams, PoCoverageStats, COVERAGE_DTYPE, PoComponentsParams, PoComponentsStats, COMPONENT_DTYPE, PoPartitionParams, PoPartitionStats, SCC_DTYPE

OverlapT = Tuple[str, str, int, int, int, int]

_PYT = [False, None]


def _pytuples():
    if not _PYT[0]:
        _PYT[0] = True
        path = os.path.join(os.path.dirname(os.path.abspath(__file__)), "_pytuples.so")
        if os.path.exists(path) and not os.environ.get("PHASM_NO_PYTUPLES"):
            try:
                lib = ctypes.PyDLL(path)
                lib.po_rows_to_tuples.restype = ctypes.py_object
                lib.po_rows_to_tuples.argtypes = [ctypes.c_void_p, ctypes.c_uint64, ctypes.py_object]
# ... 302 lines not shown
        _check(self._h, self._lib.po_add_segment(self._h, b, len(b), int(length)))

    def add_gfa(self, path: str) -> Tuple[int, OverlapResult]:
        n = ctypes.c_uint64()
        r = ctypes.c_void_p()
        _check(self._h, self._lib.po_add_gfa(self._h, os.fsencode(path), ctypes.byref(n), ctypes.byref(r)))
        return int(n.value), OverlapResult(self, r)

    def result_from_rows(self, rows: np.ndarray) -> OverlapResult:
        if rows.dtype != ROW_DTYPE:
            arr = np.asarray(rows)
            out = np.empty(len(arr), dtype=ROW_DTYPE)
            for k, name in enumerate(ROW_DTYPE.names):
                out[name] = arr[:, k]
            rows = out
        rows = np.ascontiguousarray(rows)
        r = ctypes.c_void_p()
        _check(self._h, self._lib.po_result_from_rows(self._h, rows.ctypes.data_as(ctypes.c_void_p), len(rows), ctypes.byref(r)))
        return OverlapResult(self, r)

    def layout_edges(self, rows: OverlapResult, min_read_length: int = 0, min_overlap_length: int = 0,
                     max_overhang_abs: int = 1000, max_overhang_rel: float = 0.8,
                     want_removed: bool = True) -> Tuple[OverlapResult, Optional[np.ndarray]]:
        prm = PoLayoutParams(int(min_read_length), int(min_overlap_length), int(max_overhang_abs), 0, float(max_overhang_rel))
        removed = np.zeros(len(self) // 2, dtype=np.uint8) if want_removed else None
        r = ctypes.c_void_p()
        _check(self._h, self._lib.po_layout_edges(
            self._h, rows._ptr, ctypes.byref(prm),
            removed.ctypes.data_as(ctypes.c_void_p) if removed is not None and len(removed) else None, ctypes.byref(r)))
        return OverlapResult(self, r, EDGE_DTYPE), removed

    def _edge_stage(self, fn, edges: OverlapResult, prm, want_flags: bool):
        flags = np.zeros(len(edges), dtype=np.uint8) if want_flags else None
        r = ctypes.c_void_p()
        _check(self._h, fn(self._h, edges._ptr, ctypes.byref(prm),
                           flags.ctypes.data_as(ctypes.c_void_p) if flags is not None and len(flags) else None, ctypes.byref(r)))
        kept = OverlapResult(self, r, EDGE_DTYPE)
        return (kept, flags) if want_flags else kept

    def _stats(self, fn, struct) -> dict:
        s = struct()
        _check(self._h, fn(self._h, ctypes.byref(s)))
        return s.as_dict()

    def layout_stats(self) -> dict:
        return self._stats(self._lib.po_get_layout_stats, PoLayoutStats)

    def layout_reduce(self, edges: OverlapResult, length_fuzz: int = 1000, want_flags: bool = False):
        if not -2**31 <= int(length_fuzz) < 2**31:
            raise ValueError("length_fuzz does not fit 32 bits")
        prm = PoReduceParams(int(length_fuzz), 0)
        return self._edge_stage(self._lib.po_layout_reduce, edges, prm, want_flags)

    def reduce_stats(self) -> dict:
        return self._stats(self._lib.po_get_reduce_stats, PoReduceStats)

    def layout_tips(self, edges: OverlapResult, max_tip_len: int = 4, max_tip_len_bases: int = 5000, want_flags: bool = False):
        if not 0 <= int(max_tip_len) < 2**32:
            raise ValueError("max_tip_len does not fit 32 bits")
        if not -2**31 <= int(max_tip_len_bases) < 2**31:
            raise ValueError("max_tip_len_bases does not fit 32 bits")
        prm = PoTipsParams(int(max_tip_len), int(max_tip_len_bases), 0)
        return self._edge_stage(self._lib.po_layout_tips, edges, prm, want_flags)

    def layout_diamonds(self, edges: OverlapResult, want_flags: bool = False):
        prm = PoDiamondParams(0)
        return self._edge_stage(self._lib.po_layout_diamonds, edges, prm, want_flags)

    def diamond_stats(self) -> dict:
        return self._stats(self._lib.po_get_diamond_stats, PoDiamondStats)

    def layout_merge(self, edges: OverlapResult, want_flags: bool = False):
        prm = PoMergeParams(0)
        return self._edge_stage(self._lib.po_layout_merge, edges, prm, want_flags)

    def merge_stats(self) -> dict:
        return self._stats(self._lib.po_get_merge_stats, PoMergeStats)

    def layout_coverage(self, graph: OverlapResult, rows: OverlapResult) -> np.ndarray:
        prm = PoCoverageParams(0)
        out = np.zeros(len(graph), dtype=COVERAGE_DTYPE)
        _check(self._h, self._lib.po_layout_coverage(
            self._h, graph._ptr, rows._ptr, ctypes.byref(prm), out.ctypes.data_as(ctypes.c_void_p) if len(out) else None))
        return out

    def coverage_stats(self) -> dict:
        return self._stats(self._lib.po_get_coverage_stats, PoCoverageStats)

    def _graph_stage(self, fn, graph: OverlapResult, prm, n_order: Optional[int], outputs):
        if n_order is None:
            n_order = len(graph.node_order())
        arrays = [np.zeros(int(n_order) if per == "node" else len(graph), dtype=dt) for dt, per in outputs]
        n = ctypes.c_uint64()
        _check(self._h, fn(self._h, graph._ptr, ctypes.byref(prm), *[_ptr(a) for a in arrays], ctypes.byref(n)))
        return (*arrays[:-1], arrays[-1][:int(n.value)].copy())

    def layout_components(self, graph: OverlapResult, n_order: Optional[int] = None):
        return self._graph_stage(self._lib.po_layout_components, graph, PoComponentsParams(0), n_order,
                                 [(np.uint32, "node"), (np.uint32, "edge"), (COMPONENT_DTYPE, "node")])

    def components_stats(self) -> dict:
        return self._stats(self._lib.po_get_components_stats, PoComponentsStats)

    def layout_partition(self, graph: OverlapResult, n_order: Optional[int] = None):
        return self._graph_stage(self._lib.po_layout_partition, graph, PoPartitionParams(0), n_order,
                                 [(np.uint32, "node"), (np.uint8, "node"), (np.uint8, "edge"), (SCC_DTYPE, "node")])

    def partition_stats(self) -> dict:
        return self._stats(self._lib.po_get_partition_stats, PoPartitionStats)

    def graph_from_edges(self, edges, node_order) -> OverlapResult:
        edges = np.asarray(edges)
        if edges.dtype != EDGE_DTYPE:
            arr = edges.reshape(-1, 4)
            out = np.empty(len(arr), dtype=EDGE_DTYPE)
            for k, name in enumerate(EDGE_DTYPE.names):
                out[name] = arr[:, k]
            edges = out
        edges = np.ascontiguousarray(edges)
        order = np.ascontiguousarray(np.asarray(node_order, dtype=np.int64).reshape(-1))
        if len(order) and (order.min() < 0 or order.max() >= 2**32):
            raise ValueError("a node of the node order does not fit 32 bits")
        order = order.astype(np.uint32)
        r = ctypes.c_void_p()
        _check(self._h, self._lib.po_graph_from_edges(self._h, _ptr(edges), len(edges), _ptr(order), len(order), ctypes.byref(r)))
        return OverlapResult(self, r, EDGE_DTYPE)

    def node_order_stats(self) -> dict:
        return self._stats(self._lib.po_get_node_order_stats, PoNodeOrderStats)

    def tips_stats(self) -> dict:
        return self._stats(self._lib.po_get_tips_stats, PoTipsStats)

    def __len__(self) -> int:
        return int(self._lib.po_num_sequences(self._h))

    def ids(self) -> List[str]:
        out = []
        p = ctypes.c_void_p()
        n = ctypes.c_size_t()
        for i in range(len(self)):
            self._lib.po_get_id(self._h, i, ctypes.byref(p), ctypes.byref(n))
            out.append(ctypes.string_at(p.value, n.value).decode("utf-8", "surrogateescape") if n.value else "")
        return out

    def lengths(self) -> np.ndarray:
        return np.array([self._lib.po_get_length(self._h, i) for i in range(len(self))], dtype=np.int64)

    def stats(self) -> dict:
        s = PoStats()
        _check(self._h, self._lib.po_get_stats(self._h, ctypes.byref(s)))
        return s.as_dict()

    def close(self) -> None:
        if getattr(self, "_h", None):
            self._lib.po_destroy(self._h)
            self._h = None

    def __del__(self):
        try:
            self.close()
        except Exception:
            pass
```

Measured before the change: 1.524 billion.

## Extrapolate candidate caps for unpredicted stream pieces and pre-reserve device buffers

On the first streamed call, when no prediction from an earlier call exists, candidate capacities for later pieces are estimated from counts of already-finished pieces. A small linear-program bound over word-range sums drives the estimate, so those pieces can use the asynchronous count path instead of a blocking host sync. A single rows block is pre-allocated and carved into per-piece slices, and per-call device/host buffers are reserved up front to avoid hipMalloc/hipHostMalloc during streaming. Stream-info counters are added for diagnostics. The risks are wasted memory from over-reservation and fallback to the classic path when an extrapolated cap is too small.

```diff
diff --git a/include/phasm_overlap.h b/include/phasm_overlap.h
--- a/include/phasm_overlap.h
+++ b/include/phasm_overlap.h
@@ -368,10 +368,25 @@
                             po_row* rows_out, uint64_t n_rows_expected);
 int po_debug_expand_packed(const uint64_t* records, uint64_t n, uint32_t sh_b, uint32_t sh_p, const uint32_t* lengths, uint32_t n_reads,
                            uint32_t paired, po_row* rows_out, uint64_t n_rows_expected);
+uint64_t po_debug_extrap_cap(const uint64_t* w, const uint64_t* cnt, uint32_t n_known, uint32_t n_pieces, uint32_t target, double scale);
 int po_debug_fault_backtrace(int fd);
 int po_debug_pointer_info(const void* p, int32_t* hip_type, int32_t* hsa_type, uint64_t* base, uint64_t* bytes);
 
 po_status po_get_stats(const po_handle* h, po_stats* out);
+#define PO_STREAM_INFO_PIECES 16
+typedef struct po_stream_info {
+    uint32_t n_pieces;
+    uint32_t n_predicted;
+    uint32_t n_extrapolated;
+    uint32_t n_sync;
+    uint32_t n_misses;
+    uint32_t dev_allocs_queued, host_allocs_queued;
+    uint32_t dev_allocs_call, host_allocs_call;
+    uint32_t n_deferred_rows;
+    uint64_t piece_count[PO_STREAM_INFO_PIECES];
+    uint64_t piece_cap[PO_STREAM_INFO_PIECES];
+} po_stream_info;
+po_status po_last_stream_info(const po_handle* h, po_stream_info* out);
 const char* po_last_error(const po_handle* h);
 int po_abi_version(void);
 
diff --git a/phasm_amd/_lib.py b/phasm_amd/_lib.py
--- a/phasm_amd/_lib.py
+++ b/phasm_amd/_lib.py
@@ -155,6 +155,20 @@
 
     def as_dict(self) -> dict:
         return {name: getattr(self, name) for name, _ in self._fields_}
+
+
+class PoStreamInfo(ctypes.Structure):
+    _fields_ = [("n_pieces", ctypes.c_uint32), ("n_predicted", ctypes.c_uint32), ("n_extrapolated", ctypes.c_uint32),
+                ("n_sync", ctypes.c_uint32), ("n_misses", ctypes.c_uint32),
+                ("dev_allocs_queued", ctypes.c_uint32), ("host_allocs_queued", ctypes.c_uint32),
+                ("dev_allocs_call", ctypes.c_uint32), ("host_allocs_call", ctypes.c_uint32), ("n_deferred_rows", ctypes.c_uint32),
+                ("piece_count", ctypes.c_uint64 * 16), ("piece_cap", ctypes.c_uint64 * 16)]
+
+    def as_dict(self) -> dict:
+        d = {name: getattr(self, name) for name, _ in self._fields_[:10]}
+        d["piece_count"] = list(self.piece_count)[:self.n_pieces]
+        d["piece_cap"] = list(self.piece_cap)[:self.n_pieces]
+        return d
 
 
 class PoStats(ctypes.Structure):
@@ -256,6 +270,8 @@
     ("po_result_node_order", ctypes.c_int, [_P, ctypes.c_void_p, ctypes.c_uint64, ctypes.POINTER(ctypes.c_uint64)]),
     ("po_get_node_order_stats", ctypes.c_int, [_P, ctypes.POINTER(PoNodeOrderStats)]),
     ("po_get_stats", ctypes.c_int, [_P, ctypes.POINTER(PoStats)]),
+    ("po_last_stream_info", ctypes.c_int, [_P, ctypes.POINTER(PoStreamInfo)]),
+    ("po_debug_extrap_cap", ctypes.c_uint64, [ctypes.c_void_p, ctypes.c_void_p, ctypes.c_uint32, ctypes.c_uint32, ctypes.c_uint32, ctypes.c_double]),
     ("po_last_error", ctypes.c_char_p, [_P]),
     ("po_debug_fault_backtrace", ctypes.c_int, [ctypes.c_int]),
     ("po_debug_store_words", ctypes.c_uint64, [_P, ctypes.c_int, ctypes.POINTER(ctypes.c_void_p)]),
diff --git a/phasm_amd/csrc/c_api.hip b/phasm_amd/csrc/c_api.hip
--- a/phasm_amd/csrc/c_api.hip
+++ b/phasm_amd/csrc/c_api.hip
@@ -289,6 +289,16 @@
     uint64_t st_pred_cand[PO_MAX_PIECES] = {};
     std::vector<uint32_t> st_pred_sig;
     bool st_pred_valid = false;
+    bool st_extrap = false;
+    uint32_t st_pieces = 0, st_max_na = 0;
+    uint64_t st_w[PO_MAX_PIECES + 1] = {};
+    uint64_t st_cnt[PO_MAX_PIECES] = {};
+    uint32_t st_known_n = 0;
+    DevBuf rows_block;
+    size_t rows_block_used = 0;
+    po_stream_info st_info = {};
+    uint32_t call_dev_allocs = 0, call_host_allocs = 0;
+    uint64_t reserve_bases = 0;
     bool phase_events = true;
     bool pair_events = true;
     bool st_selfclean = false;
@@ -404,6 +414,7 @@
 po_status ensure(po_handle* h, DevBuf& b, size_t bytes, double scale = 1.0, bool arena_ok = true) {
     if (bytes <= b.cap) return PO_OK;
     AllocTrace tr("hipMalloc", bytes);
+    if (h) ++h->call_dev_allocs;
     const bool first = b.p == nullptr;
     b.release();
     size_t want = bytes + bytes / 8 + 256;
@@ -447,6 +458,7 @@
 po_status ensure_host(po_handle* h, HostBuf& b, size_t bytes) {
     if (bytes <= b.cap) return PO_OK;
     AllocTrace tr("hipHostMalloc", bytes);
+    if (h) ++h->call_host_allocs;
     b.release();
     const size_t want = bytes + bytes / 16 + 4096;
     hipError_t e = hipHostMalloc(&b.p, want, hipHostMallocDefault);
@@ -468,6 +480,7 @@
 }
 
 po_status init_device(po_handle* h);
+void call_reserve_grow(po_handle* h);
 
 inline bool home_enabled() {
     const char* e = getenv("PHASM_HOME");
@@ -479,6 +492,14 @@
     h->pool_bases = bases + bases / 2;
     if (getenv("PHASM_NO_POOL")) return;
     if (!h->dev_ready && init_device(h) != PO_OK) h->err.clear();
+    const bool exact = bases == h->total_bases;
+    struct ReserveLast {
+        po_handle* h;
+        bool on;
+        ~ReserveLast() {
+            if (on) call_reserve_grow(h);
+        }
+    } reserve_last{h, exact};
     const uint64_t want = std::min<uint64_t>(h->pool_bases / 160 * sizeof(po_row), 4ull << 30);
     if (h->spare_host.cap >= want || h->live_results) return;
     int n = 0;
@@ -1213,6 +1234,140 @@
     return static_cast<const char*>(h->stage_host.p) + off;
 }
 
+inline bool in_rows_block(const po_handle* h, const DevBuf& b) {
+    const char* p = static_cast<const char*>(b.p), *lo = static_cast<const char*>(h->rows_block.p);
+    return p && lo && p >= lo && p < lo + h->rows_block.cap;
+}
+
+void rows_block_reset(po_handle* h) {
+    for (DevBuf& b : h->chunk_rows)
+        if (in_rows_block(h, b)) b = DevBuf();
+    if (in_rows_block(h, h->spare_rows)) h->spare_rows = DevBuf();
+    h->rows_block_used = 0;
+}
+
+bool rows_block_remake(po_handle* h, size_t bytes) {
+    if (h->live_results) return false;
+    rows_block_reset(h);
+    if (ensure(h, h->rows_block, bytes, 1.0, false) != PO_OK) {
+        h->err.clear();
+        (void)hipGetLastError();
+        return false;
+    }
+    return true;
+}
+
+DevBuf rows_block_carve(po_handle* h, size_t bytes) {
+    DevBuf s;
+    const size_t need = (bytes + 255) & ~size_t(255);
+    if (!h->rows_block.p || h->rows_block_used + need > h->rows_block.cap) return s;
+    s.p = h->rows_block.as<char>() + h->rows_block_used;
+    s.cap = need;
+    s.arena = true;
+    h->rows_block_used += need;
+    return s;
+}
+
+void call_reserve_grow(po_handle* h) {
+    if (getenv("PHASM_NO_POOL") || !h->dev_ready || h->live_results || h->segments_only) return;
+    const uint64_t n = h->len.size();
+    if (!n || !h->total_bases) return;
+    if (hipSetDevice(h->device) != hipSuccess) {
+        (void)hipGetLastError();
+        return;
+    }
+    auto half_more = [](uint64_t v) { return v + v / 2; };
+    const uint64_t n_t = half_more(n) + 2;
+    const uint64_t words_t = half_more((uint64_t)h->words[0].size() + h->words[1].size()) + 74;
+    const uint64_t tiles_t = words_t / po::TILE_WORDS + n_t;
+    const uint64_t exc_t = half_more(h->exc_pos.size());
+    if (n_t >= 0xFFFFFFF0ull || tiles_t > 0x7FFFFF00ull / po::WAVE) return;
+    size_t stage = ((size_t)n_t + 1) * 4 + (size_t)exc_t * 5 + 192 + (size_t)n_t / 2 + 64;
+    for (const WordStore& w : h->words)
+        if (!store_is_pinned(w) && half_more(w.size()) * 8 <= STAGE_MAX) stage += (size_t)half_more(w.size()) * 8 + 64;
+    const size_t first_bytes = (size_t)n_t * (n_t > 160000 ? LEAD_WORDS : 2u) * 8;
+    const size_t rows_bytes = (size_t)std::min<uint64_t>(half_more(h->total_bases) / 160 * sizeof(po::Cand), 2ull << 30);
+    const size_t dev_total = (size_t)words_t * 8 + (size_t)n_t * 16 + (size_t)tiles_t * sizeof(po::TileRec) + first_bytes + rows_bytes;
+    size_t mem_free = 0, mem_total = 0;
+    if (hipMemGetInfo(&mem_free, &mem_total) != hipSuccess || dev_total + dev_total / 4 > mem_free / 2) {
+        (void)hipGetLastError();
+        return;
+    }
+    AllocTrace tr("call reserve", dev_total);
+    const uint32_t dev0 = h->call_dev_allocs, host0 = h->call_host_allocs;
+    bool ok = ensure(h, h->d_words, (size_t)words_t * 8) == PO_OK && ensure(h, h->d_woff, ((size_t)n_t + 1) * 8) == PO_OK &&
+              ensure(h, h->d_len, ((size_t)n_t + 1) * 4) == PO_OK && ensure(h, h->d_read_tile0, ((size_t)n_t + 1) * 4) == PO_OK &&
+              ensure(h, h->d_tiles, ((size_t)tiles_t + 1) * sizeof(po::TileRec)) == PO_OK &&
+              ensure_host(h, h->stage_host, stage) == PO_OK && ensure_host(h, h->meta_host, (size_t)n_t * 16 + 64) == PO_OK;
+    if (ok && h->bits == 2)
+        ok = ensure(h, h->d_first, first_bytes) == PO_OK && ensure(h, h->d_defer, ((size_t)1 << 16) * sizeof(po::Cand) + 16) == PO_OK;
+    if (ok && h->bits == 2 && h->rows_block.cap < rows_bytes) (void)rows_block_remake(h, rows_bytes);
+    if (!ok) {
+        h->err.clear();
+        (void)hipGetLastError();
+    }
+    h->call_dev_allocs = dev0;
+    h->call_host_allocs = host0;
+    h->meta_n = 0xFFFFFFFFu;
+    h->reserve_bases = h->total_bases;
+}
+
+constexpr double EXTRAP_TOL = 0.2;
+constexpr double EXTRAP_MARGIN = 1.6;
+constexpr uint64_t EXTRAP_FLOOR = 64;
+
+double extrap_bound(const double* a, const double* b, const double* c, uint32_t n, bool* ok) {
+    struct Half { double a, b, r; };
+    Half hp[2 * PO_MAX_PIECES + 2];
+    uint32_t m = 0;
+    for (uint32_t i = 0; i < n; ++i) {
+        hp[m++] = Half{a[i], b[i], c[i] / (1.0 - EXTRAP_TOL)};
+        hp[m++] = Half{-a[i], -b[i], -c[i] / (1.0 + EXTRAP_TOL)};
+    }
+    hp[m++] = Half{-1.0, 0.0, 0.0};
+    hp[m++] = Half{0.0, -1.0, 0.0};
+    double best = -1.0;
+    for (uint32_t j = 0; j < m; ++j)
+        for (uint32_t k = j + 1; k < m; ++k) {
+            const double det = hp[j].a * hp[k].b - hp[k].a * hp[j].b;
+            if (std::fabs(det) < 1e-12 * (std::fabs(hp[j].a * hp[k].b) + std::fabs(hp[k].a * hp[j].b)) || det == 0.0) continue;
+            const double x = (hp[j].r * hp[k].b - hp[k].r * hp[j].b) / det, y = (hp[j].a * hp[k].r - hp[k].a * hp[j].r) / det;
+            bool inside = true;
+            for (uint32_t q = 0; q < m && inside; ++q)
+                inside = hp[q].a * x + hp[q].b * y <= hp[q].r + 1e-9 * (std::fabs(hp[q].r) + std::fabs(hp[q].a * x) + std::fabs(hp[q].b * y) + 1.0);
+            if (inside) best = std::max(best, x + y);
+        }
+    *ok = best >= 0.0;
+    return best;
+}
+
+uint64_t extrap_cap(const uint64_t* w, const uint64_t* cnt, uint32_t n_known, uint32_t n_pieces, uint32_t target, double scale,
+                    uint32_t min_known = 2) {
+    if (!w || !cnt || n_known < min_known || n_known < 1 || target < n_known || target >= n_pieces || n_pieces > (uint32_t)PO_MAX_PIECES) return 0;
+    if (w[target + 1] <= w[target]) return 0;
+    const double wt0 = (double)w[target], wt1 = (double)w[target + 1];
+    const double dq_t = wt1 * wt1 - wt0 * wt0, dl_t = wt1 - wt0;
+    double a[PO_MAX_PIECES], b[PO_MAX_PIECES], c[PO_MAX_PIECES];
+    uint32_t n = 0;
+    double envelope = 0;
+    for (uint32_t i = 0; i < n_known; ++i) {
+        if (w[i + 1] <= w[i]) continue;
+        const double wi0 = (double)w[i], wi1 = (double)w[i + 1];
+        a[n] = (wi1 * wi1 - wi0 * wi0) / dq_t;
+        b[n] = (wi1 - wi0) / dl_t;
+        c[n] = (double)cnt[i];
+        if (i + 3 >= n_known) envelope = std::max(envelope, c[n] / std::min(a[n], b[n]));
+        ++n;
+    }
+    if (n < std::max(1u, min_known)) return 0;
+    bool ok = false;
+    const double bound = extrap_bound(a, b, c, n, &ok);
+    const double est = ok ? bound * EXTRAP_MARGIN * (1.0 - EXTRAP_TOL) : envelope * EXTRAP_MARGIN;
+    const double cap = (est + (double)EXTRAP_FLOOR) * (scale > 0 ? scale : 1.0);
+    if (!(cap >= 1.0) || cap >= (double)(16u << 20)) return 0;
+    return (uint64_t)cap;
+}
+
 po_status upload_meta(po_handle* h, bool* generate_out) {
     const uint32_t n = (uint32_t)h->len.size();
     const size_t per = 64 / h->bits;
@@ -1480,13 +1635,36 @@
     if (ver_timed) (void)hipEventElapsedTime(&S.ms_verify_kernel, ev[EV_VER0], ev[EV_VER1]);
 }
 
+inline void note_count(po_handle* h, uint32_t k, uint64_t c) {
+    if (k >= (uint32_t)PO_MAX_PIECES) return;
+    h->st_info.piece_count[k] = c;
+    if (k < h->st_known_n) return;
+    for (uint32_t i = h->st_known_n; i < k; ++i) h->st_cnt[i] = 0;
+    h->st_cnt[k] = c;
+    h->st_known_n = k + 1;
+}
+
+inline bool extrap_enabled() {
+    return !getenv("PHASM_SYNC_COUNT") && !getenv("PHASM_TAIL_CLASSIC") && !getenv("PHASM_STREAM_SYNC");
+}
+
+inline double extrap_scale_env() {
+    const char* e = getenv("PHASM_EXTRAP_SCALE");
+    const double v = e ? atof(e) : 1.0;
+    return v > 0 ? v : 1.0;
+}
+
 uint64_t finish_piece(po_handle* h, bool* needs_classic) {
     po_handle::Pending& P = h->st_pend;
     const int o = P.tail ? P.zone : 2, c = P.tail ? P.zone + 1 : 4;
     *needs_classic = P.tail && h->pinned[P.zone + 7] != 0;
     if (P.cap_c) {
         P.S.n_candidates = h->pinned[P.zone + 8];
-        if (P.S.n_candidates > P.cap_c) *needs_classic = true;
+        note_count(h, P.k, P.S.n_candidates);
+        if (P.S.n_candidates > P.cap_c) {
+            *needs_classic = true;
+            ++h->st_info.n_misses;
+        }
     }
     const uint64_t n_rows = h->pinned[o];
     P.S.n_rows = n_rows;
@@ -1841,11 +2019,23 @@
     const int zone = 64 + 16 * (int)(shard & 1u);
     uint32_t cap_c = 0;
     bool async_count = false, pred_order = true;
-    if (streamed && h->st_harvest && h->st_pred_valid && !dp && !want_cands && !getenv("PHASM_SYNC_COUNT") && !getenv("PHASM_TAIL_CLASSIC")) {
+    const bool extrapolate = !h->st_pred_valid && h->st_extrap;
+    if (streamed && h->st_harvest && (h->st_pred_valid || h->st_extrap) && !dp && !want_cands && !getenv("PHASM_SYNC_COUNT") && !getenv("PHASM_TAIL_CLASSIC")) {
         uint64_t pred = h->st_pred_cand[shard];
         uint64_t cap = pred + pred / 50 + 256;
         if (const char* e = getenv("PHASM_PRED_SCALE")) cap = pred = (uint64_t)((double)pred * atof(e));
+        if (extrapolate) cap = pred = extrap_cap(h->st_w, h->st_cnt, h->st_known_n, h->st_pieces, shard, extrap_scale_env());
         const uint64_t worst = cap * 4u;
+        if (extrapolate && pred) {
+            const uint64_t need = h->home_on ? cap * sizeof(po::Cand) : worst * sizeof(po_row);
+            if (!(h->spare_rows.p && h->spare_rows.cap >= need)) {
+                const DevBuf slice = rows_block_carve(h, need + 65536);
+                if (slice.p) {
+                    h->spare_rows.release();
+                    h->spare_rows = slice;
+                }
+            }
+        }
         bool order = pred >= 400000 && (r_end - r_begin) >= 4096;
         if (const char* e = getenv("PHASM_VERIFY_ORDER")) order = atoi(e) != 0;
         pred_order = order;
@@ -1858,6 +2048,11 @@
                                   fits(h->d_vrank, (uint64_t)(r_end - r_begin) * 4))) && h->dev_words < 0xFFFFFFF0ull;
         cap_c = (uint32_t)cap;
     }
+    if (streamed && shard < (uint32_t)PO_MAX_PIECES) {
+        h->st_info.piece_cap[shard] = async_count ? cap_c : 0u;
+        if (async_count) ++(extrapolate ? h->st_info.n_extrapolated : h->st_info.n_predicted);
+        else ++h->st_info.n_sync;
+    }
     volatile uint64_t* count_slot = async_count ? &h->pinned[zone + 8] : &h->pinned[1];
     volatile uint64_t* also_slot = async_count ? &h->pinned[zone + 9] : &h->pinned[8];
     if (ntiles <= po::PS_SMALL_MAX) {
@@ -1876,7 +2071,7 @@
     if (async_count) {
         n_cand64 = cap_c;
         n_selfrep_reads = 0;
-        S.n_predicted = 1;
+        S.n_predicted = extrapolate ? 0u : 1u;
         G.n_dev = scalars;
         G.cap = cap_c;
     } else {
@@ -1887,6 +2082,7 @@
         HIP_TRY(h, hipStreamSynchronize(st));
         n_cand64 = h->pinned[1];
         n_selfrep_reads = (uint32_t)h->pinned[8];
+        if (streamed) note_count(h, shard, n_cand64);
     }
     if (nshards > 1 || streamed || wide || dpE) n_selfrep_reads |= 1u;
     S.n_candidates = n_cand64;
@@ -1903,6 +2099,27 @@
     std::function<po_status()> classic_tail;
     const bool sel_in_verify = (nshards > 1 || streamed || wide) && !dp && !getenv("PHASM_SELECT_KERNEL");
     if (n_cand) {
+        if (streamed && extrapolate && !async_count) {
+            uint64_t n_room = n_cand, n_sum = (uint64_t)n_cand + 4096;
+            const double sc = std::max(1.0, extrap_scale_env());
+            for (uint32_t j = shard + 1; j < h->st_pieces; ++j) {
+                const uint64_t c = extrap_cap(h->st_w, h->st_cnt, h->st_known_n, h->st_pieces, j, sc, 1);
+                n_room = std::max(n_room, c + c / 4);
+                n_sum += c + c / 4 + 4096;
+            }
+            n_room = std::min<uint64_t>(n_room, 16u << 20);
+            PO_TRY(ensure(h, h->d_cand_a, (size_t)n_room * 4));
+            PO_TRY(ensure(h, h->d_cand_p, (size_t)n_room * 4));
+            PO_TRY(ensure(h, h->d_cand_b, (size_t)n_room * 4));
+            PO_TRY(ensure(h, h->d_type, (size_t)n_room));
+            PO_TRY(ensure(h, h->d_rowcnt, (size_t)n_room));
+            PO_TRY(ensure(h, h->d_row_off, ((size_t)n_room + 1) * 4));
+            PO_TRY(ensure(h, h->d_vlabel, (size_t)h->st_max_na * 4));
+            PO_TRY(ensure(h, h->d_vperm, (size_t)h->st_max_na * 4));
+            PO_TRY(ensure(h, h->d_vrank, (size_t)h->st_max_na * 4));
+            const uint64_t block = n_sum * (h->home_on ? sizeof(po::Cand) : 4u * sizeof(po_row));
+            if (h->rows_block_used == 0 && h->rows_block.cap < block && block <= (2ull << 30)) (void)rows_block_remake(h, (size_t)block);
+        }
         PO_TRY(ensure_piece(h, h->d_cand_a, (size_t)n_cand * 4));
         PO_TRY(ensure_piece(h, h->d_cand_p, (size_t)n_cand * 4));
         PO_TRY(ensure_piece(h, h->d_cand_b, (size_t)n_cand * 4));
@@ -2085,8 +2302,15 @@
         const bool home_tail_ok = h->home_on && !want_cands && !dpE && !getenv("PHASM_TAIL_CLASSIC") &&
                                   (!n_selfrep_reads || ((nshards > 1 || streamed || wide) && n_cand < (16u << 20))) &&
                                   cdiv(n_cand, po::TAIL_TILE) <= po::TAIL_MAX_TILES;
-        if (home_tail_ok && !async_count && h->spare_rows.cap < (size_t)n_cand * sizeof(po::Cand))
-            PO_TRY(ensure(h, h->spare_rows, (size_t)n_cand * sizeof(po::Cand) + (streamed ? 65536 : 0), 1.0, false));
+        if (home_tail_ok && !async_count && h->spare_rows.cap < (size_t)n_cand * sizeof(po::Cand)) {
+            const DevBuf slice = streamed && extrapolate ? rows_block_carve(h, (size_t)n_cand * sizeof(po::Cand) + 65536) : DevBuf();
+            if (slice.p) {
+                h->spare_rows.release();
+                h->spare_rows = slice;
+            } else {
+                PO_TRY(ensure(h, h->spare_rows, (size_t)n_cand * sizeof(po::Cand) + (streamed ? 65536 : 0), 1.0, false));
+            }
+        }
         const bool compact_tail = home_tail_ok && h->spare_rows.p && h->spare_rows.cap >= (size_t)n_cand * sizeof(po::Cand);
         const bool can_tail = compact_tail ||
                               (!want_cands && !dpE && h->spare_rows.p && h->spare_rows.cap >= worst_rows * sizeof(po_row) &&
@@ -3850,6 +4074,18 @@
 
 int po_abi_version(void) { return PO_ABI_VERSION; }
 
+static_assert(PO_STREAM_INFO_PIECES == PO_MAX_PIECES, "po_stream_info holds every piece of a streamed call");
+
+po_status po_last_stream_info(const po_handle* h, po_stream_info* out) {
+    if (!h || !out) return PO_ERR_INVALID;
+    *out = h->st_info;
+    return PO_OK;
+}
+
+uint64_t po_debug_extrap_cap(const uint64_t* w, const uint64_t* cnt, uint32_t n_known, uint32_t n_pieces, uint32_t target, double scale) {
+    return extrap_cap(w, cnt, n_known, n_pieces, target, scale);
+}
+
 po_status po_create(po_handle** out) {
     if (!out) return PO_ERR_INVALID;
     po_handle* h = new (std::nothrow) po_handle();
@@ -3897,6 +4133,7 @@
         h->scratch_host.release();
         h->home_stage.release();
         for (DevBuf& b : h->chunk_rows) b.release();
+        h->rows_block.release();
         h->d_first.release();
         h->d_defer.release();
         h->meta_host.release();
@@ -4024,6 +4261,7 @@
         ::close(fd);
         if (done) {
             if (h->total_bases >= h->pool_bases && h->total_bases >= (64ull << 20)) result_pool_grow(h);
+            else if (h->total_bases >= (64ull << 20) && h->total_bases / 2 >= h->reserve_bases / 2 + h->reserve_bases / 4) call_reserve_grow(h);
             if (h->bits == 2) note_first_words(h);
             return PO_OK;
         }
@@ -4451,8 +4689,9 @@
 std::vector<uint32_t> stream_bounds(const po_handle* h) {
     const uint32_t n = (uint32_t)h->len.size();
     const uint64_t bytes0 = (uint64_t)h->words[0].size() * 8;
-    uint64_t max_pieces = h->chunk_rows[0].p ? 12 : 8;
-    const bool big = bytes0 >= (512ull << 20) && h->chunk_rows[0].p;
+    const bool cheap_pieces = h->chunk_rows[0].p || extrap_enabled();
+    uint64_t max_pieces = cheap_pieces ? 12 : 8;
+    const bool big = bytes0 >= (512ull << 20) && cheap_pieces;
     if (big) max_pieces = 15;
     if (const char* e = getenv("PHASM_STREAM_MAX_PIECES")) max_pieces = (uint64_t)std::max(2, std::min(PO_MAX_PIECES - 1, atoi(e)));
     const uint32_t n_pieces = (uint32_t)std::min<uint64_t>(max_pieces, std::max<uint64_t>(2, (bytes0 + (8ull << 20)) / (16ull << 20)));
@@ -4576,6 +4815,19 @@
     sig.push_back((uint32_t)(h->total_bases & 0xFFFFFFFFu));
     h->st_pred_valid = h->st_pred_valid && sig == h->st_pred_sig;
     uint64_t new_pred[PO_MAX_PIECES] = {};
+    h->st_extrap = !h->st_pred_valid && extrap_enabled();
+    h->st_pieces = P;
+    h->st_known_n = 0;
+    h->st_max_na = 0;
+    for (uint32_t k = 0; k <= P; ++k) h->st_w[k] = bounds[k] < n ? h->woff[bounds[k]] : h->words[0].size();
+    for (uint32_t k = 0; k < P; ++k) h->st_max_na = std::max(h->st_max_na, bounds[k + 1] - bounds[k]);
+    std::memset(h->st_cnt, 0, sizeof(h->st_cnt));
+    h->st_info = po_stream_info();
+    h->st_info.n_pieces = P;
+    if (h->st_extrap) {
+        if (!h->live_results) rows_block_reset(h);
+        else h->rows_block_used = h->rows_block.cap + 1;
+    }
     h->st_selfclean = false;
     h->st_early_index = P > 1 && h->poison < 0 && !getenv("PHASM_NO_INDEX_REUSE") && !getenv("PHASM_LATE_INDEX");
     {
@@ -4586,6 +4838,8 @@
         h->st_lead = (h->bits == 2 && wide && m >= 32u * 4u + 31u && !(win && atoi(win) < 4) && !getenv("PHASM_STREAM_LEAD2")) ? LEAD_WORDS : 2u;
     }
     PO_TRY(stream_begin(h, bounds));
+    h->st_info.dev_allocs_queued = h->call_dev_allocs;
+    h->st_info.host_allocs_queued = h->call_host_allocs;
     if (trace) std::fprintf(stderr, "[stream] %u pieces queued at %.3f ms\n", P, since());
     if (h->st_early_index) {
         po_result part;
@@ -4611,6 +4865,7 @@
     auto completed = [&](uint32_t k, const po_stats& S, uint64_t nk) -> po_status {
         add_stats(sum, S);
         new_pred[k] = S.n_candidates;
+        note_count(h, k, S.n_candidates);
         const double seen = (double)bounds[k + 1] / (double)n;
         if (h->chunk_compact[k]) PO_TRY(append_home(h, R, h->chunk_rows[k], S.n_verified, nk, k, P, seen * seen));
         else PO_TRY(append_rows(h, R, h->chunk_rows[k], nk, k, P, seen * seen));
@@ -4733,6 +4988,7 @@
             sum.verify_bytes_algo += h->pinned[6];
             sum.verify_bytes_exec += h->pinned[7];
             sum.n_rows += n_rows;
+            h->st_info.n_deferred_rows = (uint32_t)std::min<uint64_t>(n_rows, 0xFFFFFFFFull);
             sum.ms_verify += ms_def;
             sum.ms_total += ms_def;
             PO_TRY(append_rows(h, R, h->chunk_rows[P], n_rows, P, P + 1));
@@ -4764,6 +5020,7 @@
     po_stats sum = {};
     bool streamed = false, overflowed = false;
     float ms_upload = 0;
+    h->call_dev_allocs = h->call_host_allocs = 0;
     try {
         st = init_device(h);
         if (st == PO_OK && !h->copy_stream && hipStreamCreateWithFlags(&h->copy_stream, hipStreamNonBlocking) != hipSuccess)
@@ -4808,6 +5065,11 @@
         st = fail(h, PO_ERR_NOMEM, "out of host memory in po_overlaps_to_host");
     }
     h->st_on = false;
+    h->st_extrap = false;
+    if (streamed || overflowed) {
+        h->st_info.dev_allocs_call = h->call_dev_allocs;
+        h->st_info.host_allocs_call = h->call_host_allocs;
+    }
     h->st_harvest = nullptr;
     h->st_pend.valid = false;
     h->ev = h->ev_sets[0];
diff --git a/phasm_amd/overlapper.py b/phasm_amd/overlapper.py
--- a/phasm_amd/overlapper.py
+++ b/phasm_amd/overlapper.py
@@ -478,6 +478,12 @@
         _check(self._h, self._lib.po_get_stats(self._h, ctypes.byref(s)))
         return s.as_dict()
 
+    def stream_info(self) -> dict:
+        from ._lib import PoStreamInfo
+        s = PoStreamInfo()
+        _check(self._h, self._lib.po_last_stream_info(self._h, ctypes.byref(s)))
+        return s.as_dict()
+
     def close(self) -> None:
         if getattr(self, "_h", None):
             self._lib.po_destroy(self._h)
```

Result: slower. 1.473 billion (-3.4%).
